# OFA-Sys/ONE-PEACE

Measured on AMD Instinct MI355X. Metric: pretrain samples/s (tri-modal global batch) ONE-PEACE-4B, higher is better.
Workload: dtype bf16

## Files before the change

include/onepeace_hip.h:

```cpp
#ifndef ONEPEACE_HIP_H
#define ONEPEACE_HIP_H

#include <stdint.h>

#ifdef __cplusplus
extern "C" {
#endif

int op_abi_version(void);
const char* op_last_error(void);

int op_prof_enable(int on);
int op_prof_reserve(int events);
int op_prof_collect(double* ms, int64_t* count, double* work, int n_families);

int op_layernorm_fwd(const void* x, const void* w, const void* b, void* y, float* mean, float* rstd, int64_t rows,
                     int64_t cols, float eps, int act_gelu, int dtype, const int* x_rows, void* stream);
int64_t op_layernorm_bwd_workspace_bytes(int64_t rows, int64_t cols);
int op_layernorm_bwd(const void* dy, const void* x, const void* w, const void* b, const float* mean, const float* rstd,
                     const void* add, void* dx, void* dw, void* db, void* workspace, int64_t rows, int64_t cols,
                     int act_gelu, int accumulate, int dtype, const int* x_rows, void* stream);
int op_layernorm_bwd_skip(const void* dy, const void* x, const void* w, const float* mean, const float* rstd, const void* add, void* dx,
                          void* dw, void* db, void* workspace, int64_t rows, int64_t cols, int accumulate, const float* ps,
                          int64_t rows_per_sample, void* stream);

int op_gemm_nt(const void* A, int64_t lda, const void* B0, const void* B1, const void* B2, int64_t ldb, int64_t n_seg,
               const void* bias0, const void* bias1, const void* bias2, void* C, int64_t ldc, void* h0, void* h1,
               const void* resid, int64_t ldr, const void* gamma, const float* rowscale, int64_t rows_per_sample,
               const float* alpha, int64_t M, int64_t N, int64_t K, int epilogue, void* workspace, int64_t workspace_bytes,
               int64_t tune, const int* resid_rows, int64_t resid_rows_total, void* stream);
int op_gemm_tn(const void* A, int64_t lda, const void* B, int64_t ldb, void* C, int64_t ldc, int64_t M, int64_t N, int64_t K,
               int accumulate, void* workspace, int64_t workspace_bytes, int64_t tune, void* stream);
int op_gemm_nt_grouped(int64_t nprob, const void* const* A, const int64_t* M, int64_t lda, const void* const* B, int64_t ldb,
                       const void* const* bias, void* const* C, int64_t ldc, void* const* h0, void* const* h1,
                       const void* const* resid, int64_t ldr, const void* const* gamma, const float* const* rowscale,
                       const int64_t* rows_per_sample, int64_t N, int64_t K, int epilogue, int64_t tune, const int* const* resid_rows,
                       int64_t resid_rows_total, void* stream);
int op_gemm_nt_batched(const void* A, int64_t lda, int64_t stride_a, const void* W, int64_t ldb, int64_t stride_b, const void* bias,
                       int64_t stride_bias, void* C, int64_t ldc, int64_t stride_c, int64_t M, int64_t N, int64_t K, int64_t batch,
                       void* stream);
int op_audio_conv1_ln_gelu_fwd(const void* wav, int64_t stride, const void* w0, const void* b0, const void* lnw, const void* lnb, void* y,
                               float* mean, float* rstd, int64_t rows, int64_t C, float eps, void* stream);
int64_t op_audio_conv1_ln_gelu_bwd_workspace_bytes(int64_t C);
int op_audio_conv1_ln_gelu_bwd(const void* dy, const void* wav, int64_t stride, const void* w0, const void* b0, const void* lnw, const void* lnb,
                               const float* mean, const float* rstd, void* dw0, void* db0, void* dlnw, void* dlnb, void* workspace,
                               int64_t rows, int64_t C, int accumulate, void* stream);
int64_t op_gemm_tn_grouped_counter_bytes(void);
int64_t op_gemm_tn_grouped_plan(int64_t nprob, const int64_t* M, const int64_t* N, const int64_t* K, int64_t workgroups, int64_t tune,
                                int32_t* out, int64_t cap);
int op_gemm_tn_grouped(int64_t nprob, const void* const* A, const int64_t* lda, const void* const* B, const int64_t* ldb, void* const* C,
                       const int64_t* ldc, const int64_t* M, const int64_t* N, const int64_t* K, const int32_t* accumulate,
                       const void* const* W, const int64_t* ldw, float* const* rowdot, const void* const* rscale, void* counters,
                       int64_t tune, void* stream);
int op_gemm_tn_grouped_lists(int64_t nprob, const void* const* A, const int64_t* lda, const void* const* B, const int64_t* ldb, void* const* C,
                             const int64_t* ldc, const int64_t* M, const int64_t* N, const int64_t* K, const int32_t* accumulate,
                             const void* const* W, const int64_t* ldw, float* const* rowdot, const void* const* rscale,
                             const int32_t* const* ktiles, const int32_t* const* n_ktiles, void* counters, int64_t tune, void* stream);
int op_live_ktiles(int64_t nseg, const float* const* ps, const int64_t* row0, const int64_t* S, const int64_t* B, int64_t nprob,
                   const int64_t* prob_row0, const int64_t* prob_rows, int32_t* const* ktiles, int32_t* const* n_ktiles, void* stream);
int op_live_mwindows(int64_t nseg, const float* const* ps, const int64_t* ps_stride, const int64_t* row0, const int64_t* S, const int64_t* B,
                     const int64_t* wps, const int64_t* odd, const int64_t* seg_list, const int64_t* seg_prob, const int64_t* seg_base, int64_t nlist,
                     int32_t* const* windows,
                     int32_t* const* n_windows, const int64_t* max_windows, int64_t nout, void* const* out, const int64_t* out_ld,
                     const int64_t* out_cols, const int64_t* out_rows, void* stream);
int op_gemm_nt_grouped_windows(int64_t nprob, const void* const* A, const int64_t* M, int64_t lda, const void* const* B, int64_t ldb,
                               void* const* C, int64_t ldc, int64_t N, int64_t K, const int32_t* windows, const int32_t* n_windows,
                               int64_t max_windows, int64_t max_row_stride, int64_t tune, void* stream);
int op_live_mwindows_fwd(int64_t nseg, const float* const* ps, const int64_t* ps_stride, const int64_t* row0, const int64_t* S, const int64_t* B,
                         const int64_t* wps, const int64_t* odd, const int64_t* seg_list, const int64_t* seg_prob, const int64_t* seg_base,
                         int64_t nlist, int32_t* const* windows, int32_t* const* n_windows, const int64_t* max_windows, int64_t nout,
                         void* const* out, const int64_t* out_ld, const int64_t* out_cols, const int64_t* out_rows,
                         const void* const* out_src, const int64_t* out_src_ld, void* stream);
int op_gemm_nt_grouped_windows_fwd(int64_t nprob, const void* const* A, const int64_t* M, int64_t lda, const void* const* B, int64_t ldb,
                                   int64_t n_seg, const void* const* bias, void* const* C, int64_t ldc, const void* const* resid, int64_t ldr,
                                   const void* const* gamma, const float* const* rowscale, const int64_t* rows_per_sample, int64_t N,
                                   int64_t K, int epilogue, const int32_t* windows, const int32_t* n_windows, int64_t max_windows,
                                   int64_t max_row_stride, int64_t tune, void* stream);
int op_gemm_plan(int64_t M, int64_t N, int64_t K, int epilogue, int has_bias, int64_t workspace_bytes, int64_t tune, int* plan);

int op_quant_fp8_rows(const void* x, int64_t ldx, void* q, int64_t ldq, float* scale, int64_t rows, int64_t cols, void* stream);
int op_layernorm_fwd_q8(const void* x, const void* w, const void* b, void* y, float* mean, float* rstd, void* q8, float* q8_scale,
                        int64_t rows, int64_t cols, float eps, void* stream);
int op_ln_geglu_fwd_q8(const void* h0, const void* h1, int64_t ldh, const void* w, const void* b, void* y, float* mean, float* rstd, void* q8,
                       float* q8_scale, int64_t rows, int64_t cols, float eps, void* stream);
int op_gemm_nt_fp8(const void* A8, int64_t lda, const float* sa, const void* B0, const void* B1, int64_t ldb, const float* sb0,
                   const float* sb1, const void* bias, void* C, int64_t ldc, void* h0, void* h1, const void* resid, int64_t ldr,
                   const void* gamma, const float* rowscale, int64_t rows_per_sample, int64_t M, int64_t N, int64_t K, int epilogue,
                   int64_t tune, void* stream);

int op_attn_fwd(const void* q, const void* k, const void* v, int64_t ld, const void* bias, int64_t bias_batch_stride,
                const void* bias_frag, const void* key_pad, void* out, int64_t ldo, float* lse, int64_t lse_ld, int64_t B,
                int64_t S, int64_t Spad, int64_t heads, int64_t head_dim, float scale, int64_t tune, void* stream);
int64_t op_attn_bias_frag_elems(int64_t n_img, int64_t S);
int op_attn_bias_pack(const void* src, void* dst, int64_t n_img, int64_t S, int64_t Spad, void* stream);
int op_attn_bwd_delta(const void* dout, const void* out, int64_t ldo, float* delta, int64_t B, int64_t S, int64_t Spad,
                      int64_t heads, void* stream);
int64_t op_attn_bwd_dbias_slabs(int64_t B, int64_t S, int64_t heads, int64_t tune);
int op_attn_bwd(const void* q, const void* k, const void* v, int64_t ld, const void* dout, const void* out, int64_t ldo,
                const void* bias, const void* biasT, const void* bias_frag, int64_t bias_batch_stride, const void* key_pad,
                const float* lse, float* delta, void* dq,
                void* dk, void* dv, int64_t ldg, float* dbias, int64_t B, int64_t S, int64_t Spad, int64_t heads,
                int64_t head_dim, float scale, int64_t tune, void* stream);

int op_relpos_bias_build(const void* table, const int* bucket, int64_t bucket_ld, void* out, int64_t heads, int64_t S,
                         int64_t Spad, int transposed, void* stream);
int op_relpos_bias_bwd(const float* dbias, int64_t S, int64_t Spad, const int* pos, const int* seg, int64_t nseg, const int* bucket_seg,
                       int64_t num_rel, float* partial_ws, float* dtable, int64_t heads, void* stream);
int op_relpos_bias_build_ids(const void* table, const int* bucket, int64_t bucket_ld, const int* ids, void* out, int64_t B,
                             int64_t heads, int64_t K, int64_t Kpad, int transposed, void* stream);
int op_relpos_bias_fold_ids(const float* dbias, const int* ids, float* dense_ws, int64_t Sfull, int64_t B, int64_t heads, int64_t K,
                            int64_t Kpad, void* stream);

int op_transpose(const void* in, void* out, int64_t rows, int64_t cols, int64_t ld_in, int64_t ld_out, void* stream);
int op_transpose_scaled(const void* in, void* out, int64_t rows, int64_t cols, int64_t ld_in, int64_t ld_out, const void* scale,
                        void* stream);
int op_transpose_batched(const void* table, int64_t n, int64_t total_tiles, void* stream);
int64_t op_transpose_desc_bytes(void);
int64_t op_colsum_workspace_bytes(int64_t N);
int op_colsum_segments(const void* x, void* out0, void* out1, void* out2, void* workspace, int64_t M, int64_t n_seg,
                       int64_t seg_cols, int accumulate, void* stream);
int64_t op_resid_bwd_workspace_bytes(int64_t N);
int op_resid_bwd(const void* dout, const void* y, const void* gamma, const float* rowscale, int64_t rows_per_sample,
                 void* dbranch, void* dgamma, void* dbias, float* g0, void* workspace, int64_t M, int64_t N, int accumulate,
                 const int* dout_rows, void* stream);
int op_resid_bwd_skip(const void* dout, const void* y, const void* gamma, const float* rowscale, int64_t rows_per_sample,
                      void* dbranch, void* dgamma, void* dbias, float* g0, void* workspace, int64_t M, int64_t N, int accumulate,
                      const int* dout_rows, void* stream);
int op_gamma_grad_finish(const float* rowdot, int64_t slots, const void* b0, const float* g00, const void* b1, const float* g01,
                         const void* b2, const float* g02, void* dgamma, int64_t N, int accumulate, void* stream);
int op_ln_geglu_bwd(const void* dy, const void* h0, const void* h1, const void* w, const float* mean, const float* rstd,
                    void* dh0, void* dh1, int64_t ldd, int64_t ldh, void* dw, void* db, void* workspace, int64_t rows,
                    int64_t cols, int accumulate, void* stream);
int op_ln_geglu_fwd(const void* h0, const void* h1, int64_t ldh, const void* w, const void* b, void* y, float* mean, float* rstd,
                    int64_t rows, int64_t cols, float eps, void* stream);
int op_ln_geglu_fwd_skip(const void* h0, const void* h1, int64_t ldh, const void* w, const void* b, void* y, float* mean, float* rstd,
                         int64_t rows, int64_t cols, float eps, const float* ps, int64_t rows_per_sample, void* stream);
int op_ln_geglu_bwd_skip(const void* dy, const void* h0, const void* h1, const void* w, const float* mean, const float* rstd,
                         void* dh0, void* dh1, int64_t ldd, int64_t ldh, void* dw, void* db, void* workspace, int64_t rows,
                         int64_t cols, int accumulate, const float* ps, int64_t rows_per_sample, void* stream);
int op_colsum(const void* x, const void* y, const float* rowscale, int64_t rows_per_sample, const void* mul, void* out,
              void* workspace, int64_t M, int64_t N, int accumulate, int out_dtype, void* stream);
int op_geglu_bwd(const void* dg, const void* h0, const void* h1, void* dh0, void* dh1, int64_t numel, void* stream);
int op_scale_rows(const void* dout, const void* gamma, const float* rowscale, int64_t rows_per_sample, void* dbranch,
                  int64_t M, int64_t N, void* stream);

int op_l2norm_fwd(const void* x, void* y, float* inv_norm, int64_t rows, int64_t cols, float eps, int out_dtype, void* stream);
int op_l2norm_bwd(const void* dy, const void* y, const float* inv_norm, void* dx, int64_t rows, int64_t cols, int y_dtype,
                  void* stream);
int op_infonce_rows(float* sim, int64_t rows, int64_t n, int64_t ld, int64_t target0, float label_smoothing, float gscale,
                    float* row_loss, float* row_hit, float* row_dot, int write_grad, void* stream);

int op_adamw_step(void* p, const void* g, float* m, float* v, int64_t numel, float lr, float beta1, float beta2, float eps,
                  float weight_decay, int64_t step, float grad_scale, const float* grad_sqnorm, float clip_norm,
                  void* stream);
int op_adamw_step_groups(void* p, const void* g, float* m, float* v, int64_t numel, const int64_t* group_end8,
                         const float* group_lr_scale, const float* group_weight_decay, int64_t n_groups, float lr, float beta1,
                         float beta2, float eps, int64_t step, float grad_scale, const float* grad_sqnorm, float clip_norm,
                         void* stream);
int op_adamw_step_groups_master(void* p, float* master, const void* g, float* m, float* v, int64_t numel,
                                const int64_t* group_end8, const float* group_lr_scale, const float* group_weight_decay,
                                int64_t n_groups, float lr, float beta1, float beta2, float eps, int64_t step, float grad_scale,
                                const float* grad_sqnorm, float clip_norm, void* stream);
int op_ema_step(float* ema, const void* p, int64_t numel, float keep, float take, void* stream);
int op_adamw_step_groups_ema(void* p, float* master, const void* g, float* m, float* v, float* ema, int64_t numel,
                             const int64_t* group_end8, const float* group_lr_scale, const float* group_weight_decay,
                             int64_t n_groups, float lr, float beta1, float beta2, float eps, int64_t step, float grad_scale,
                             const float* grad_sqnorm, float clip_norm, float ema_keep, float ema_take, void* stream);
int op_adamw_step_shard(void* p, const void* g, int64_t numel, int64_t first8, int64_t count8, float* m, float* v, float* master,
                        float* ema, const int64_t* group_end8, const float* group_lr_scale, const float* group_weight_decay,
                        int64_t n_groups, float lr, float beta1, float beta2, float eps, int64_t step, float grad_scale,
                        const float* grad_sqnorm, float clip_norm, float ema_keep, float ema_take, void* stream);
int op_sqnorm(const void* x, int64_t numel, float* workspace, float* out, void* stream);

int op_rows_gather(const void* src, void* dst, const int* list, int64_t nseg, const int64_t* src_row0, const int64_t* dst_row0,
                   const int64_t* S, const int64_t* n_kept, const int64_t* dst_rows, const int64_t* n_samples, const int64_t* list_off,
                   int64_t dst_total, int64_t cols, void* stream);
int op_rows_merge(const void* base, const void* upd, void* out, const int* list, int64_t nseg, const int64_t* src_row0,
                  const int64_t* dst_row0, const int64_t* S, const int64_t* n_kept, const int64_t* dst_rows, const int64_t* n_samples,
                  const int64_t* list_off, int64_t total, int64_t cols, void* stream);
int op_rows_map(int* map, const int* list, int64_t nseg, const int64_t* src_row0, const int64_t* dst_row0, const int64_t* S,
                const int64_t* n_kept, const int64_t* dst_rows, const int64_t* n_samples, const int64_t* list_off, int64_t dst_total,
                void* stream);

int64_t op_sim_topk_splits(int64_t M, int64_t N, int64_t splits);
int64_t op_sim_topk_workspace_bytes(int64_t M, int64_t N, int64_t k, int64_t splits);
// ... 70 lines not shown
```

one-peace_amd/csrc/attention.hip:

```cpp
#include <type_traits>

#include "common.h"

namespace {

constexpr int HD = 64;
constexpr int BQ = 128;
constexpr int BKV = 64;
constexpr int VSTRIDE = 160;

struct AttnArgs {
  const bf16_t* q; const bf16_t* k; const bf16_t* v; int64_t ld;
  const bf16_t* bias;
  int64_t bias_bs;
  const uint8_t* key_pad;
  bf16_t* out; int64_t ldo;
  float* lse;
  int64_t lse_ld;
  int B, S, Spad, heads;
  float scale;
};

__device__ __forceinline__ bf16x8 pack8(const float* a, const float* b) {
  bf16x8 r;
// ... 366 lines not shown
      if (FULL || kb < nkb) {
#pragma unroll
        for (int r = 0; r < 4; ++r) {
          const float e = __builtin_amdgcn_exp2f(__builtin_fmaf(st[kb][r], c1, -m2_use));
          pv[kb][r] = e;
          psum += e;
        }
      } else {
#pragma unroll
        for (int r = 0; r < 4; ++r) pv[kb][r] = 0.f;
      }
    }
    l_run = l_run * alpha + psum;
#pragma unroll
    for (int db = 0; db < 4; ++db)
#pragma unroll
      for (int r = 0; r < 4; ++r) ot[db][r] *= alpha;
    bf16x8 pf[2];
    pf[0] = pack8(pv[0], pv[1]);
    pf[1] = pack8(pv[2], pv[3]);

#pragma unroll
    for (int m = 0; m < 2; ++m) {
      if (!FULL && 2 * m >= nkb) break;
#pragma unroll
      for (int db = 0; db < 4; ++db) {
        const bf16x8 vf = join_tr(tr_read(vt + trsw[db] + (2 * m) * 2048), tr_read(vt + trsw[db] + (2 * m + 1) * 2048));
        ot[db] = __builtin_amdgcn_mfma_f32_16x16x32_bf16(vf, pf[m], ot[db], 0, 0, 0);
      }
    }
  };

  const int ntiles = (p.S + BKV - 1) / BKV;
  for (int kt = 0; kt < ntiles; ++kt) {
    const int k0 = kt * BKV;
    if (k0 + BKV <= p.S) tile(k0, std::true_type{});
    else tile(k0, std::false_type{});
  }

  float l = l_run;
  l += __shfl_xor(l, 16);
  l += __shfl_xor(l, 32);
  if (q0 + t >= p.S) continue;
  const float inv = 1.f / l;
  bf16_t* op = p.out + (row_base + q0 + t) * p.ldo + h * HD;
#pragma unroll
  for (int db = 0; db < 4; ++db) {
    bf16x4 o;
#pragma unroll
    for (int r = 0; r < 4; ++r) o[r] = (bf16_t)(ot[db][r] * inv);
    *reinterpret_cast<bf16x4*>(op + db * 16 + g * 4) = o;
  }
  if (g == 0 && p.lse) p.lse[((int64_t)b * p.heads + h) * p.lse_ld + q0 + t] = m2_run * (1.0f / LOG2E) + logf(l);
  }
}

constexpr int PERS_NW = 8;
constexpr int PERS_MAX_ROWS = 288;
constexpr int PERS_SCR = 68;
constexpr int PERS_PPT = 2;

__device__ __forceinline__ s16x4 tr_read_a(const char* p) {
  s16x4 r;
  asm volatile("ds_read_b64_tr_b16 %0, %1" : "=v"(r) : "v"((unsigned)(uintptr_t)((__attribute__((address_space(3))) const char*)p)));
  return r;
}
#define ATTN_WAIT_LGKM0()                         \
  do {                                            \
    __builtin_amdgcn_s_waitcnt(0xC07F);           \
    __builtin_amdgcn_sched_barrier(0);            \
  } while (0)

__device__ __forceinline__ void gload16_asm(bf16x8& d, const void* p) { asm volatile("global_load_dwordx4 %0, %1, off" : "=v"(d) : "v"(p)); }
__device__ __forceinline__ void gload4_asm(unsigned& d, const void* p) { asm volatile("global_load_dword %0, %1, off" : "=v"(d) : "v"(p)); }
template <int OFF>
__device__ __forceinline__ void gload16_s(bf16x8& d, const void* sbase, unsigned voff) {
  asm volatile("s_nop 4\n\tglobal_load_dwordx4 %0, %1, %2 offset:%3" : "=v"(d) : "v"(voff), "s"(sbase), "n"(OFF));
}
template <int OFF>
__device__ __forceinline__ void gload4_s(unsigned& d, const void* sbase, unsigned voff) {
  asm volatile("s_nop 4\n\tglobal_load_dword %0, %1, %2 offset:%3" : "=v"(d) : "v"(voff), "s"(sbase), "n"(OFF));
}

template <bool HAS_BIAS, bool HAS_PAD>
__global__ __launch_bounds__(PERS_NW * 64, 2) void attn_fwd_pers_kernel(AttnArgs p, const bf16_t* __restrict__ bias_frag, int rows_pad,
                                                                         int nitems) {
  extern __shared__ __attribute__((aligned(16))) char smem[];
  const int tid = threadIdx.x, lane = tid & 63;
  const int wid = __builtin_amdgcn_readfirstlane(tid >> 6);
  const int g = lane >> 4, t = lane & 15;
  const int KVB = 2 * rows_pad * 128;
  float* scratch = reinterpret_cast<float*>(smem + 2 * KVB);
  const int nqb = (p.S + 15) >> 4, nkp = (p.S + 31) >> 5;
  const bool has_left = nqb > 2 * PERS_NW;
  const int q0 = wid * 32;
  const int nact = min(2, max(0, nqb - 2 * wid));
  const int64_t per_head = (int64_t)nqb * nkp * FRAG_BLOCK;
  const int ntiles = (p.S + BKV - 1) / BKV;
  const float c1 = p.scale * LOG2E;

  bf16x8 sel_lo, sel_hi;
  {
    const bf16_t inv = (bf16_t)(1.0f / p.scale), zero = (bf16_t)0.f;
#pragma unroll
    for (int i = 0; i < 8; ++i) {
      sel_lo[i] = (g * 8 + i == t) ? inv : zero;
      sel_hi[i] = (g * 8 + i == 16 + t) ? inv : zero;
    }
  }
  int trsw[4];
#pragma unroll
  for (int db = 0; db < 4; ++db) trsw[db] = tr_off_swz(0, db, g, t);
  const int kswz[2] = {((0 * 4 + g) ^ (t & 7)) << 4, ((1 * 4 + g) ^ (t & 7)) << 4};

  const int ngrp = rows_pad >> 3;
  const int r_in = lane >> 3, slot = lane & 7;
  const int npiece = (2 * ngrp - wid + PERS_NW - 1) / PERS_NW;
  auto piece = [&](int it, int buf, int j) {
    const int b = it / p.heads, h = it - b * p.heads;
    const int grp = wid + j * PERS_NW;
    const bool isv = grp >= ngrp;
    const int gi = isv ? grp - ngrp : grp;
    const int r = gi * 8 + r_in;
    const int kr = min(r, p.S - 1);
    const bf16_t* src = (isv ? p.v : p.k) + ((int64_t)b * p.S + kr) * p.ld + h * HD + ((slot ^ (r & 7)) << 3);
    char* dst = smem + buf * KVB + (isv ? rows_pad * 128 : 0) + gi * 1024;
    __builtin_amdgcn_global_load_lds((const __attribute__((address_space(1))) void*)src,
                                     (__attribute__((address_space(3))) void*)dst, 16, 0, 0);
  };
  auto load_q = [&](int it, int qrow, bf16x8 (&q)[2]) {
    const int b = it / p.heads, h = it - b * p.heads;
    const bf16_t* qp = p.q + ((int64_t)b * p.S + qrow) * p.ld + h * HD;
#pragma unroll
    for (int kk = 0; kk < 2; ++kk) q[kk] = *reinterpret_cast<const bf16x8*>(qp + kk * 32 + g * 8);
  };
  const int qi_main[2] = {min(q0 + t, p.S - 1), min(q0 + 16 + t, p.S - 1)};

  bf16x8 bn[2][2];
  unsigned padn[4] = {0u, 0u, 0u, 0u};
  auto small_loads = [&](int it, int kt) {
    const int b = it / p.heads, h = it - b * p.heads;
    if constexpr (HAS_BIAS) {
      const bf16_t* fhead = bias_frag + ((p.bias_bs != 0 ? (int64_t)b * p.heads : 0) + h) * per_head + lane * 8;
#pragma unroll
      for (int qb = 0; qb < 2; ++qb) {
        const bf16_t* fb = fhead + (int64_t)min(2 * wid + qb, nqb - 1) * nkp * FRAG_BLOCK;
#pragma unroll
        for (int m = 0; m < 2; ++m) gload16_asm(bn[qb][m], fb + min(2 * kt + m, nkp - 1) * FRAG_BLOCK);
      }
    }
    if constexpr (HAS_PAD) {
      const uint8_t* pr = p.key_pad + (int64_t)b * p.Spad + g * 4 + kt * BKV;
#pragma unroll
      for (int kb = 0; kb < 4; ++kb) gload4_asm(padn[kb], pr + kb * 16);
    }
  };

  constexpr int NSMALL = (HAS_BIAS ? 4 : 0) + (HAS_PAD ? 4 : 0);
  bf16x8 qn[2][2], ql[2], bfl[2];
  unsigned padl[2][2] = {{0u, 0u}, {0u, 0u}};
  auto late_loads = [&](int it_next, int it) {
    {
      const int b = it_next / p.heads, h = it_next - b * p.heads;
#pragma unroll
      for (int qb = 0; qb < 2; ++qb) {
        const bf16_t* qp = p.q + ((int64_t)b * p.S + qi_main[qb]) * p.ld + h * HD;
#pragma unroll
        for (int kk = 0; kk < 2; ++kk) gload16_asm(qn[qb][kk], qp + kk * 32 + g * 8);
      }
    }
    if (has_left) {
      const int b = it / p.heads, h = it - b * p.heads;
      const bf16_t* qp = p.q + ((int64_t)b * p.S + p.S - 1) * p.ld + h * HD;
#pragma unroll
      for (int kk = 0; kk < 2; ++kk) gload16_asm(ql[kk], qp + kk * 32 + g * 8);
      if constexpr (HAS_BIAS) {
        const bf16_t* fleft = bias_frag + ((p.bias_bs != 0 ? (int64_t)b * p.heads : 0) + h) * per_head + lane * 8 + (int64_t)(nqb - 1) * nkp * FRAG_BLOCK;
        gload16_asm(bfl[0], fleft + wid * FRAG_BLOCK);
        gload16_asm(bfl[1], fleft + min(PERS_NW, nkp - 1) * FRAG_BLOCK);
      }
      if constexpr (HAS_PAD) {
        const uint8_t* pr = p.key_pad + (int64_t)b * p.Spad + g * 4;
#pragma unroll
        for (int j = 0; j < 2; ++j) {
          gload4_asm(padl[0][j], pr + (2 * wid + j) * 16);
          gload4_asm(padl[1][j], pr + min((2 * PERS_NW + j) * 16, p.Spad - 16));
        }
      }
    }
  };

  int item = blockIdx.x;
  const int step = gridDim.x;
  if (item < nitems) {
    for (int j = 0; j < npiece; ++j) piece(item, 0, j);
    load_q(item, qi_main[0], qn[0]);
    load_q(item, qi_main[1], qn[1]);
    small_loads(item, 0);
  }
  int buf = 0, prev_item = -1;
  auto wait_all = [&]() {
    asm volatile("s_waitcnt vmcnt(0)" : "+v"(qn[0][0]), "+v"(qn[0][1]), "+v"(qn[1][0]), "+v"(qn[1][1]), "+v"(bn[0][0]), "+v"(bn[0][1]), "+v"(bn[1][0]), "+v"(bn[1][1]),
                 "+v"(padn[0]), "+v"(padn[1]), "+v"(padn[2]), "+v"(padn[3]) : : "memory");
  };
  wait_all();

  auto merge_left = [&](int it, int sb) {
    const float* sc = scratch + sb * (PERS_NW * PERS_SCR);
    float M = -INFINITY;
#pragma unroll
    for (int w = 0; w < PERS_NW; ++w) M = fmaxf(M, sc[w * PERS_SCR + 64]);
    float L = 0.f, o = 0.f;
#pragma unroll
    for (int w = 0; w < PERS_NW; ++w) {
      const float f = __builtin_amdgcn_exp2f(sc[w * PERS_SCR + 64] - M);
      L = __builtin_fmaf(sc[w * PERS_SCR + 65], f, L);
      o = __builtin_fmaf(sc[w * PERS_SCR + lane], f, o);
    }
    const int b = it / p.heads, h = it - b * p.heads;
    const int qrow = p.S - 1;
    p.out[((int64_t)b * p.S + qrow) * p.ldo + h * HD + lane] = (bf16_t)(o / L);
    if (lane == 0 && p.lse) p.lse[((int64_t)b * p.heads + h) * p.lse_ld + qrow] = M * (1.0f / LOG2E) + logf(L);
  };

  for (; item < nitems; item += step, buf ^= 1) {
    const int b = item / p.heads, h = item - b * p.heads;
    const int64_t row_base = (int64_t)b * p.S;
    __syncthreads();
    bf16x8 qf[2][2] = {{qn[0][0], qn[0][1]}, {qn[1][0], qn[1][1]}};
    const bool more = item + step < nitems;
    const int nxt = more ? item + step : item;
    if (has_left && prev_item >= 0 && wid == ((prev_item / step) & (PERS_NW - 1))) merge_left(prev_item, buf ^ 1);
    prev_item = item;

    const char* ldsK = smem + buf * KVB;
    const char* ldsV = ldsK + rows_pad * 128;

    f32x4 ot[2][4];
    float m2_run[2] = {-INFINITY, -INFINITY}, l_run[2] = {0.f, 0.f};
#pragma unroll
    for (int qb = 0; qb < 2; ++qb)
#pragma unroll
      for (int db = 0; db < 4; ++db) ot[qb][db] = (f32x4){0.f, 0.f, 0.f, 0.f};

    auto tile = [&](const int kt, auto full_c) {
      constexpr bool FULL = decltype(full_c)::value;
      const int k0 = kt * BKV;
      const int nkb = FULL ? 4 : ((p.S - k0 + 15) >> 4);
      bf16x8 bf[2][2];
      unsigned padw[4] = {0u, 0u, 0u, 0u};
      if constexpr (HAS_BIAS) {
#pragma unroll
        for (int qb = 0; qb < 2; ++qb)
#pragma unroll
          for (int m = 0; m < 2; ++m) bf[qb][m] = bn[qb][m];
      }
      if constexpr (HAS_PAD) {
#pragma unroll
        for (int kb = 0; kb < 4; ++kb) padw[kb] = padn[kb];
      }
      __builtin_amdgcn_sched_barrier(0);
      if constexpr (FULL) {
        small_loads(item, kt + 1);
      } else {
        late_loads(nxt, item);
        small_loads(nxt, 0);
      }
      __builtin_amdgcn_sched_barrier(0);
#pragma unroll
      for (int jj = 0; jj < PERS_PPT; ++jj) piece(nxt, buf ^ 1, min(kt * PERS_PPT + jj, npiece - 1));
      __builtin_amdgcn_sched_barrier(0);
      if (nact == 0) return;

      const char* kt_ = ldsK + k0 * 128;
      const char* vt = ldsV + k0 * 128;
      f32x4 st[2][4];
#pragma unroll
      for (int qb = 0; qb < 2; ++qb)
#pragma unroll
        for (int kb = 0; kb < 4; ++kb) st[qb][kb] = (f32x4){0.f, 0.f, 0.f, 0.f};
#pragma unroll
      for (int kb = 0; kb < 4; ++kb) {
        if (!FULL && kb >= nkb) break;
#pragma unroll
        for (int kk = 0; kk < 2; ++kk) {
          const bf16x8 kf = *reinterpret_cast<const bf16x8*>(kt_ + (kb * 16 + t) * 128 + kswz[kk]);
#pragma unroll
          for (int qb = 0; qb < 2; ++qb) st[qb][kb] = __builtin_amdgcn_mfma_f32_16x16x32_bf16(kf, qf[qb][kk], st[qb][kb], 0, 0, 0);
        }
        if constexpr (HAS_BIAS) {
#pragma unroll
          for (int qb = 0; qb < 2; ++qb)
            st[qb][kb] = __builtin_amdgcn_mfma_f32_16x16x32_bf16(bf[qb][kb >> 1], (kb & 1) ? sel_hi : sel_lo, st[qb][kb], 0, 0, 0);
        }
      }
      s16x4 va0[4], va1[4];
#pragma unroll
      for (int db = 0; db < 4; ++db) {
        va0[db] = tr_read_a(vt + trsw[db]);
        va1[db] = tr_read_a(vt + trsw[db] + 2048);
      }
      bf16x8 pf[2][2];
#pragma unroll
      for (int qb = 0; qb < 2; ++qb) {
        float mx = -INFINITY;
#pragma unroll
        for (int kb = 0; kb < 4; ++kb) {
          if (!FULL && kb >= nkb) break;
          const int key = k0 + kb * 16 + g * 4;
#pragma unroll
          for (int r = 0; r < 4; ++r) {
            if constexpr (!FULL || HAS_PAD) {
              bool masked = false;
              if constexpr (!FULL) masked = key + r >= p.S;
              if constexpr (HAS_PAD) masked = masked || ((padw[kb] >> (8 * r)) & 0xffu);
              st[qb][kb][r] = masked ? -INFINITY : st[qb][kb][r];
            }
            mx = fmaxf(mx, st[qb][kb][r]);
          }
        }
        mx = fmaxf(mx, __shfl_xor(mx, 16));
        mx = fmaxf(mx, __shfl_xor(mx, 32));
        const float m2_new = fmaxf(m2_run[qb], mx * c1);
        const float m2_use = (m2_new == -INFINITY) ? 0.f : m2_new;
        const float alpha = __builtin_amdgcn_exp2f(m2_run[qb] - m2_use);
        m2_run[qb] = m2_new;
        float psum = 0.f;
        float pv[4][4];
#pragma unroll
        for (int kb = 0; kb < 4; ++kb) {
          if (FULL || kb < nkb) {
#pragma unroll
            for (int r = 0; r < 4; ++r) {
              const float e = __builtin_amdgcn_exp2f(__builtin_fmaf(st[qb][kb][r], c1, -m2_use));
              pv[kb][r] = e;
              psum += e;
            }
          } else {
#pragma unroll
            for (int r = 0; r < 4; ++r) pv[kb][r] = 0.f;
          }
        }
        l_run[qb] = l_run[qb] * alpha + psum;
#pragma unroll
        for (int db = 0; db < 4; ++db)
#pragma unroll
          for (int r = 0; r < 4; ++r) ot[qb][db][r] *= alpha;
        pf[qb][0] = pack8(pv[0], pv[1]);
// ... 776 lines not shown
#pragma unroll
        for (int kb = 0; kb < 4; ++kb) { st[kb] = (f32x4){0.f, 0.f, 0.f, 0.f}; ds[0][kb] = (f32x4){0.f, 0.f, 0.f, 0.f}; }
#pragma unroll
        for (int kb = 0; kb < 4; ++kb) {
          if (k0 + kb * 16 >= p.S) break;
#pragma unroll
          for (int kk = 0; kk < 2; ++kk) {
            st[kb] = __builtin_amdgcn_mfma_f32_16x16x32_bf16(kfrag(kb, kk), qf[0][kk], st[kb], 0, 0, 0);
            ds[0][kb] = __builtin_amdgcn_mfma_f32_16x16x32_bf16(vfrag(kb, kk), of[0][kk], ds[0][kb], 0, 0, 0);
          }
          st[kb] = __builtin_amdgcn_mfma_f32_16x16x32_bf16(bfr[kb >> 1], (kb & 1) ? sel_hi : sel_lo, st[kb], 0, 0, 0);
        }
        const float nl2 = -lse[0] * LOG2E, dl = del[0];
        const bool may_mask = (k0 + BKV > p.S) || (p.key_pad != nullptr);
        if (may_mask) {
#pragma unroll
          for (int kb = 0; kb < 4; ++kb) {
            const int key = k0 + kb * 16 + g * 4;
#pragma unroll
            for (int r = 0; r < 4; ++r) {
              const bool dead = (key + r >= p.S) || ((padw[kb] >> (8 * r)) & 0xffu);
              const float pr = __builtin_amdgcn_exp2f(dead ? -INFINITY : __builtin_fmaf(st[kb][r], c1, nl2));
              ds[0][kb][r] = pr * (ds[0][kb][r] - dl);
            }
          }
        } else {
#pragma unroll
          for (int kb = 0; kb < 4; ++kb)
#pragma unroll
            for (int r = 0; r < 4; ++r)
              ds[0][kb][r] = __builtin_amdgcn_exp2f(__builtin_fmaf(st[kb][r], c1, nl2)) * (ds[0][kb][r] - dl);
        }
      } else {
        ds_tile<1, true, (NT < 6)>(p, b, h, k0, q0w, g, t, qf, of, lse, del, kfrag, vfrag, biasfrag, prefetch, ds);
      }
#pragma unroll
      for (int c = 0; c < NT; ++c) {
        if (kt == c) {
#pragma unroll
          for (int kb = 0; kb < 4; ++kb)
            if (c < NT - 1 || kb < LASTB) acc[c][kb] += ds[0][kb];
        }
      }
#pragma unroll
      for (int m = 0; m < 2; ++m) {
        if (k0 + m * 32 >= p.S) break;
        float a0[4], a1[4];
#pragma unroll
        for (int r = 0; r < 4; ++r) { a0[r] = ds[0][2 * m][r]; a1[r] = ds[0][2 * m + 1][r]; }
        const bf16x8 dsf = pack8(a0, a1);
#pragma unroll
        for (int db = 0; db < 4; ++db) {
          const bf16x8 kT = join_tr(tr_read(ldsK + trsw[db] + (2 * m) * 2048), tr_read(ldsK + trsw[db] + (2 * m + 1) * 2048));
          dqT[db] = __builtin_amdgcn_mfma_f32_16x16x32_bf16(kT, dsf, dqT[db], 0, 0, 0);
        }
      }
    }
    if (wave_active && q0w + t < p.S) {
      bf16_t* qp = p.dq + ((int64_t)b * p.S + q0w + t) * p.ldg + h * HD;
#pragma unroll
      for (int db = 0; db < 4; ++db) {
        bf16x4 a;
#pragma unroll
        for (int r = 0; r < 4; ++r) a[r] = (bf16_t)(dqT[db][r] * p.scale);
        *reinterpret_cast<bf16x4*>(qp + db * 16 + g * 4) = a;
      }
    }
  }
  if (!wave_active || q0w + t >= p.S) return;
  float* drow = p.dbias + (((int64_t)chunk * p.heads + h) * p.S + q0w + t) * p.Spad + g * 4;
#pragma unroll
  for (int kt = 0; kt < NT; ++kt) {
    f32x4 cur[4];
#pragma unroll
    for (int kb = 0; kb < 4; ++kb)
      if ((kt < NT - 1 || kb < LASTB) && kt * BKV + kb * 16 < p.Spad) cur[kb] = *reinterpret_cast<const f32x4*>(drow + kt * BKV + kb * 16);
#pragma unroll
    for (int kb = 0; kb < 4; ++kb)
      if ((kt < NT - 1 || kb < LASTB) && kt * BKV + kb * 16 < p.Spad)
        *reinterpret_cast<f32x4*>(drow + kt * BKV + kb * 16) = cur[kb] + acc[kt][kb];
  }
}

template <bool HAS_BIAS, bool HAS_PAD, int NT, int LASTB, bool LEFT>
__device__ __forceinline__ void attn_bwd_dq_pers_body(const AttnBwdArgs& p, char* smem, int rows_pad, int nqh, int qhalf0) {
  const int tid = threadIdx.x, lane = tid & 63;
  const int wid = __builtin_amdgcn_readfirstlane(tid >> 6);
  const int g = lane >> 4, t = lane & 15;
  const int KVB = 2 * rows_pad * 128;
  float* scratch = reinterpret_cast<float*>(smem + 2 * KVB);
  const int nqb = (p.S + 15) >> 4, nkp = (p.S + 31) >> 5;
  const int qhalf = qhalf0, h = (blockIdx.x / nqh) % p.heads, chunk = blockIdx.x / (nqh * p.heads);
  const int b_begin = chunk * p.bchunk, b_end = min(p.B, b_begin + p.bchunk);
  if (b_begin >= b_end) return;
  const int qblk = qhalf * PERS_NW + wid;
  const bool active = qblk < min(nqb, 2 * PERS_NW);
  constexpr bool has_left = LEFT;
  const int q0w = min(qblk, nqb - 1) * 16;
  const int qi = min(q0w + t, p.S - 1);
  const float c1 = p.scale * LOG2E;
  const int64_t per_head = (int64_t)nqb * nkp * FRAG_BLOCK;

  bf16x8 sel_lo, sel_hi;
  {
    const bf16_t inv = (bf16_t)(1.0f / p.scale), zero = (bf16_t)0.f;
#pragma unroll
    for (int i = 0; i < 8; ++i) {
      sel_lo[i] = (g * 8 + i == t) ? inv : zero;
      sel_hi[i] = (g * 8 + i == 16 + t) ? inv : zero;
    }
  }
  int trsw[4];
#pragma unroll
  for (int db = 0; db < 4; ++db) trsw[db] = tr_off_swz(0, db, g, t);
  const int kswz[2] = {((0 * 4 + g) ^ (t & 7)) << 4, ((1 * 4 + g) ^ (t & 7)) << 4};

  const int ngrp = rows_pad >> 3;
  const int r_in = lane >> 3, slot = lane & 7;
  const int npiece = (2 * ngrp - wid + PERS_NW - 1) / PERS_NW;
  auto piece = [&](int b, int buf, int j) {
    const int grp = wid + j * PERS_NW;
    const bool isv = grp >= ngrp;
    const int gi = isv ? grp - ngrp : grp;
    int rl = r_in;
    asm volatile("" : "+v"(rl));
    const int r = gi * 8 + rl;
    const int kr = min(r, p.S - 1);
    const unsigned voff = (unsigned)((kr * (int)p.ld + ((slot ^ (r & 7)) << 3)) * 2);
    const char* sbase = (const char*)((isv ? p.v : p.k) + (int64_t)b * p.S * p.ld + h * HD);
    char* dst = smem + buf * KVB + (isv ? rows_pad * 128 : 0) + gi * 1024;
    __builtin_amdgcn_global_load_lds((const __attribute__((address_space(1))) void*)(sbase + voff),
                                     (__attribute__((address_space(3))) void*)dst, 16, 0, 0);
  };

  constexpr int NSMALL = (HAS_BIAS ? 2 : 0) + (HAS_PAD ? 4 : 0);
  constexpr int BPPT = 3;
  auto ppt_of = [](int kt) { return kt < 3 ? BPPT : 0; };
  const bf16_t* fwave = HAS_BIAS ? p.bias_frag + (int64_t)h * per_head + (int64_t)(q0w >> 4) * nkp * FRAG_BLOCK : nullptr;
  const bf16_t* fleft = HAS_BIAS ? p.bias_frag + (int64_t)h * per_head + (int64_t)(nqb - 1) * nkp * FRAG_BLOCK : nullptr;
  const unsigned vo_frag = lane * 16, vo_pad = g * 4;
  const unsigned vo_q = (unsigned)(((int64_t)qi * p.ld + h * HD + g * 8) * 2), vo_o = (unsigned)(((int64_t)qi * p.ldo + h * HD + g * 8) * 2);
  const unsigned vo_ql = (unsigned)(((int64_t)(p.S - 1) * p.ld + h * HD + g * 8) * 2), vo_ol = (unsigned)(((int64_t)(p.S - 1) * p.ldo + h * HD + g * 8) * 2);
  const unsigned vo_lse = qi * 4, vo_lsel = (p.S - 1) * 4;
  bf16x8 bn[2];
  unsigned padn[4] = {0u, 0u, 0u, 0u};
  auto small_loads = [&](int b, int kt) {
    if constexpr (HAS_BIAS) {
      gload16_s<0>(bn[0], fwave + min(2 * kt, nkp - 1) * FRAG_BLOCK, vo_frag);
      gload16_s<0>(bn[1], fwave + min(2 * kt + 1, nkp - 1) * FRAG_BLOCK, vo_frag);
    }
    if constexpr (HAS_PAD) {
      const uint8_t* pr = p.key_pad + (int64_t)b * p.Spad + kt * BKV;
      gload4_s<0>(padn[0], pr, vo_pad);
      gload4_s<16>(padn[1], pr, vo_pad);
      gload4_s<32>(padn[2], pr, vo_pad);
      gload4_s<48>(padn[3], pr, vo_pad);
    }
  };
  bf16x8 qn[2], don[2], oon[2], ql[2], dol[2], ool[2], bfl[2];
  float lsen, lsel;
  unsigned padl[2][2] = {{0u, 0u}, {0u, 0u}};
  auto query_loads = [&](int b, unsigned voq, unsigned voo, unsigned vol, bf16x8 (&q)[2], bf16x8 (&d)[2], bf16x8 (&o)[2], float& l) {
    const bf16_t* sq = p.q + (int64_t)b * p.S * p.ld;
    const bf16_t* sd = p.dout + (int64_t)b * p.S * p.ldo;
    const bf16_t* so = p.out + (int64_t)b * p.S * p.ldo;
    gload16_s<0>(q[0], sq, voq);
    gload16_s<64>(q[1], sq, voq);
    gload16_s<0>(d[0], sd, voo);
    gload16_s<64>(d[1], sd, voo);
    gload16_s<0>(o[0], so, voo);
    gload16_s<64>(o[1], so, voo);
    unsigned lw;
    gload4_s<0>(lw, p.lse + ((int64_t)b * p.heads + h) * p.Spad, vol);
    l = __builtin_bit_cast(float, lw);
  };
  auto late_loads = [&](int b_next, int b) {
    (void)b_next;
    if (has_left) {
      query_loads(b, vo_ql, vo_ol, vo_lsel, ql, dol, ool, lsel);
      if constexpr (HAS_BIAS) {
        gload16_s<0>(bfl[0], fleft + wid * FRAG_BLOCK, vo_frag);
        gload16_s<0>(bfl[1], fleft + min(PERS_NW, nkp - 1) * FRAG_BLOCK, vo_frag);
      }
      if constexpr (HAS_PAD) {
        const uint8_t* pr = p.key_pad + (int64_t)b * p.Spad;
        gload4_s<0>(padl[0][0], pr + 2 * wid * 16, vo_pad);
        gload4_s<16>(padl[0][1], pr + 2 * wid * 16, vo_pad);
        gload4_s<0>(padl[1][0], pr + min(2 * PERS_NW * 16, p.Spad - 32), vo_pad);
        gload4_s<16>(padl[1][1], pr + min(2 * PERS_NW * 16, p.Spad - 32), vo_pad);
      }
    }
  };

  f32x4 acc[NT][4], accl[2][2];
#pragma unroll
  for (int kt = 0; kt < NT; ++kt)
#pragma unroll
    for (int kb = 0; kb < 4; ++kb) acc[kt][kb] = (f32x4){0.f, 0.f, 0.f, 0.f};
#pragma unroll
  for (int i = 0; i < 2; ++i)
#pragma unroll
    for (int j = 0; j < 2; ++j) accl[i][j] = (f32x4){0.f, 0.f, 0.f, 0.f};

  for (int j = 0; j < npiece; ++j) piece(b_begin, 0, j);
  query_loads(b_begin, vo_q, vo_o, vo_lse, qn, don, oon, lsen);
  small_loads(b_begin, 0);
  int buf = 0, prev_b = -1;
  auto merge_left = [&](int b, int sb) {
    const float* sc = scratch + sb * (PERS_NW * 64);
    float o = 0.f;
#pragma unroll
    for (int w = 0; w < PERS_NW; ++w) o += sc[w * 64 + lane];
    p.dq[((int64_t)b * p.S + p.S - 1) * p.ldg + h * HD + lane] = (bf16_t)(o * p.scale);
  };

  auto wait_all = [&]() {
    asm volatile("s_waitcnt vmcnt(0)" : "+v"(qn[0]), "+v"(qn[1]), "+v"(don[0]), "+v"(don[1]), "+v"(oon[0]), "+v"(oon[1]), "+v"(lsen), "+v"(bn[0]), "+v"(bn[1]),
                 "+v"(padn[0]), "+v"(padn[1]), "+v"(padn[2]), "+v"(padn[3]) : : "memory");
  };
  wait_all();
  for (int b = b_begin; b < b_end; ++b, buf ^= 1) {
    __syncthreads();
    const bf16x8 qf[2] = {qn[0], qn[1]}, dof[2] = {don[0], don[1]};
    const float dl = delta_from_frags(dof, oon);
    const float nl2 = -lsen * LOG2E;
    if (active && g == 0 && q0w + t < p.S) p.delta_w[((int64_t)b * p.heads + h) * p.Spad + q0w + t] = dl;
    const int nxt = b + 1 < b_end ? b + 1 : b;
    if (has_left && prev_b >= 0 && wid == (prev_b & (PERS_NW - 1))) merge_left(prev_b, buf ^ 1);
    prev_b = b;
    const char* ldsK = smem + buf * KVB;
    const char* ldsV = ldsK + rows_pad * 128;
    f32x4 dqT[4];
#pragma unroll
    for (int db = 0; db < 4; ++db) dqT[db] = (f32x4){0.f, 0.f, 0.f, 0.f};

    auto tile = [&](const int kt, auto last_c) {
      constexpr bool LAST = decltype(last_c)::value;
      const int k0 = kt * BKV;
      if (kt > 0) {
        if (ppt_of(kt - 1) > 0) {
          if constexpr (HAS_BIAS && HAS_PAD)
            asm volatile("s_waitcnt vmcnt(%6)" : "+v"(bn[0]), "+v"(bn[1]), "+v"(padn[0]), "+v"(padn[1]), "+v"(padn[2]), "+v"(padn[3]) : "n"(BPPT));
          else if constexpr (HAS_BIAS)
            asm volatile("s_waitcnt vmcnt(%2)" : "+v"(bn[0]), "+v"(bn[1]) : "n"(BPPT));
          else if constexpr (HAS_PAD)
            asm volatile("s_waitcnt vmcnt(%4)" : "+v"(padn[0]), "+v"(padn[1]), "+v"(padn[2]), "+v"(padn[3]) : "n"(BPPT));
        } else {
          if constexpr (HAS_BIAS && HAS_PAD)
            asm volatile("s_waitcnt vmcnt(0)" : "+v"(bn[0]), "+v"(bn[1]), "+v"(padn[0]), "+v"(padn[1]), "+v"(padn[2]), "+v"(padn[3]));
          else if constexpr (HAS_BIAS)
            asm volatile("s_waitcnt vmcnt(0)" : "+v"(bn[0]), "+v"(bn[1]));
          else if constexpr (HAS_PAD)
            asm volatile("s_waitcnt vmcnt(0)" : "+v"(padn[0]), "+v"(padn[1]), "+v"(padn[2]), "+v"(padn[3]));
        }
      }
      bf16x8 bf[2];
      unsigned padw[4] = {0u, 0u, 0u, 0u};
      if constexpr (HAS_BIAS) { bf[0] = bn[0]; bf[1] = bn[1]; }
      if constexpr (HAS_PAD) {
#pragma unroll
        for (int kb = 0; kb < 4; ++kb) padw[kb] = padn[kb];
      }
      __builtin_amdgcn_sched_barrier(0);
      if constexpr (!LAST) {
        if constexpr (!LEFT) {
          if (kt == NT - 2) query_loads(nxt, vo_q, vo_o, vo_lse, qn, don, oon, lsen);
        }
        small_loads(b, kt + 1);
      } else {
        late_loads(nxt, b);
        small_loads(nxt, 0);
      }
      __builtin_amdgcn_sched_barrier(0);
#pragma unroll
      for (int jj = 0; jj < BPPT; ++jj)
        if (ppt_of(kt) > 0) piece(nxt, buf ^ 1, min(kt * BPPT + jj, npiece - 1));
      __builtin_amdgcn_sched_barrier(0);
      const char* kt_ = ldsK + k0 * 128;
      const char* vt = ldsV + k0 * 128;
      constexpr int NKB = LAST ? LASTB : 4;
      constexpr int NM = (NKB + 1) / 2;
      if (!active) return;
#pragma unroll
      for (int m = 0; m < NM; ++m) {
        f32x4 st[2], ds[2];
#pragma unroll
        for (int j = 0; j < 2; ++j) {
          const int kb = 2 * m + j;
          st[j] = (f32x4){0.f, 0.f, 0.f, 0.f};
          ds[j] = (f32x4){0.f, 0.f, 0.f, 0.f};
          if (kb >= NKB) continue;
#pragma unroll
          for (int kk = 0; kk < 2; ++kk) {
            const bf16x8 kf = *reinterpret_cast<const bf16x8*>(kt_ + (kb * 16 + t) * 128 + kswz[kk]);
            const bf16x8 vf = *reinterpret_cast<const bf16x8*>(vt + (kb * 16 + t) * 128 + kswz[kk]);
            st[j] = __builtin_amdgcn_mfma_f32_16x16x32_bf16(kf, qf[kk], st[j], 0, 0, 0);
            ds[j] = __builtin_amdgcn_mfma_f32_16x16x32_bf16(vf, dof[kk], ds[j], 0, 0, 0);
          }
          if constexpr (HAS_BIAS) st[j] = __builtin_amdgcn_mfma_f32_16x16x32_bf16(bf[m], j ? sel_hi : sel_lo, st[j], 0, 0, 0);
        }
#pragma unroll
        for (int j = 0; j < 2; ++j) {
          const int kb = 2 * m + j;
          if (kb >= NKB) continue;
          const int key = k0 + kb * 16 + g * 4;
#pragma unroll
          for (int r = 0; r < 4; ++r) {
            float x = __builtin_fmaf(st[j][r], c1, nl2);
            if constexpr (LAST || HAS_PAD) {
              bool dead = false;
              if constexpr (LAST) dead = key + r >= p.S;
// ... 58 lines not shown
          s4[j] = (f32x4){0.f, 0.f, 0.f, 0.f};
          d4[j] = (f32x4){0.f, 0.f, 0.f, 0.f};
#pragma unroll
          for (int kk = 0; kk < 2; ++kk) {
            const bf16x8 kf = *reinterpret_cast<const bf16x8*>(ldsK + ((2 * kp + j) * 16 + t) * 128 + kswz[kk]);
            const bf16x8 vf = *reinterpret_cast<const bf16x8*>(ldsV + ((2 * kp + j) * 16 + t) * 128 + kswz[kk]);
            s4[j] = __builtin_amdgcn_mfma_f32_16x16x32_bf16(kf, ql[kk], s4[j], 0, 0, 0);
            d4[j] = __builtin_amdgcn_mfma_f32_16x16x32_bf16(vf, dol[kk], d4[j], 0, 0, 0);
          }
          if constexpr (HAS_BIAS) s4[j] = __builtin_amdgcn_mfma_f32_16x16x32_bf16(bfl[pc], j ? sel_hi : sel_lo, s4[j], 0, 0, 0);
        }
        float a0[4], a1[4];
#pragma unroll
        for (int j = 0; j < 2; ++j)
#pragma unroll
          for (int r = 0; r < 4; ++r) {
            bool dead = (2 * kp + j) * 16 + g * 4 + r >= p.S;
            if constexpr (HAS_PAD) dead = dead || ((padl[pc][j] >> (8 * r)) & 0xffu);
            const float x = dead ? -INFINITY : __builtin_fmaf(s4[j][r], c1, nl2l);
            const float v = __builtin_amdgcn_exp2f(x) * (d4[j][r] - dll);
            d4[j][r] = v;
            (j ? a1 : a0)[r] = v;
          }
        if constexpr (HAS_BIAS) { accl[pc][0] += d4[0]; accl[pc][1] += d4[1]; }
        const bf16x8 dsf = pack8(a0, a1);
        s16x4 k0r[4], k1r[4];
#pragma unroll
        for (int db = 0; db < 4; ++db) {
          k0r[db] = tr_read_a(ldsK + trsw[db] + (2 * kp) * 2048);
          k1r[db] = tr_read_a(ldsK + trsw[db] + (2 * kp + 1) * 2048);
        }
        ATTN_WAIT_LGKM0();
#pragma unroll
        for (int db = 0; db < 4; ++db) dql[db] = __builtin_amdgcn_mfma_f32_16x16x32_bf16(join_tr(k0r[db], k1r[db]), dsf, dql[db], 0, 0, 0);
      }
      float* sc = scratch + (buf * PERS_NW + wid) * 64;
      if (t == 0) {
#pragma unroll
        for (int db = 0; db < 4; ++db) *reinterpret_cast<f32x4*>(sc + db * 16 + g * 4) = dql[db];
      }
    }

    wait_all();
  }
  if (has_left && prev_b >= 0) {
    __syncthreads();
    if (wid == 0) merge_left(prev_b, buf ^ 1);
  }
  if constexpr (HAS_BIAS) {
    if (p.dbias == nullptr) return;
    if (active && q0w + t < p.S) {
      float* drow = p.dbias + (((int64_t)chunk * p.heads + h) * p.S + q0w + t) * p.Spad + g * 4;
#pragma unroll
      for (int kt = 0; kt < NT; ++kt) {
        f32x4 cur[4];
#pragma unroll
        for (int kb = 0; kb < 4; ++kb)
          if ((kt < NT - 1 || kb < LASTB) && kt * BKV + kb * 16 < p.Spad) cur[kb] = *reinterpret_cast<const f32x4*>(drow + kt * BKV + kb * 16);
#pragma unroll
        for (int kb = 0; kb < 4; ++kb)
          if ((kt < NT - 1 || kb < LASTB) && kt * BKV + kb * 16 < p.Spad)
            *reinterpret_cast<f32x4*>(drow + kt * BKV + kb * 16) = cur[kb] + acc[kt][kb];
      }
    }
    if (has_left && t == 0) {
      float* drow = p.dbias + (((int64_t)chunk * p.heads + h) * p.S + p.S - 1) * p.Spad + g * 4;
#pragma unroll
      for (int pc = 0; pc < 2; ++pc) {
        if (pc == 1 && wid != 0) break;
        const int kp = pc == 0 ? wid : PERS_NW;
#pragma unroll
        for (int j = 0; j < 2; ++j) {
          const int key0 = (2 * kp + j) * 16;
          if (key0 < p.Spad) {
            float* d = drow + key0;
            *reinterpret_cast<f32x4*>(d) = *reinterpret_cast<const f32x4*>(d) + accl[pc][j];
          }
        }
      }
    }
  }
}

template <bool HAS_BIAS, bool HAS_PAD, int NT, int LASTB>
__global__ __launch_bounds__(PERS_NW * 64, 2) void attn_bwd_dq_pers_kernel(AttnBwdArgs p, int rows_pad, int nqh) {
  extern __shared__ __attribute__((aligned(16))) char smem[];
  const int qhalf = blockIdx.x % nqh;
  const bool lone = ((p.S + 15) >> 4) > 2 * PERS_NW && qhalf == nqh - 1;
  if constexpr (NT == 5) {
    if (lone) {
      attn_bwd_dq_pers_body<HAS_BIAS, HAS_PAD, NT, LASTB, true>(p, smem, rows_pad, nqh, qhalf);
      return;
    }
  }
  attn_bwd_dq_pers_body<HAS_BIAS, HAS_PAD, NT, LASTB, false>(p, smem, rows_pad, nqh, qhalf);
}

constexpr int PERS_SCRL = 136;

template <int OFF>
__device__ __forceinline__ void gload1_s(unsigned& d, const void* sbase, unsigned voff) {
  asm volatile("s_nop 4\n\tglobal_load_ubyte %0, %1, %2 offset:%3" : "=v"(d) : "v"(voff), "s"(sbase), "n"(OFF));
}

__device__ __forceinline__ u32x4 attn_raw_rsrc(const void* base, int nbytes) {
  const uint64_t a = (uint64_t)base;
  return (u32x4){(unsigned)__builtin_amdgcn_readfirstlane((int)(unsigned)a), (unsigned)__builtin_amdgcn_readfirstlane((int)(unsigned)(a >> 32)) & 0xffffu,
                 (unsigned)__builtin_amdgcn_readfirstlane(nbytes), 0x00020000u};
}
__device__ __forceinline__ void bstore8(const bf16x4& data, const u32x4& rsrc, unsigned voff) {
  asm volatile("s_nop 4\n\tbuffer_store_dwordx2 %0, %1, %2, 0 offen\n\ts_nop 1" ::"v"(data), "v"(voff), "s"(rsrc) : "memory");
}

template <bool HAS_BIAS, bool HAS_PAD, int NT, bool LONE>
__global__ __launch_bounds__(PERS_NW * 64, 2) void attn_bwd_dkdv_pers_kernel(AttnBwdArgs p, int rows_pad, int nitems) {
  extern __shared__ __attribute__((aligned(16))) char smem[];
  const int tid = threadIdx.x, lane = tid & 63;
  const int wid = __builtin_amdgcn_readfirstlane(tid >> 6);
  const int g = lane >> 4, t = lane & 15;
  const int QBY = rows_pad * 128;
  const int BUFB = 2 * QBY + 6144;
  float* scratch = reinterpret_cast<float*>(smem + 2 * BUFB);
  const int kbase = wid * 32;
  const bool wave_active = kbase < min(p.S, 256);
  const float c1 = p.scale * LOG2E;

  bf16x8 sel_lo, sel_hi;
  {
    const bf16_t inv = (bf16_t)(1.0f / p.scale), zero = (bf16_t)0.f;
#pragma unroll
    for (int i = 0; i < 8; ++i) {
      sel_lo[i] = (g * 8 + i == t) ? inv : zero;
      sel_hi[i] = (g * 8 + i == 16 + t) ? inv : zero;
    }
  }
  int trsw[4];
#pragma unroll
  for (int db = 0; db < 4; ++db) trsw[db] = tr_off_swz(0, db, g, t);
  const int kswz[2] = {((0 * 4 + g) ^ (t & 7)) << 4, ((1 * 4 + g) ^ (t & 7)) << 4};

  const int ngrp = rows_pad >> 3;
  const int NG = 2 * ngrp + (LONE ? 6 : 4);
  const int r_in = lane >> 3, slot = lane & 7;
  const int npiece = (NG - wid + PERS_NW - 1) / PERS_NW;
  auto piece = [&](int it, int buf, int j) {
    const int b = it / p.heads, h = it - b * p.heads;
    const int grp = wid + j * PERS_NW;
    int rl = r_in;
    asm volatile("" : "+v"(rl));
    const char* sbase;
    unsigned voff;
    int dst_off;
    if (grp < 2 * ngrp) {
      const bool isd = grp >= ngrp;
      const int gi = isd ? grp - ngrp : grp;
      const int r = gi * 8 + rl;
      const int qr = min(r, p.S - 1);
      const int ldx = isd ? (int)p.ldo : (int)p.ld;
      voff = (unsigned)((qr * ldx + ((slot ^ (r & 7)) << 3)) * 2);
      sbase = isd ? (const char*)(p.dout + (int64_t)b * p.S * p.ldo + h * HD) : (const char*)(p.q + (int64_t)b * p.S * p.ld + h * HD);
      dst_off = (isd ? QBY : 0) + gi * 1024;
    } else {
      const int e = grp - 2 * ngrp;
      if (e < 4) {
        voff = (unsigned)min((e & 1) * 1024 + (rl * 8 + slot) * 16, p.Spad * 4 - 16);
        sbase = (const char*)((e < 2 ? p.lse : p.delta) + ((int64_t)b * p.heads + h) * p.Spad);
      } else {
        voff = (unsigned)(((p.S - 1) * (int)p.ld + slot * 8) * 2);
        sbase = (const char*)((e == 4 ? p.k : p.v) + (int64_t)b * p.S * p.ld + h * HD);
      }
      dst_off = 2 * QBY + e * 1024;
    }
    __builtin_amdgcn_global_load_lds((const __attribute__((address_space(1))) void*)(sbase + voff),
                                     (__attribute__((address_space(3))) void*)(smem + buf * BUFB + dst_off), 16, 0, 0);
  };

  const int key_kb[2] = {min(kbase + t, p.S - 1), min(kbase + 16 + t, p.S - 1)};
  const unsigned vo_k[2] = {(unsigned)((key_kb[0] * (int)p.ld + g * 8) * 2), (unsigned)((key_kb[1] * (int)p.ld + g * 8) * 2)};
  bf16x8 kf[2][2], vf[2][2], kn[LONE ? 1 : 2][2], vn[LONE ? 1 : 2][2];
  unsigned kdn[2] = {0u, 0u}, kdl = 0u;
  auto kv_loads = [&](int it, bf16x8 (&kd)[2][2], bf16x8 (&vd)[2][2]) {
    const int b = it / p.heads, h = it - b * p.heads;
    const bf16_t* sk = p.k + (int64_t)b * p.S * p.ld + h * HD;
    const bf16_t* sv = p.v + (int64_t)b * p.S * p.ld + h * HD;
#pragma unroll
    for (int kb = 0; kb < 2; ++kb) {
      gload16_s<0>(kd[kb][0], sk, vo_k[kb]);
      gload16_s<64>(kd[kb][1], sk, vo_k[kb]);
      gload16_s<0>(vd[kb][0], sv, vo_k[kb]);
      gload16_s<64>(vd[kb][1], sv, vo_k[kb]);
    }
    if constexpr (HAS_PAD) {
      const uint8_t* pr = p.key_pad + (int64_t)b * p.Spad;
      gload1_s<0>(kdn[0], pr, (unsigned)key_kb[0]);
      gload1_s<0>(kdn[1], pr, (unsigned)key_kb[1]);
      if constexpr (LONE) gload1_s<0>(kdl, pr, (unsigned)(p.S - 1));
    }
  };
  constexpr int NKV = 8 + (HAS_PAD ? (LONE ? 3 : 2) : 0);
  const unsigned vo_b[2] = {(unsigned)((key_kb[0] * p.Spad + g * 8) * 2), (unsigned)((key_kb[1] * p.Spad + g * 8) * 2)};
  const unsigned vo_bl = (unsigned)(((p.S - 1) * p.Spad + g * 8) * 2);
  bf16x8 bn[2][2], bfl[2];
  auto bias_loads = [&](int it, auto qt_c, auto m_c) {
    constexpr int QT = decltype(qt_c)::value, M = decltype(m_c)::value;
    if constexpr (HAS_BIAS) {
      const int h = it % p.heads;
      const bf16_t* sb = p.biasT + (int64_t)h * p.S * p.Spad;
      gload16_s<(QT * 64 + M * 32) * 2>(bn[M][0], sb, vo_b[0]);
      gload16_s<(QT * 64 + M * 32) * 2>(bn[M][1], sb, vo_b[1]);
    }
  };
  constexpr int NBH = HAS_BIAS ? 2 : 0;
  auto lone_bias_loads = [&](int it) {
    if constexpr (HAS_BIAS && LONE) {
      const int h = it % p.heads;
      const bf16_t* sb = p.biasT + (int64_t)h * p.S * p.Spad;
      gload16_s<0>(bfl[0], sb + wid * 32, vo_bl);
      gload16_s<512>(bfl[1], sb, vo_bl);
    }
  };
  constexpr int NLB = (HAS_BIAS && LONE) ? 2 : 0;
  constexpr int BPPT = NT == 5 ? 3 : 4;

  int item = blockIdx.x;
  const int step = gridDim.x;
  using I0 = std::integral_constant<int, 0>;
  using I1 = std::integral_constant<int, 1>;
  if (item < nitems) {
    for (int j = 0; j < npiece; ++j) piece(item, 0, j);
    if constexpr (LONE) kv_loads(item, kf, vf);
    else kv_loads(item, kn, vn);
    bias_loads(item, I0{}, I0{});
    bias_loads(item, I0{}, I1{});
  }
#define DKDV_WAIT_LOADS(NST)                                                                                                                  \
  do {                                                                                                                                     \
    if constexpr (LONE)                                                                                                                    \
      asm volatile("s_waitcnt vmcnt(%15)" : "+v"(kf[0][0]), "+v"(kf[0][1]), "+v"(kf[1][0]), "+v"(kf[1][1]), "+v"(vf[0][0]), "+v"(vf[0][1]),   \
                   "+v"(vf[1][0]), "+v"(vf[1][1]), "+v"(bn[0][0]), "+v"(bn[0][1]), "+v"(bn[1][0]), "+v"(bn[1][1]), "+v"(kdn[0]), "+v"(kdn[1]), \
                   "+v"(kdl) : "n"(NST) : "memory");                                                                                      \
    else                                                                                                                                   \
      asm volatile("s_waitcnt vmcnt(%15)" : "+v"(kn[0][0]), "+v"(kn[0][1]), "+v"(kn[1][0]), "+v"(kn[1][1]), "+v"(vn[0][0]), "+v"(vn[0][1]),   \
                   "+v"(vn[1][0]), "+v"(vn[1][1]), "+v"(bn[0][0]), "+v"(bn[0][1]), "+v"(bn[1][0]), "+v"(bn[1][1]), "+v"(kdn[0]), "+v"(kdn[1]), \
                   "+v"(kdl) : "n"(NST) : "memory");                                                                                      \
  } while (0)
  DKDV_WAIT_LOADS(0);
  int buf = 0, prev_item = -1;
  auto merge_lone = [&](int it, int sb) {
    const float* sc = scratch + sb * (PERS_NW * PERS_SCRL);
    float dv = 0.f, dk = 0.f;
#pragma unroll
    for (int w = 0; w < PERS_NW; ++w) { dv += sc[w * PERS_SCRL + lane]; dk += sc[w * PERS_SCRL + 64 + lane]; }
    const bool dead = sc[128] != 0.f;
    const int b = it / p.heads, h = it - b * p.heads;
    const int64_t row = ((int64_t)b * p.S + p.S - 1) * p.ldg + h * HD + lane;
    p.dv[row] = dead ? (bf16_t)0.f : (bf16_t)dv;
    p.dk[row] = dead ? (bf16_t)0.f : (bf16_t)(dk * p.scale);
  };

  for (; item < nitems; item += step, buf ^= 1) {
    const int b = item / p.heads, h = item - b * p.heads;
    asm volatile("s_waitcnt lgkmcnt(0)" ::: "memory");
    __builtin_amdgcn_s_barrier();
    asm volatile("" ::: "memory");
    if constexpr (!LONE) {
#pragma unroll
      for (int kb = 0; kb < 2; ++kb)
#pragma unroll
        for (int kk = 0; kk < 2; ++kk) { kf[kb][kk] = kn[kb][kk]; vf[kb][kk] = vn[kb][kk]; }
    }
    const bool kdead[2] = {HAS_PAD && kdn[0] != 0u, HAS_PAD && kdn[1] != 0u};
    const bool ldead = HAS_PAD && LONE && kdl != 0u;
    const int nxt = item + step < nitems ? item + step : item;
    if (LONE && prev_item >= 0 && wid == ((prev_item / step) & (PERS_NW - 1))) merge_lone(prev_item, buf ^ 1);
    prev_item = item;
    const char* ldsQ = smem + buf * BUFB;
    const char* ldsO = ldsQ + QBY;
    const float* ldsL = reinterpret_cast<const float*>(ldsQ + 2 * QBY);
    const float* ldsD = ldsL + 512;

    f32x4 dvT[2][4], dkT[2][4];
#pragma unroll
    for (int kb = 0; kb < 2; ++kb)
#pragma unroll
      for (int db = 0; db < 4; ++db) { dvT[kb][db] = (f32x4){0.f, 0.f, 0.f, 0.f}; dkT[kb][db] = (f32x4){0.f, 0.f, 0.f, 0.f}; }

    auto half = [&](const int q0h, auto nkb_c, const bf16x8 (&kx)[2][2], const bf16x8 (&vx)[2][2], const bf16x8 (&bx)[2],
                    f32x4 (&dvx)[2][4], f32x4 (&dkx)[2][4]) {
      constexpr int NKB = decltype(nkb_c)::value;
      f32x4 s[2][NKB], dp[2][NKB];
#pragma unroll
      for (int j = 0; j < 2; ++j)
#pragma unroll
        for (int kb = 0; kb < NKB; ++kb) { s[j][kb] = (f32x4){0.f, 0.f, 0.f, 0.f}; dp[j][kb] = (f32x4){0.f, 0.f, 0.f, 0.f}; }
      const bool second = q0h + 16 < p.S;
#pragma unroll
      for (int j = 0; j < 2; ++j) {
        if (j == 1 && !second) continue;
#pragma unroll
        for (int kk = 0; kk < 2; ++kk) {
          const int off = (q0h + j * 16 + t) * 128 + kswz[kk];
          const bf16x8 qfr = *reinterpret_cast<const bf16x8*>(ldsQ + off);
          const bf16x8 ofr = *reinterpret_cast<const bf16x8*>(ldsO + off);
#pragma unroll
          for (int kb = 0; kb < NKB; ++kb) {
            s[j][kb] = __builtin_amdgcn_mfma_f32_16x16x32_bf16(qfr, kx[kb][kk], s[j][kb], 0, 0, 0);
            dp[j][kb] = __builtin_amdgcn_mfma_f32_16x16x32_bf16(ofr, vx[kb][kk], dp[j][kb], 0, 0, 0);
          }
        }
        if constexpr (HAS_BIAS) {
#pragma unroll
          for (int kb = 0; kb < NKB; ++kb) s[j][kb] = __builtin_amdgcn_mfma_f32_16x16x32_bf16(j ? sel_hi : sel_lo, bx[kb], s[j][kb], 0, 0, 0);
        }
      }
      const s16x4 zero4 = {0, 0, 0, 0};
      s16x4 o0[2], o1[2], q0r[2], q1r[2];
      auto tr_request = [&](int dh) {
#pragma unroll
        for (int i = 0; i < 2; ++i) {
          const int db = 2 * dh + i;
          o0[i] = tr_read_a(ldsO + q0h * 128 + trsw[db]);
          q0r[i] = tr_read_a(ldsQ + q0h * 128 + trsw[db]);
          o1[i] = zero4;
          q1r[i] = zero4;
          if (second) {
            o1[i] = tr_read_a(ldsO + q0h * 128 + trsw[db] + 2048);
            q1r[i] = tr_read_a(ldsQ + q0h * 128 + trsw[db] + 2048);
          }
        }
      };
      float l2[2][4], dl[2][4];
#pragma unroll
      for (int j = 0; j < 2; ++j) {
        if (j == 1 && !second) continue;
        const int qrow = q0h + j * 16 + g * 4;
        const f32x4 l4 = *reinterpret_cast<const f32x4*>(ldsL + qrow);
        const f32x4 d4 = *reinterpret_cast<const f32x4*>(ldsD + qrow);
#pragma unroll
        for (int r = 0; r < 4; ++r) {
          const bool live = qrow + r < p.S;
          l2[j][r] = live ? l4[r] * LOG2E : INFINITY;
          dl[j][r] = live ? d4[r] : 0.f;
        }
      }
      __builtin_amdgcn_sched_barrier(0);
      tr_request(0);
      __builtin_amdgcn_sched_barrier(0);
#pragma unroll
      for (int j = 0; j < 2; ++j) {
        if (j == 1 && !second) continue;
#pragma unroll
        for (int kb = 0; kb < NKB; ++kb) {
#pragma unroll
          for (int r = 0; r < 4; ++r) {
            const float pr = __builtin_amdgcn_exp2f(__builtin_fmaf(s[j][kb][r], c1, -l2[j][r]));
            s[j][kb][r] = pr;
            dp[j][kb][r] = pr * (dp[j][kb][r] - dl[j][r]);
          }
        }
      }
      bf16x8 pfr[NKB], dsf[NKB];
#pragma unroll
      for (int kb = 0; kb < NKB; ++kb) {
        float a0[4], a1[4], b0[4], b1[4];
#pragma unroll
        for (int r = 0; r < 4; ++r) {
          a0[r] = s[0][kb][r]; a1[r] = s[1][kb][r];
          b0[r] = dp[0][kb][r]; b1[r] = dp[1][kb][r];
        }
        pfr[kb] = pack8(a0, a1);
        dsf[kb] = pack8(b0, b1);
      }
#pragma unroll
      for (int dh = 0; dh < 2; ++dh) {
        if (dh == 1) tr_request(1);
        ATTN_WAIT_LGKM0();
#pragma unroll
        for (int i = 0; i < 2; ++i) {
          const int db = 2 * dh + i;
          const bf16x8 oT = join_tr(o0[i], o1[i]), qT = join_tr(q0r[i], q1r[i]);
#pragma unroll
          for (int kb = 0; kb < NKB; ++kb) {
            dvx[kb][db] = __builtin_amdgcn_mfma_f32_16x16x32_bf16(oT, pfr[kb], dvx[kb][db], 0, 0, 0);
            dkx[kb][db] = __builtin_amdgcn_mfma_f32_16x16x32_bf16(qT, dsf[kb], dkx[kb][db], 0, 0, 0);
          }
        }
      }
    };

    auto tile = [&](auto qt_c) {
      constexpr int QT = decltype(qt_c)::value;
      constexpr bool LAST = QT == NT - 1;
      using QN = std::integral_constant<int, LAST ? 0 : QT + 1>;
      if constexpr (!LAST) {
#pragma unroll
        for (int jj = 0; jj < BPPT; ++jj) piece(nxt, buf ^ 1, min(QT * BPPT + jj, npiece - 1));
      }
      __builtin_amdgcn_sched_barrier(0);
      if (wave_active) half(QT * 64, std::integral_constant<int, 2>{}, kf, vf, bn[0], dvT, dkT);
      __builtin_amdgcn_sched_barrier(0);
      if constexpr (!LAST) bias_loads(item, QN{}, I0{});
      if constexpr (HAS_BIAS && QT > 0) {
        if constexpr (!LAST) asm volatile("s_waitcnt vmcnt(%2)" : "+v"(bn[1][0]), "+v"(bn[1][1]) : "n"(BPPT + NBH));
        else asm volatile("s_waitcnt vmcnt(0)" : "+v"(bn[1][0]), "+v"(bn[1][1]));
      }
      __builtin_amdgcn_sched_barrier(0);
      if (wave_active && QT * 64 + 32 < p.S) half(QT * 64 + 32, std::integral_constant<int, 2>{}, kf, vf, bn[1], dvT, dkT);
      __builtin_amdgcn_sched_barrier(0);
      if constexpr (!LAST) {
        bias_loads(item, QN{}, I1{});
        if constexpr (HAS_BIAS) asm volatile("s_waitcnt vmcnt(%2)" : "+v"(bn[0][0]), "+v"(bn[0][1]) : "n"(NBH));
      } else {
        lone_bias_loads(item);
        bias_loads(nxt, I0{}, I0{});
        bias_loads(nxt, I0{}, I1{});
        if constexpr (!LONE) kv_loads(nxt, kn, vn);
      }
    };
    tile(std::integral_constant<int, 0>{});
    tile(std::integral_constant<int, 1>{});
    tile(std::integral_constant<int, 2>{});
    tile(std::integral_constant<int, 3>{});
    if constexpr (NT == 5) tile(std::integral_constant<int, 4>{});

    if constexpr (LONE) {
      kv_loads(nxt, kf, vf);
      if constexpr (NLB > 0) asm volatile("s_waitcnt vmcnt(%2)" : "+v"(bfl[0]), "+v"(bfl[1]) : "n"(NKV + 2 * NBH));
      const char* ldsLK = ldsQ + 2 * QBY + 4096;
      bf16x8 kl[2][2], vl[2][2];
#pragma unroll
      for (int kk = 0; kk < 2; ++kk) {
        kl[0][kk] = *reinterpret_cast<const bf16x8*>(ldsLK + (kk * 4 + g) * 16);
        vl[0][kk] = *reinterpret_cast<const bf16x8*>(ldsLK + 1024 + (kk * 4 + g) * 16);
        kl[1][kk] = kl[0][kk];
        vl[1][kk] = vl[0][kk];
      }
      f32x4 dvl[2][4], dkl[2][4];
#pragma unroll
      for (int db = 0; db < 4; ++db) { dvl[0][db] = (f32x4){0.f, 0.f, 0.f, 0.f}; dkl[0][db] = (f32x4){0.f, 0.f, 0.f, 0.f}; }
      const bf16x8 bl0[2] = {bfl[0], bfl[0]}, bl1[2] = {bfl[1], bfl[1]};
      half(wid * 32, std::integral_constant<int, 1>{}, kl, vl, bl0, dvl, dkl);
      if (wid == 0) half(256, std::integral_constant<int, 1>{}, kl, vl, bl1, dvl, dkl);
      float* sc = scratch + (buf * PERS_NW + wid) * PERS_SCRL;
      if (t == 0) {
#pragma unroll
        for (int db = 0; db < 4; ++db) {
          *reinterpret_cast<f32x4*>(sc + db * 16 + g * 4) = dvl[0][db];
          *reinterpret_cast<f32x4*>(sc + 64 + db * 16 + g * 4) = dkl[0][db];
        }
      }
      if (wid == 0 && lane == 0) sc[128] = ldead ? 1.f : 0.f;
    }

    {
      const int nrec = ((min(p.S, 256) - 1) * (int)p.ldg + HD) * 2;
      const u32x4 rk = attn_raw_rsrc(p.dk + (int64_t)b * p.S * p.ldg + h * HD, nrec);
      const u32x4 rv = attn_raw_rsrc(p.dv + (int64_t)b * p.S * p.ldg + h * HD, nrec);
#pragma unroll
      for (int kb = 0; kb < 2; ++kb) {
        const unsigned voff = (unsigned)(((kbase + kb * 16 + t) * (int)p.ldg + g * 4) * 2);
#pragma unroll
        for (int db = 0; db < 4; ++db) {
          bf16x4 a, c;
#pragma unroll
          for (int r = 0; r < 4; ++r) {
            a[r] = kdead[kb] ? (bf16_t)0.f : (bf16_t)(dkT[kb][db][r] * p.scale);
            c[r] = kdead[kb] ? (bf16_t)0.f : (bf16_t)dvT[kb][db][r];
          }
          bstore8(a, rk, voff + db * 32);
          bstore8(c, rv, voff + db * 32);
        }
      }
      DKDV_WAIT_LOADS(16);
    }
  }
  if (LONE && prev_item >= 0) {
    __syncthreads();
    if (wid == 0) merge_lone(prev_item, buf ^ 1);
  }
}

#undef DKDV_WAIT_LOADS

__global__ __launch_bounds__(256, 2) void attn_bwd_dbias_kernel(AttnBwdArgs p) {
  __shared__ __attribute__((aligned(16))) char smem[2 * 64 * 128];
  char* ldsK = smem;
  char* ldsV = smem + 64 * 128;
  const int tid = threadIdx.x, lane = tid & 63, wid = tid >> 6;
  const int g = lane >> 4, t = lane & 15;
  const int h = blockIdx.z % p.heads, chunk = blockIdx.z / p.heads;
  const int q0w = blockIdx.x * BQ + wid * 32;
  const int k0 = blockIdx.y * BKV;
  const bool wave_active = q0w < p.S;
  f32x4 acc[2][4];
  bf16x4 breg[2][4];
#pragma unroll
// ... 16 lines not shown
    for (int i = 0; i < 2; ++i) {
      const int kr = min(k0 + st_row[i], p.S - 1);
      const int64_t off = ((int64_t)b * p.S + kr) * p.ld + h * HD + st_c[i] * 8;
      rk[i] = *reinterpret_cast<const u32x4*>(p.k + off);
      rv[i] = *reinterpret_cast<const u32x4*>(p.v + off);
    }
  };
  auto write_tile = [&]() {
#pragma unroll
    for (int i = 0; i < 2; ++i) {
      const int off = st_row[i] * 128 + ((st_c[i] ^ (st_row[i] & 7)) << 4);
      *reinterpret_cast<u32x4*>(ldsK + off) = rk[i];
      *reinterpret_cast<u32x4*>(ldsV + off) = rv[i];
    }
  };
  const int b_begin = chunk * p.bchunk, b_end = min(p.B, (chunk + 1) * p.bchunk);
  bf16x8 qn[2][2], on[2][2];
  float lsen[2], deln[2];
  auto load_q = [&](int b) {
    const int64_t row_base = (int64_t)b * p.S;
#pragma unroll
    for (int qb = 0; qb < 2; ++qb) {
      const int qi = min(q0w + qb * 16 + t, p.S - 1);
#pragma unroll
      for (int kk = 0; kk < 2; ++kk) {
        qn[qb][kk] = *reinterpret_cast<const bf16x8*>(p.q + (row_base + qi) * p.ld + h * HD + kk * 32 + g * 8);
        on[qb][kk] = *reinterpret_cast<const bf16x8*>(p.dout + (row_base + qi) * p.ldo + h * HD + kk * 32 + g * 8);
      }
      lsen[qb] = p.lse[((int64_t)b * p.heads + h) * p.Spad + qi];
      deln[qb] = p.delta[((int64_t)b * p.heads + h) * p.Spad + qi];
    }
  };
  if (b_begin < b_end) {
    load_tile(b_begin);
    if (wave_active) load_q(b_begin);
  }
  for (int b = b_begin; b < b_end; ++b) {
    __syncthreads();
    write_tile();
    __syncthreads();
    if (b + 1 < b_end) load_tile(b + 1);
    if (!wave_active) continue;
    bf16x8 qf[2][2], of[2][2];
    float lse[2], del[2];
#pragma unroll
    for (int qb = 0; qb < 2; ++qb) {
#pragma unroll
      for (int kk = 0; kk < 2; ++kk) { qf[qb][kk] = qn[qb][kk]; of[qb][kk] = on[qb][kk]; }
      lse[qb] = lsen[qb];
      del[qb] = deln[qb];
    }
    if (b + 1 < b_end) load_q(b + 1);
    auto kfrag = [&](int kb, int kk) {
      return *reinterpret_cast<const bf16x8*>(ldsK + (kb * 16 + t) * 128 + (((kk * 4 + g) ^ (t & 7)) << 4));
    };
    auto vfrag = [&](int kb, int kk) {
      return *reinterpret_cast<const bf16x8*>(ldsV + (kb * 16 + t) * 128 + (((kk * 4 + g) ^ (t & 7)) << 4));
    };
    auto biasfrag = [&](int qb, int kb, int, int) { return breg[qb][kb]; };
    f32x4 ds[2][4];
    ds_tile<2, true, false>(p, b, h, k0, q0w, g, t, qf, of, lse, del, kfrag, vfrag, biasfrag, [] {}, ds);
#pragma unroll
    for (int qb = 0; qb < 2; ++qb)
#pragma unroll
      for (int kb = 0; kb < 4; ++kb)
#pragma unroll
        for (int r = 0; r < 4; ++r) acc[qb][kb][r] += ds[qb][kb][r];
  }
  if (!wave_active) return;
#pragma unroll
  for (int qb = 0; qb < 2; ++qb) {
    const int qi = q0w + qb * 16 + t;
    if (qi >= p.S) continue;
#pragma unroll
    for (int kb = 0; kb < 4; ++kb) {
      float* dst = p.dbias + ((int64_t)chunk * p.heads + h) * ((int64_t)p.S * p.Spad) + (int64_t)qi * p.Spad + k0 + kb * 16 + g * 4;
      if (k0 + kb * 16 >= p.Spad) continue;
#pragma unroll
      for (int r = 0; r < 4; ++r) dst[r] += acc[qb][kb][r];
    }
  }
}

enum : int64_t {
  FWD_STREAMING = 1 << 0, FWD_ABLATE_SHIFT = 1, FWD_ABLATE_MASK = 3, FWD_WAVES_SHIFT = 3, FWD_WAVES_MASK = 15, FWD_NO_PERS = 1 << 7,
  BWD_SEPARATE_DBIAS = 1 << 0, BWD_ROUND2_CHUNKS = 1 << 1, BWD_DKDV_KEYS_SHIFT = 2, BWD_DKDV_KEYS_MASK = 3, BWD_CHUNKS_SHIFT = 4,
  BWD_CHUNKS_MASK = 63, BWD_NO_PERS_DQ = 1 << 10, BWD_NO_LONE_KEYS = 1 << 11, BWD_NO_PERS_DKDV = 1 << 12, BWD_PERS_DKDV_256 = 1 << 13,
};

template <typename F> int with_bias_pad(const void* bias, const void* key_pad, F&& f) {
  return op_with_bool(bias != nullptr, [&](auto hb) { return op_with_bool(key_pad != nullptr, [&](auto hp) { return f(hb, hp); }); });
}

inline int dbias_chunks(int64_t B, int64_t S, int64_t heads, bool merge, bool round2_rule = false, int forced = 0) {
  if (!merge || ceil_div(S, BKV) > 6) return 1;
  if (forced > 0) return ceil_div(B, ceil_div(B, min((int64_t)forced, B)));
  if (round2_rule) {
    const int64_t base2 = (int64_t)ceil_div(S, 64) * heads;
    int chunks = (int)((768 + base2 - 1) / base2);
    if (chunks < 1) chunks = 1;
    if (chunks > B) chunks = (int)B;
    return ceil_div(B, ceil_div(B, chunks));
  }
  const int cus = op_num_cus();
  const int64_t base = (int64_t)ceil_div(S, 64) * heads, slots = 2 * (int64_t)cus;
  int best = 1;
  double best_cost = 1e30;
  for (int c = 1; c <= 32 && c <= B; ++c) {
    const int bchunk = ceil_div(B, c), n = ceil_div(B, bchunk);
    if (n != c) continue;
    const double cost = (double)ceil_div(base * n, slots) * bchunk + 0.05 * n;
    if (cost < best_cost - 1e-9) { best_cost = cost; best = c; }
  }
  return best;
}

inline int sep_bchunk(int64_t B, int64_t S, int64_t heads) {
  const int64_t base = (int64_t)ceil_div(S, BQ) * ceil_div(S, BKV) * heads;
  int chunks = (int)((1024 + base - 1) / base);
  if (chunks < 1) chunks = 1;
  if (chunks > B) chunks = (int)B;
  return ceil_div(B, chunks);
}

inline int pers_bwd_chunks(int64_t B, int64_t S, int64_t heads) {
  const int nqh = ceil_div(min((int64_t)ceil_div(S, 16), (int64_t)2 * PERS_NW), PERS_NW);
  int c = (int)(op_num_cus() / (heads * nqh));
  if (c < 1) c = 1;
  if (c > B) c = (int)B;
  return ceil_div(B, ceil_div(B, c));
}
inline bool pers_bwd_shape(int64_t S) { return S > 192 && S <= 257; }

inline int dkdv_pers_rows(int64_t S) { return (int)((S + 15) / 16) * 16; }
inline size_t dkdv_pers_lds(int64_t S) { return (size_t)2 * (2 * dkdv_pers_rows(S) * 128 + 6144) + 2 * PERS_NW * PERS_SCRL * 4; }

}

extern "C" int op_prof_begin(int family, double work, void* stream);
extern "C" void op_prof_end(int slot, void* stream);

static int attn_launched(int rc, int slot, void* stream) {
  op_prof_end(slot, stream);
  if (rc != OP_OK) return rc;
  OP_LAUNCH_CHECK();
  return OP_OK;
}

extern "C" {

int64_t op_attn_bwd_dbias_slabs(int64_t B, int64_t S, int64_t heads, int64_t tune) {
  if ((tune & BWD_SEPARATE_DBIAS) || ceil_div(S, BKV) > 6) return ceil_div(B, sep_bchunk(B, S, heads));
  const int64_t n = dbias_chunks(B, S, heads, true, (tune & BWD_ROUND2_CHUNKS) != 0, (int)((tune >> BWD_CHUNKS_SHIFT) & BWD_CHUNKS_MASK));
  if (!(tune & BWD_NO_PERS_DQ) && pers_bwd_shape(S)) return max(n, (int64_t)pers_bwd_chunks(B, S, heads));
  return n;
}

int op_attn_fwd(const void* q, const void* k, const void* v, int64_t ld, const void* bias, int64_t bias_batch_stride,
                const void* bias_frag, const void* key_pad, void* out, int64_t ldo, float* lse, int64_t lse_ld, int64_t B,
                int64_t S, int64_t Spad, int64_t heads, int64_t head_dim, float scale, int64_t tune, void* stream) {
  OP_CHECK_ARG(q && k && v && out, "attn_fwd: null pointer");
  OP_CHECK_ARG(head_dim == HD, "attn_fwd: head_dim %lld unsupported (only 64)", (long long)head_dim);
  OP_CHECK_ARG(B > 0 && S > 0 && heads > 0 && ld % 8 == 0 && ldo % 4 == 0, "attn_fwd: bad sizes");
  OP_CHECK_ARG((!bias && !key_pad) || (Spad >= ((S + 63) / 64) * 64 && Spad % 8 == 0),
               "attn_fwd: Spad must be >= S rounded up to 64");
  AttnArgs a;
  a.q = (const bf16_t*)q; a.k = (const bf16_t*)k; a.v = (const bf16_t*)v; a.ld = ld;
  a.bias = (const bf16_t*)bias; a.bias_bs = bias ? bias_batch_stride : 0; a.key_pad = (const uint8_t*)key_pad;
  a.out = (bf16_t*)out; a.ldo = ldo; a.lse = lse; a.lse_ld = lse_ld > 0 ? lse_ld : S;
  a.B = (int)B; a.S = (int)S; a.Spad = (int)Spad; a.heads = (int)heads; a.scale = scale;
  dim3 grid(ceil_div(S, BQ), (unsigned)heads, (unsigned)B);
  const int slot = op_prof_begin(1, 4.0 * (double)B * (double)heads * (double)S * (double)S * HD, stream);
  hipStream_t s = (hipStream_t)stream;
  const bool inv_exact = (float)(bf16_t)(1.0f / scale) * scale == 1.0f;
  const bf16_t* fr = (const bf16_t*)bias_frag;
  if (!(tune & FWD_STREAMING) && !(tune & FWD_NO_PERS) && S > 192 && S <= 257 && (!bias || (bias_frag && inv_exact))) {
    const int rows_pad = ceil_div(S, 32) * 32;
    const size_t sh = (size_t)4 * rows_pad * 128 + 2 * PERS_NW * PERS_SCR * 4;
    const int nitems = (int)(B * heads);
    const int nwg = min(nitems, op_num_cus());
    return attn_launched(with_bias_pad(bias, key_pad, [&](auto hb, auto hp) {
      constexpr auto kern = attn_fwd_pers_kernel<decltype(hb)::value, decltype(hp)::value>;
      OP_ENSURE_LDS(kern, 4 * PERS_MAX_ROWS * 128 + 2 * PERS_NW * PERS_SCR * 4, "attn_fwd");
      hipLaunchKernelGGL(kern, dim3(nwg), dim3(PERS_NW * 64), sh, s, a, fr, rows_pad, nitems);
      return OP_OK;
    }), slot, stream);
  }
  if (!(tune & FWD_STREAMING) && S <= RES_MAX_S && (!bias || (bias_frag && inv_exact))) {
    const int nqb = ceil_div(S, 16);
    const int nwg = ceil_div(nqb, RES_MAX_NW);
    const int qb_per_wg = ceil_div(nqb, nwg);
    int nwaves = qb_per_wg;
    const int forced_waves = (int)((tune >> FWD_WAVES_SHIFT) & FWD_WAVES_MASK);
    if (forced_waves) nwaves = min(qb_per_wg, forced_waves);
    else if (qb_per_wg == 9) nwaves = 8;
    const int rows_pad = ceil_div(S, 32) * 32;
    const size_t sh = (size_t)2 * rows_pad * 128;
    const dim3 rgrid(nwg, (unsigned)heads, (unsigned)B);
    const int abl = (int)((tune >> FWD_ABLATE_SHIFT) & FWD_ABLATE_MASK);
    return attn_launched(with_bias_pad(bias, key_pad, [&](auto hb, auto hp) {
      constexpr auto kern = attn_fwd_res_kernel<decltype(hb)::value, decltype(hp)::value>;
      OP_ENSURE_LDS(kern, 2 * RES_MAX_S * 128, "attn_fwd");
      hipLaunchKernelGGL(kern, rgrid, dim3(nwaves * 64), sh, s, a, fr, rows_pad, qb_per_wg, abl);
      return OP_OK;
    }), slot, stream);
  }
  return attn_launched(with_bias_pad(bias, key_pad, [&](auto hb, auto hp) {
    hipLaunchKernelGGL((attn_fwd_kernel<decltype(hb)::value, decltype(hp)::value>), grid, dim3(256), 0, s, a);
    return OP_OK;
  }), slot, stream);
}


int64_t op_attn_bias_frag_elems(int64_t n_img, int64_t S) {
  return n_img * (int64_t)ceil_div(S, 16) * ceil_div(S, 32) * FRAG_BLOCK;
}

int op_attn_bias_pack(const void* src, void* dst, int64_t n_img, int64_t S, int64_t Spad, void* stream) {
  OP_CHECK_ARG(src && dst && n_img > 0 && S > 0 && Spad >= S, "attn_bias_pack: bad args");
  const int nqb = ceil_div(S, 16), nkp = ceil_div(S, 32);
  const int64_t total = n_img * nqb * nkp * 64;
  hipLaunchKernelGGL(bias_pack_kernel, dim3(ceil_div(total, 256)), dim3(256), 0, (hipStream_t)stream, (const bf16_t*)src,
                     (bf16_t*)dst, (int)S, (int)Spad, nqb, nkp, total);
  OP_LAUNCH_CHECK();
  return OP_OK;
}

int op_attn_bwd_delta(const void* dout, const void* out, int64_t ldo, float* delta, int64_t B, int64_t S, int64_t Spad,
                      int64_t heads, void* stream) {
  OP_CHECK_ARG(dout && out && delta && ldo % 8 == 0, "attn_bwd_delta: bad args");
  const int64_t threads = B * S * heads * 8;
  hipLaunchKernelGGL(attn_delta_kernel, dim3(ceil_div(threads, 256)), dim3(256), 0, (hipStream_t)stream, (const bf16_t*)dout,
                     (const bf16_t*)out, ldo, delta, (int)B, (int)S, (int)Spad, (int)heads);
  OP_LAUNCH_CHECK();
  return OP_OK;
}

int op_attn_bwd(const void* q, const void* k, const void* v, int64_t ld, const void* dout, const void* out, int64_t ldo, const void* bias,
                const void* biasT, const void* bias_frag, int64_t bias_batch_stride, const void* key_pad, const float* lse,
                float* delta, void* dq,
                void* dk, void* dv, int64_t ldg, float* dbias, int64_t B, int64_t S, int64_t Spad, int64_t heads,
                int64_t head_dim, float scale, int64_t tune, void* stream) {
  const bool merge_dbias = !(tune & BWD_SEPARATE_DBIAS);
  OP_CHECK_ARG(q && k && v && dout && lse && delta && dq && dk && dv, "attn_bwd: null pointer");
  OP_CHECK_ARG(head_dim == HD, "attn_bwd: head_dim %lld unsupported (only 64)", (long long)head_dim);
  OP_CHECK_ARG(B > 0 && S > 0 && heads > 0, "attn_bwd: bad sizes");
  OP_CHECK_ARG(Spad >= ((S + 127) / 128) * 128 && Spad % 8 == 0, "attn_bwd: Spad must be >= S rounded up to 128");
  OP_CHECK_ARG((bias == nullptr) == (biasT == nullptr), "attn_bwd: bias and biasT must be given together");
  OP_CHECK_ARG(!dbias || bias, "attn_bwd: dbias without a bias");
  OP_CHECK_ARG(ld % 8 == 0 && ldo % 8 == 0 && ldg % 4 == 0, "attn_bwd: bad leading dims");
  AttnBwdArgs a;
  a.q = (const bf16_t*)q; a.k = (const bf16_t*)k; a.v = (const bf16_t*)v; a.ld = ld;
  a.dout = (const bf16_t*)dout; a.ldo = ldo; a.bias = (const bf16_t*)bias; a.biasT = (const bf16_t*)biasT;
  a.bias_frag = bias ? (const bf16_t*)bias_frag : nullptr;
  a.bias_bs = bias ? bias_batch_stride : 0;
  a.key_pad = (const uint8_t*)key_pad; a.lse = lse; a.delta = delta; a.out = (const bf16_t*)out; a.delta_w = delta;
  a.dq = (bf16_t*)dq; a.dk = (bf16_t*)dk; a.dv = (bf16_t*)dv; a.ldg = ldg; a.dbias = dbias;
  a.B = (int)B; a.S = (int)S; a.Spad = (int)Spad; a.heads = (int)heads; a.scale = scale;
  a.lone_keys = !(tune & BWD_NO_LONE_KEYS);
  a.bchunk = sep_bchunk(B, S, heads);
  hipStream_t s = (hipStream_t)stream;
  const double fl = 4.0 * (double)B * (double)heads * (double)S * (double)S * HD;
  const int bchunk_dkdv = a.bchunk;
  auto launch_dkdv = [&]() {
    AttnBwdArgs d = a;
    d.bchunk = bchunk_dkdv;
    const int sl = op_prof_begin(2, 2.0 * fl, stream);
    const int kb = ((tune >> BWD_DKDV_KEYS_SHIFT) & BWD_DKDV_KEYS_MASK) == 2 ? 1 : 2;
    return attn_launched(op_with_bool(bias != nullptr, [&](auto hb) {
      return op_with_int<1, 2>(kb, [&](auto kbc) {
        constexpr int KB = decltype(kbc)::value;
        hipLaunchKernelGGL((attn_bwd_dkdv_kernel<decltype(hb)::value, KB>), dim3(ceil_div(S, 64 * KB), (unsigned)heads, (unsigned)B), dim3(256),
                           0, s, d);
        return OP_OK;
      });
    }), sl, stream);
  };
  if (!out) {
    const int rc = launch_dkdv();
    if (rc != OP_OK) return rc;
  }
  const int nt = ceil_div(S, BKV);
  if (merge_dbias && !(tune & BWD_NO_PERS_DQ) && out && pers_bwd_shape(S) && a.bias_bs == 0 &&
      (!bias || (a.bias_frag != nullptr && (float)(bf16_t)(1.0f / scale) * scale == 1.0f))) {
    const int nqb = ceil_div(S, 16);
    const int nqh = ceil_div(min(nqb, 2 * PERS_NW), PERS_NW);
    const int chunks = pers_bwd_chunks(B, S, heads);
    a.bchunk = ceil_div(B, chunks);
    const int rows_pad = S > 256 ? PERS_MAX_ROWS : 256;
    const size_t sh = (size_t)4 * rows_pad * 128 + 2 * PERS_NW * 64 * 4;
    const int nwg = chunks * (int)heads * nqh;
    AttnBwdArgs d = a;
    if (!bias) d.dbias = nullptr;
    const int slot = op_prof_begin(2, 1.5 * fl, stream);
    int rc = attn_launched(with_bias_pad(bias, key_pad, [&](auto hb, auto hp) {
      return op_with_bool(S > 256, [&](auto lone) {
        constexpr bool LONE = decltype(lone)::value;
        constexpr auto kern = attn_bwd_dq_pers_kernel<decltype(hb)::value, decltype(hp)::value, LONE ? 5 : 4, LONE ? 1 : 4>;
        OP_ENSURE_LDS(kern, 4 * PERS_MAX_ROWS * 128 + 2 * PERS_NW * 64 * 4, "attn_bwd");
        hipLaunchKernelGGL(kern, dim3(nwg), dim3(PERS_NW * 64), sh, s, d, rows_pad, nqh);
        return OP_OK;
      });
    }), slot, stream);
    if (rc != OP_OK) return rc;
    a.bchunk = bchunk_dkdv;
    if ((tune & BWD_NO_PERS_DKDV) || (bias && !biasT) || (S == 256 && !(tune & BWD_PERS_DKDV_256))) return launch_dkdv();
    const int dk_rows = dkdv_pers_rows(S), nitems = a.B * a.heads, dk_nwg = min(nitems, op_num_cus());
    const int dk_slot = op_prof_begin(2, 2.0 * fl, stream);
    return attn_launched(with_bias_pad(bias, key_pad, [&](auto hb, auto hp) {
      return op_with_bool(S > 256, [&](auto lone) {
        constexpr bool LONE = decltype(lone)::value;
        constexpr auto kern = attn_bwd_dkdv_pers_kernel<decltype(hb)::value, decltype(hp)::value, LONE ? 5 : 4, LONE>;
        OP_ENSURE_LDS(kern, (int)dkdv_pers_lds(LONE ? 257 : 256), "attn_bwd");
        hipLaunchKernelGGL(kern, dim3(dk_nwg), dim3(PERS_NW * 64), dkdv_pers_lds(S), s, a, dk_rows, nitems);
        return OP_OK;
      });
    }), dk_slot, stream);
  }
  if (dbias && nt <= 6 && merge_dbias) {
    const int chunks = a.bias_bs != 0 ? (int)B : dbias_chunks(B, S, heads, true, (tune & BWD_ROUND2_CHUNKS) != 0,
                                                              (int)((tune >> BWD_CHUNKS_SHIFT) & BWD_CHUNKS_MASK));
    a.bchunk = ceil_div(B, chunks);
    const dim3 grid(ceil_div(S, 64), (unsigned)heads, (unsigned)chunks);
    const bool one_block = ceil_div(S - (nt - 1) * BKV, 16) == 1;
    const bool frag = a.bias_frag != nullptr && (float)(bf16_t)(1.0f / scale) * scale == 1.0f && (nt <= 4 || (nt == 5 && one_block));
    const int slot = op_prof_begin(2, 1.5 * fl, stream);
    const int rc = attn_launched(op_with_int<1, 2, 3, 4, 5, 6>(nt, [&](auto n) {
      return op_with_bool(frag, [&](auto fr) {
        return op_with_bool(one_block, [&](auto ob) {
          hipLaunchKernelGGL((attn_bwd_dq_dbias_kernel<decltype(n)::value, decltype(fr)::value, decltype(ob)::value ? 1 : 4>), grid, dim3(256),
                             0, s, a);
          return OP_OK;
        });
      });
    }), slot, stream);
    return rc != OP_OK || !out ? rc : launch_dkdv();
  }
  const int slot = op_prof_begin(2, 1.5 * fl, stream);
  int rc = attn_launched(op_with_bool(bias != nullptr, [&](auto hb) {
    hipLaunchKernelGGL(attn_bwd_dq_kernel<decltype(hb)::value>, dim3(ceil_div(S, BQ), (unsigned)heads, (unsigned)B), dim3(256), 0, s, a);
    return OP_OK;
  }), slot, stream);
  if (rc == OP_OK && out) rc = launch_dkdv();
  if (rc != OP_OK) return rc;
  if (dbias) {
    if (a.bias_bs != 0) a.bchunk = 1;
    const int chunks = ceil_div(B, a.bchunk);
    hipLaunchKernelGGL(attn_bwd_dbias_kernel, dim3(ceil_div(S, BQ), ceil_div(S, BKV), (unsigned)(heads * chunks)), dim3(256), 0,
                       s, a);
    OP_LAUNCH_CHECK();
  }
  return OP_OK;
}

}
```

one-peace_amd/hip.py:

```python
import ctypes
import os
from ctypes import c_double, c_float, c_int, c_int64, c_ubyte, c_void_p

import torch

_HERE = os.path.dirname(os.path.abspath(__file__))
LIB_PATH = os.environ.get("ONEPEACE_HIP_LIB") or os.path.join(_HERE, "lib", "libonepeace_hip.so")
_lib = None

DT_BF16, DT_F32 = 0, 1
EPI_BIAS, EPI_F32, EPI_GEGLU, EPI_RESID = 0, 1, 2, 3
PROF_GEMM, PROF_ATTN = 0, 1
ATTN_RESIDENT_MAX_S = 320

P = c_void_p
I64 = c_int64

SIGNATURES = {
    "op_abi_version": (c_int, []),
    "op_last_error": (ctypes.c_char_p, []),
    "op_prof_enable": (c_int, [c_int]),
    "op_prof_reserve": (c_int, [c_int]),
    "op_prof_collect": (c_int, [P, P, P, c_int]),
    "op_layernorm_fwd": (c_int, [P, P, P, P, P, P, I64, I64, c_float, c_int, c_int, P, P]),
    "op_layernorm_bwd_workspace_bytes": (I64, [I64, I64]),
    "op_attn_bwd_dbias_slabs": (I64, [I64, I64, I64, I64]),
    "op_layernorm_bwd": (c_int, [P, P, P, P, P, P, P, P, P, P, P, I64, I64, c_int, c_int, c_int, P, P]),
    "op_gemm_plan": (c_int, [c_int64, c_int64, c_int64, c_int, c_int, c_int64, I64, P]),
    "op_gemm_nt": (c_int, [P, I64, P, P, P, I64, I64, P, P, P, P, I64, P, P, P, I64, P, P, I64, P, I64, I64, I64,
                           c_int, P, I64, I64, P, I64, P]),
    "op_gemm_nt_grouped": (c_int, [I64, P, P, I64, P, I64, P, P, I64, P, P, P, I64, P, P, P, I64, I64, c_int, I64, P, I64, P]),
    "op_gemm_tn": (c_int, [P, I64, P, I64, P, I64, I64, I64, I64, c_int, P, I64, I64, P]),
    "op_gemm_tn_grouped_counter_bytes": (I64, []),
    "op_gemm_tn_grouped_plan": (I64, [I64, P, P, P, I64, I64, P, I64]),
    "op_gemm_tn_grouped": (c_int, [I64, P, P, P, P, P, P, P, P, P, P, P, P, P, P, P, I64, P]),
    "op_gemm_tn_grouped_lists": (c_int, [I64, P, P, P, P, P, P, P, P, P, P, P, P, P, P, P, P, P, I64, P]),
    "op_live_ktiles": (c_int, [I64, P, P, P, P, I64, P, P, P, P, P]),
    "op_live_mwindows": (c_int, [I64, P, P, P, P, P, P, P, P, P, P, I64, P, P, P, I64, P, P, P, P, P]),
    "op_gemm_nt_grouped_windows": (c_int, [I64, P, P, I64, P, I64, P, I64, I64, I64, P, P, I64, I64, I64, P]),
    "op_live_mwindows_fwd": (c_int, [I64, P, P, P, P, P, P, P, P, P, P, I64, P, P, P, I64, P, P, P, P, P, P, P]),
    "op_gemm_nt_grouped_windows_fwd": (c_int, [I64, P, P, I64, P, I64, I64, P, P, I64, P, I64, P, P, P, I64, I64, c_int, P, P, I64, I64,
                                               I64, P]),
    "op_gemm_nt_batched": (c_int, [P, I64, I64, P, I64, I64, P, I64, P, I64, I64, I64, I64, I64, I64, P]),
    "op_audio_conv1_ln_gelu_fwd": (c_int, [P, I64, P, P, P, P, P, P, P, I64, I64, c_float, P]),
    "op_audio_conv1_ln_gelu_bwd_workspace_bytes": (I64, [I64]),
    "op_audio_conv1_ln_gelu_bwd": (c_int, [P, P, I64, P, P, P, P, P, P, P, P, P, P, P, I64, I64, c_int, P]),
    "op_transpose": (c_int, [P, P, I64, I64, I64, I64, P]),
    "op_transpose_scaled": (c_int, [P, P, I64, I64, I64, I64, P, P]),
    "op_transpose_batched": (c_int, [P, I64, I64, P]),
    "op_transpose_desc_bytes": (I64, []),
    "op_colsum_workspace_bytes": (I64, [I64]),
    "op_colsum_segments": (c_int, [P, P, P, P, P, I64, I64, I64, c_int, P]),
    "op_resid_bwd_workspace_bytes": (I64, [I64]),
    "op_resid_bwd": (c_int, [P, P, P, P, I64, P, P, P, P, P, I64, I64, c_int, P, P]),
    "op_resid_bwd_skip": (c_int, [P, P, P, P, I64, P, P, P, P, P, I64, I64, c_int, P, P]),
    "op_layernorm_bwd_skip": (c_int, [P, P, P, P, P, P, P, P, P, P, I64, I64, c_int, P, I64, P]),
    "op_gamma_grad_finish": (c_int, [P, I64, P, P, P, P, P, P, P, I64, c_int, P]),
    "op_ln_geglu_bwd": (c_int, [P, P, P, P, P, P, P, P, I64, I64, P, P, P, I64, I64, c_int, P]),
    "op_ln_geglu_fwd": (c_int, [P, P, I64, P, P, P, P, P, I64, I64, c_float, P]),
    "op_ln_geglu_bwd_skip": (c_int, [P, P, P, P, P, P, P, P, I64, I64, P, P, P, I64, I64, c_int, P, I64, P]),
    "op_ln_geglu_fwd_skip": (c_int, [P, P, I64, P, P, P, P, P, I64, I64, c_float, P, I64, P]),
    "op_colsum": (c_int, [P, P, P, I64, P, P, P, I64, I64, c_int, c_int, P]),
    "op_geglu_bwd": (c_int, [P, P, P, P, P, I64, P]),
    "op_scale_rows": (c_int, [P, P, P, I64, P, I64, I64, P]),
    "op_l2norm_fwd": (c_int, [P, P, P, I64, I64, c_float, c_int, P]),
    "op_l2norm_bwd": (c_int, [P, P, P, P, I64, I64, c_int, P]),
    "op_infonce_rows": (c_int, [P, I64, I64, I64, I64, c_float, c_float, P, P, P, c_int, P]),
    "op_adamw_step": (c_int, [P, P, P, P, I64, c_float, c_float, c_float, c_float, c_float, I64, c_float, P, c_float, P]),
    "op_adamw_step_groups": (c_int, [P, P, P, P, I64, P, P, P, I64, c_float, c_float, c_float, c_float, I64, c_float, P, c_float, P]),
    "op_adamw_step_groups_master": (c_int, [P, P, P, P, P, I64, P, P, P, I64, c_float, c_float, c_float, c_float, I64, c_float, P,
                                           c_float, P]),
    "op_ema_step": (c_int, [P, P, I64, c_float, c_float, P]),
    "op_adamw_step_groups_ema": (c_int, [P, P, P, P, P, P, I64, P, P, P, I64, c_float, c_float, c_float, c_float, I64, c_float, P,
                                        c_float, c_float, c_float, P]),
    "op_adamw_step_shard": (c_int, [P, P, I64, I64, I64, P, P, P, P, P, P, P, I64, c_float, c_float, c_float, c_float, I64, c_float, P,
                                   c_float, c_float, c_float, P]),
    "op_sqnorm": (c_int, [P, I64, P, P, P]),
    "op_relpos_bias_build": (c_int, [P, P, I64, P, I64, I64, I64, c_int, P]),
    "op_relpos_bias_bwd": (c_int, [P, I64, I64, P, P, I64, P, I64, P, P, I64, P]),
    "op_relpos_bias_build_ids": (c_int, [P, P, I64, P, P, I64, I64, I64, I64, c_int, P]),
    "op_relpos_bias_fold_ids": (c_int, [P, P, P, I64, I64, I64, I64, I64, P]),
    "op_attn_fwd": (c_int, [P, P, P, I64, P, I64, P, P, P, I64, P, I64, I64, I64, I64, I64, I64, c_float, I64, P]),
    "op_attn_bias_frag_elems": (I64, [I64, I64]),
    "op_attn_bias_pack": (c_int, [P, P, I64, I64, I64, P]),
    "op_attn_bwd_delta": (c_int, [P, P, I64, P, I64, I64, I64, I64, P]),
    "op_attn_bwd": (c_int, [P, P, P, I64, P, P, I64, P, P, P, I64, P, P, P, P, P, P, I64, P, I64, I64, I64, I64, I64, c_float, I64, P]),
    "op_quant_fp8_rows": (c_int, [P, I64, P, I64, P, I64, I64, P]),
    "op_layernorm_fwd_q8": (c_int, [P, P, P, P, P, P, P, P, I64, I64, c_float, P]),
    "op_ln_geglu_fwd_q8": (c_int, [P, P, I64, P, P, P, P, P, P, P, I64, I64, c_float, P]),
    "op_gemm_nt_fp8": (c_int, [P, I64, P, P, P, I64, P, P, P, P, I64, P, P, P, I64, P, P, I64, I64, I64, I64, c_int, I64, P]),
    "op_rows_gather": (c_int, [P, P, P, I64, P, P, P, P, P, P, P, I64, I64, P]),
    "op_rows_merge": (c_int, [P, P, P, P, I64, P, P, P, P, P, P, P, I64, I64, P]),
    "op_rows_map": (c_int, [P, P, I64, P, P, P, P, P, P, P, I64, P]),
    "op_sim_topk_splits": (I64, [I64, I64, I64]),
    "op_sim_topk_workspace_bytes": (I64, [I64, I64, I64, I64]),
    "op_sim_topk": (c_int, [P, I64, P, I64, I64, I64, I64, I64, P, P, P, I64, I64, P]),
    "op_image_resize_normalize": (c_int, [P, I64, P, P, I64, P, I64, I64, P, P, P, c_int, P, I64, P]),
    "op_image_resize_normalize_flip": (c_int, [P, I64, P, P, I64, P, I64, I64, P, P, P, c_int, P, I64, P, P]),
    "op_mix_images": (c_int, [P, P, c_int, c_int, I64, I64, I64, I64, P, P, P, P, P]),
    "op_image_color_jitter": (c_int, [P, I64, I64, P, P, P, P, P, P]),
    "op_image_gaussian_blur": (c_int, [P, I64, I64, P, P, P, P, P, P, P]),
    "op_image_normalize_flip": (c_int, [P, I64, I64, P, P, P, c_int, P, P]),
    "op_image_randaug_layer": (c_int, [P, I64, I64, P, P, P, P, P, P, P, P]),
    "op_image_erase": (c_int, [P, c_int, I64, I64, P, P, P, P, P]),
    "op_audio_normalize_pad": (c_int, [P, I64, P, P, I64, I64, I64, P, I64, c_int, P, I64, P]),
    "op_audio_resample": (c_int, [P, I64, P, P, I64, P, I64, P, I64, P]),
    "op_average_precision_workspace_bytes": (I64, [I64, I64]),
    "op_average_precision": (c_int, [P, I64, P, I64, I64, I64, P, P, P, I64, P]),
    "op_row_loss": (c_int, [P, c_int, I64, P, c_int, I64, I64, I64, c_int, c_float, c_float, c_float, P, P, P, P, P]),
    "op_box_loss": (c_int, [P, c_int, P, I64, c_float, P, P, P]),
    "op_attn_pool_fwd": (c_int, [P, P, I64, I64, P, P, I64, P, P, I64, I64, I64, I64, P]),
    "op_attn_pool_bwd": (c_int, [P, P, P, I64, I64, P, P, P, P, I64, I64, P, I64, I64, I64, I64, P]),
    "op_token_mean_ln_fwd": (c_int, [P, I64, I64, P, P, c_float, P, P, P, P, P, I64, I64, I64, P]),
    "op_token_mean_ln_bwd": (c_int, [P, P, P, P, P, P, I64, I64, P, P, I64, I64, I64, P]),
    "op_attn_frames_fwd": (c_int, [P, P, P, I64, P, I64, I64, I64, I64, I64, I64, c_float, P]),
    "op_attn_frames_bwd": (c_int, [P, P, P, I64, P, I64, P, P, P, I64, I64, I64, I64, I64, I64, c_float, P]),
    "op_mask_patches": (c_int, [P, P, I64, I64, I64, I64, P, P, P, P, P]),
    "op_mask_words": (c_int, [P, I64, I64, I64, I64, P, I64, P, P, c_float, c_double, P, P, I64, P, P, I64, P, P]),
    "op_mask_blocks": (c_int, [P, P, P, I64, P, I64, I64, I64, P, P, I64, P]),
}


PROBE_SIGNATURES = {
    "op_last_error": (ctypes.c_char_p, []),
    "op_probe_mfma16": (c_int, [P, P, P, c_int, P]),
    "op_probe_mfma32": (c_int, [P, P, P, c_int, P]),
    "op_probe_tr16": (c_int, [P, P, P, c_int, P]),
    "op_probe_glds": (c_int, [P, P, c_int, P, P]),
    "op_probe_mfma_f8": (c_int, [P, P, P, P, P, c_int, P]),
    "op_probe_mfma_rate": (c_int, [P, P, P, c_int, c_int, P]),
    "op_probe_lds_atomic": (c_int, [P, P, c_int, c_int, c_int, P]),
    "op_probe_occupy": (c_int, [P, ctypes.c_longlong, c_int, ctypes.c_longlong, P, P]),
}


class Tuning:

    def __init__(self):
        self.reset()

    def reset(self):
        self.tile_mode = 0
        self.fullline = 2
        self.tail_rows = 1
        self.gm = 0
        self.force_splits = 0
        self.glds = 1
        self.sched = int(os.environ.get("ONEPEACE_TUNE_SCHED", "0"))
        self.fp8_small = 0
        self.merge_dbias = 1
        self.resident = 1
        self.attn_waves = 0
        self.attn_pers = 1
        self.dbias_chunks_r2 = 0
        self.dkdv_keys = 0
        self.dbias_chunks = 0
        self.attn_pers_dkdv = 1
        self.attn_lone_keys = 1
        self.attn_pers_bwd = 1

    def gemm(self):
        fl = {2: 0, 0: 1, 1: 2, 3: 3}.get(self.fullline, 0)
        tr = 0 if self.tail_rows == 1 else self.tail_rows + 1
        return (self.tile_mode | fl << 2 | tr << 4 | (self.gm & 31) << 7 | (self.force_splits & 15) << 15
                | (0 if self.glds else 1) << 19 | (self.sched & 7) << 20)

    def attn_fwd(self):
        return (0 if self.resident & 1 else 1) | ((self.resident >> 1) & 3) << 1 | (self.attn_waves & 15) << 3 | (0 if self.attn_pers else 128)

# ... 789 lines not shown
def sqnorm(x, out=None):
    if out is None:
        out = torch.empty(1, dtype=torch.float32, device=x.device)
    ws = workspace(4096, x.device, "sqnorm")
    _check(lib().op_sqnorm(ptr(x), x.numel(), ptr(ws), ptr(out), stream()), "op_sqnorm")
    return out


def relpos_bias_build(table, bucket_i32, S, Spad, transposed=False):
    heads = table.shape[1]
    out = torch.empty(heads, S, Spad, dtype=torch.bfloat16, device=table.device)
    _check(lib().op_relpos_bias_build(ptr(table), ptr(bucket_i32), bucket_i32.stride(0), ptr(out), heads, S, Spad,
                                      int(transposed), stream()), "op_relpos_bias_build")
    return out


PAIR_SEG = 32


def relpos_pairs(bucket_i32, S, num_rel):
    key = (S, num_rel, bucket_i32._version)
    cached = getattr(bucket_i32, "_op_pairs", None)
    if cached is not None and cached[0] == key:
        return cached[1]
    dev = bucket_i32.device
    vals, order = torch.sort(bucket_i32[:S, :S].reshape(-1).long(), stable=True)
    pair_off = torch.searchsorted(vals, torch.arange(num_rel + 1, device=dev))
    bucket_seg = torch.zeros(num_rel + 1, dtype=torch.int64, device=dev)
    bucket_seg[1:] = ((pair_off[1:] - pair_off[:-1] + PAIR_SEG - 1) // PAIR_SEG).cumsum(0)
    nseg = S * S // PAIR_SEG + num_rel
    t = torch.arange(nseg, device=dev)
    r = torch.searchsorted(bucket_seg[1:], t, right=True)
    rc = r.clamp(max=num_rel - 1)
    seg = torch.full((nseg + 1,), S * S, dtype=torch.int64, device=dev)
    seg[:nseg] = torch.where(r < num_rel, pair_off[rc] + (t - bucket_seg[rc]) * PAIR_SEG, S * S)
    res = (order.to(torch.int32), seg.to(torch.int32), bucket_seg.to(torch.int32), nseg)
    bucket_i32._op_pairs = (key, res)
    return res


def relpos_bias_bwd(dbias_f32, bucket_i32, num_rel, S, Spad):
    heads = dbias_f32.shape[0]
    pos, seg, bucket_seg, nseg = relpos_pairs(bucket_i32, S, num_rel)
    dtable = torch.empty(num_rel, heads, dtype=torch.float32, device=dbias_f32.device)
    partial = torch.empty(nseg, heads, dtype=torch.float32, device=dbias_f32.device)
    _check(lib().op_relpos_bias_bwd(ptr(dbias_f32), S, Spad, ptr(pos), ptr(seg), nseg, ptr(bucket_seg), num_rel, ptr(partial), ptr(dtable),
                                    heads, stream()), "op_relpos_bias_bwd")
    return dtable


def relpos_bias_build_ids(table, bucket_i32, ids_i32, Kpad, transposed=False):
    B, K = ids_i32.shape
    heads = table.shape[1]
    out = torch.empty(B, heads, K, Kpad, dtype=torch.bfloat16, device=table.device)
    _check(lib().op_relpos_bias_build_ids(ptr(table), ptr(bucket_i32), bucket_i32.stride(0), ptr(ids_i32), ptr(out), B, heads, K, Kpad,
                                          int(transposed), stream()), "op_relpos_bias_build_ids")
    return out


def relpos_bias_bwd_ids(dbias_f32, bucket_i32, ids_i32, num_rel):
    B, heads, K, Kpad = dbias_f32.shape
    Sfull = bucket_i32.shape[0]
    dense = torch.zeros(heads, Sfull, Sfull, dtype=torch.float32, device=dbias_f32.device)
    _check(lib().op_relpos_bias_fold_ids(ptr(dbias_f32), ptr(ids_i32), ptr(dense), Sfull, B, heads, K, Kpad, stream()),
           "op_relpos_bias_fold_ids")
    return relpos_bias_bwd(dense, bucket_i32, num_rel, Sfull, Sfull)


def attn_spad(S):
    return ((S + 127) // 128) * 128


def _bias_bstride(bias):
    return bias.stride(0) if bias is not None and bias.dim() == 4 else 0


def attn_bias_pack(image, S):
    n_img = image.numel() // (image.shape[-2] * image.shape[-1])
    out = torch.empty(lib().op_attn_bias_frag_elems(n_img, S), dtype=torch.bfloat16, device=image.device)
    _check(lib().op_attn_bias_pack(ptr(image), ptr(out), n_img, S, image.shape[-1], stream()), "op_attn_bias_pack")
    return out


def attn_fwd(q, k, v, ld, B, S, heads, scale, bias=None, key_pad=None, Spad=0, out=None, want_lse=True, bias_frag=None):
    dev = q.device
    H = heads * 64
    Spad = Spad or attn_spad(S)
    if out is None:
        out = torch.empty(B * S, H, dtype=torch.bfloat16, device=dev)
    lse = torch.empty(B, heads, Spad, dtype=torch.float32, device=dev) if want_lse else None
    _check(lib().op_attn_fwd(ptr(q), ptr(k), ptr(v), ld, ptr(bias), _bias_bstride(bias), ptr(bias_frag), ptr(key_pad), ptr(out), out.stride(0),
                             ptr(lse), Spad, B, S, Spad, heads, 64, scale, TUNE.attn_fwd(), stream()), "op_attn_fwd")
    return out, lse


def attn_bwd(q, k, v, ld, dout, out, lse, B, S, heads, scale, bias=None, biasT=None, key_pad=None, Spad=0, dqkv=None,
             want_dbias=False, bias_frag=None):
    dev = q.device
    H = heads * 64
    Spad = Spad or attn_spad(S)
    delta = torch.empty(B, heads, Spad, dtype=torch.float32, device=dev)
    assert out.stride(0) == dout.stride(0)
    if dqkv is None:
        dqkv = torch.empty(B * S, 3 * H, dtype=torch.bfloat16, device=dev)
    per_sample = bias is not None and bias.dim() == 4
    dbias = attn_dbias_buffer(B, S, heads, Spad, dev, per_sample) if want_dbias else None
    dq, dk, dv = dqkv[:, :H], dqkv[:, H:2 * H], dqkv[:, 2 * H:]
    attn_bwd_launch(q, k, v, ld, dout, bias, biasT, key_pad, lse, delta, dq, dk, dv, dqkv.stride(0), dbias, B, S, Spad, heads, scale,
                    bias_frag, out=out)
    if dbias is None:
        return dqkv, None
    return dqkv, (dbias if per_sample else dbias.sum(0))


def attn_bwd_launch(q, k, v, ld, dout, bias, biasT, key_pad, lse, delta, dq, dk, dv, ldg, dbias, B, S, Spad, heads, scale,
                    bias_frag=None, out=None):
    _check(lib().op_attn_bwd(ptr(q), ptr(k), ptr(v), ld, ptr(dout), ptr(out), dout.stride(0), ptr(bias), ptr(biasT), ptr(bias_frag),
                             _bias_bstride(bias),
                             ptr(key_pad), ptr(lse), ptr(delta), ptr(dq), ptr(dk), ptr(dv), ldg, ptr(dbias), B, S, Spad, heads,
                             64, scale, TUNE.attn_bwd(), stream()), "op_attn_bwd")


def attn_dbias_buffer(B, S, heads, Spad, device, per_sample=False):
    slabs = B if per_sample else lib().op_attn_bwd_dbias_slabs(B, S, heads, TUNE.attn_bwd())
    return torch.zeros(slabs, heads, S, Spad, dtype=torch.float32, device=device)


class profile_kernels:

    def __enter__(self):
        lib().op_prof_enable(1)
        return self

    def __exit__(self, *exc):
        lib().op_prof_enable(0)

    @staticmethod
    def collect(n=4):
        ms = (c_double * n)()
        cnt = (c_int64 * n)()
        work = (c_double * n)()
        lib().op_prof_collect(ms, cnt, work, n)
        return [dict(ms=ms[i], count=cnt[i], work=work[i]) for i in range(n)]


class KeptRows:

    def __init__(self, segs, lists, base, full_rows, scale, pad=256):
        n = len(segs)
        assert 1 <= n <= 4
        self.lists, self.full_rows, self.scale, self.nseg = lists, int(full_rows), float(scale), n
        self.S = [int(s[1]) for s in segs]
        self.n_samples = [int(s[2]) for s in segs]
        self.n_kept = [len(s[3]) for s in segs]
        self.src_row0 = [int(s[0]) for s in segs]
        self.dst_rows = [-(-(k * S) // pad) * pad for k, S in zip(self.n_kept, self.S)]
        self.dst_row0, self.off_kept, self.off_inv = [], [], []
        r, o = 0, int(base)
        for k, ns, dr in zip(self.n_kept, self.n_samples, self.dst_rows):
            self.dst_row0.append(r)
            self.off_kept.append(o)
            self.off_inv.append(o + k)
            r, o = r + dr, o + k + ns
        self.total, self.list_end = r, o
        arr = lambda v: (c_int64 * n)(*v)
        self._c = tuple(arr(v) for v in (self.src_row0, self.dst_row0, self.S, self.n_kept, self.dst_rows, self.n_samples))
        self._c_kept, self._c_inv = arr(self.off_kept), arr(self.off_inv)

    def kept_list(self, i):
        return self.lists[self.off_kept[i]:self.off_kept[i] + self.n_kept[i]]

    def rowmap(self):
        m = getattr(self, "_rowmap", None)
        if m is None:
            m = torch.empty(self.total, dtype=torch.int32, device=self.lists.device)
            c = self._c
            _check(lib().op_rows_map(ptr(m), ptr(self.lists), self.nseg, c[0], c[1], c[2], c[3], c[4], c[5], self._c_kept, self.total,
                                     stream()), "op_rows_map")
            self._rowmap = m
        return m


def pack_kept_lists(plans):
    out, bases = [], []
    for segs in plans:
        bases.append(len(out))
        for _, _, ns, kept in segs:
            inv = [-1] * ns
            for j, smp in enumerate(kept):
                inv[smp] = j
            out.extend(int(v) for v in kept)
            out.extend(inv)
    return torch.tensor(out if out else [0], dtype=torch.int32), bases


def rows_gather(src, kr):
    assert src.dim() == 2 and src.is_contiguous() and src.shape[0] == kr.full_rows and src.dtype == torch.bfloat16
    dst = torch.empty(kr.total, src.shape[1], dtype=src.dtype, device=src.device)
    c = kr._c
# ... 644 lines not shown
```

one-peace_amd/ops.py:

```python
import math
import os
import weakref

import torch
import torch.nn.functional as F

from . import hip

_wt_cache = {}
_cache_epoch = 0


_refresh_plan = None


def invalidate_weight_cache():
    global _cache_epoch
    _cache_epoch += 1


def refresh_weight_cache():
    global _cache_epoch, _refresh_plan
    _cache_epoch += 1
    if not FP8_FFN and (_fp8_cache or _fp8_derived_cache):
# ... 168 lines not shown
    r, cols = t.shape[0] - rows0, t.shape[1]
    key = (t.device, torch.cuda.current_stream(t.device).cuda_stream, operand, r, cols)
    buf = _tail_pads.get(key)
    if buf is None:
        if len(_tail_pads) > 64:
            _tail_pads.clear()
        buf = _tail_pads[key] = torch.zeros(64, cols, dtype=t.dtype, device=t.device)
    buf[:r].copy_(t[rows0:])
    return buf


def wgrad_tn_rows(K):
    return K - K % 64


def wgrad(dy, x, out=None, accumulate=False):
    K, M = dy.shape
    N = x.shape[1]
    K0 = wgrad_tn_rows(K)
    if K0 >= 64 and hip.gemm_tn_supported(K0, M, N, dy.stride(0), x.stride(0), out.stride(0) if out is not None else 0):
        out = hip.gemm_tn(dy[:K0], x[:K0], out, accumulate)
        if K0 != K:
            hip.gemm_tn(_tail_pad(dy, K0, 0), _tail_pad(x, K0, 1), out, True)
        return out
    if out is not None and accumulate:
        return out.add_(hip.gemm_nt(_t_pad(dy), [_t_pad(x)]))
    return hip.gemm_nt(_t_pad(dy), [_t_pad(x)], out=out)


GROUPED_WGRAD = os.environ.get("ONEPEACE_GROUPED_WGRAD", "1") != "0"
SKIP_ZERO_BACKWARD = os.environ.get("ONEPEACE_SKIP_ZERO_BACKWARD", "1") != "0"


def _live_ktiles(segs, probs, device):
    if not (SKIP_ZERO_BACKWARD and GROUPED_WGRAD) or all(q[0] is None for q in segs):
        return [None] * len(probs)
    if any(rows % 64 != 0 or rows < 64 for _, rows in probs) or len(segs) > 4 or len(probs) > 8:
        return [None] * len(probs)
    if any(ps is not None and (ps.dtype != torch.float32 or not ps.is_contiguous() or ps.numel() < B) for ps, _, _, B in segs):
        return [None] * len(probs)
    return hip.live_ktiles(segs, probs, device)


SKIP_ZERO_DGRAD = os.environ.get("ONEPEACE_SKIP_ZERO_DGRAD", "1") != "0"
_dense_dgrad_plans = {}


def _dense_dgrad_sums_k_in_one_piece(M, N, K, device):
    scratch = hip.splitk_scratch(M, N, K, hip.EPI_BIAS, device)
    ws = scratch.numel() if scratch is not None else 0
    key = (M, N, K, ws, hip.TUNE.gemm())
    if key not in _dense_dgrad_plans:
        _, splits, _, tail = hip.gemm_plan(M, N, K, hip.EPI_BIAS, False, ws)
        _dense_dgrad_plans[key] = splits == 1 and (tail == 0 or hip.gemm_plan(tail, N, K, hip.EPI_BIAS, False, ws)[1] == 1)
    return _dense_dgrad_plans[key]


def _dgrad_windows(segs, lists, outs, dense, unread=()):
    outs = list(outs) + ([] if SKIP_ZERO_ROWS else list(unread))
    every = outs + (list(unread) if SKIP_ZERO_ROWS else [])
    if not SKIP_ZERO_DGRAD or all(q[0] is None for q in segs) or len(segs) > 4 or len(lists) > 4 or len(every) > 4:
        return None
    if any(N % 256 != 0 or K % 64 != 0 or K < 128 or not _dense_dgrad_sums_k_in_one_piece(M, N, K, every[0].device) for M, N, K in dense):
        return None
    if any(ps is not None and (ps.dtype != torch.float32 or not ps.is_contiguous() or ps.numel() <= (B - 1) * st) for ps, _, _, B, st in segs):
        return None
    if any(o.dtype != torch.bfloat16 or o.stride(0) % 8 != 0 or o.shape[1] % 8 != 0 for o in every):
        return None
    return hip.live_mwindows(segs, lists, outs)


def _bwd_fills(pairs):
    pairs = [(o, skips) for o, skips in pairs if o is not None]
    return [o for o, skips in pairs if not skips], [o for o, skips in pairs if skips]


def _dgrad_listed(As, Ws, outs, windows, segs):
    return hip.gemm_nt_windows(As, Ws, outs, windows, max([sg.S for sg in segs if hip.mwindow_rule(sg.S)[1]] or [1]))


SKIP_ZERO_FWD = os.environ.get("ONEPEACE_SKIP_ZERO_FWD", "1") != "0"
_dense_fwd_plans = {}
SKIP_ZERO_ROWS = os.environ.get("ONEPEACE_SKIP_ZERO_ROWS", "1") != "0"


def _dense_fwd_sums_k_in_one_piece(M, N, K, epilogue, has_bias, device):
    scratch = hip.splitk_scratch(M, N, K, epilogue, device)
    ws = scratch.numel() if scratch is not None else 0
    key = (M, N, K, epilogue, has_bias, ws, hip.TUNE.gemm())
    if key not in _dense_fwd_plans:
        _, splits, _, tail = hip.gemm_plan(M, N, K, epilogue, has_bias, ws)
        _dense_fwd_plans[key] = splits == 1 and (tail == 0 or hip.gemm_plan(tail, N, K, epilogue, has_bias, ws)[1] == 1)
    return _dense_fwd_plans[key]


def _fwd_windows_apply(segs, nlists, nouts, dense, device, flags=True):
    if not SKIP_ZERO_FWD or not flags or all(q[0] is None for q in segs) or len(segs) > 4 or nlists > 4 or nouts > 4:
        return False
    if any(ps is not None and (ps.dtype != torch.float32 or not ps.is_contiguous() or ps.numel() <= (B - 1) * st) for ps, _, _, B, st in segs):
        return False
    if any(S * B >= 1 << 27 or row0 + S * B + 256 * 64 >= 1 << 28 for _, row0, S, B, _ in segs):
        return False
    mrs = max([q[2] for q in segs if hip.mwindow_rule(q[2])[1]] or [1])
    for M, N, K, epi, has_bias in dense:
        if N % 256 != 0 or K % 64 != 0 or K < 128 or M * max(N, K) >= 1 << 30 or mrs * max(N, K) >= 1 << 23:
            return False
        if not _dense_fwd_sums_k_in_one_piece(M, N, K, epi, has_bias, device):
            return False
    return True


class _WgradQueue:

    def __init__(self):
        self.items, self.done, self.after, self.armed, self.epoch = [], [], [], False, 0
        self.lists = []

    def reset(self):
        self.items, self.done, self.after, self.armed = [], [], [], False
        self.lists = []
        self.epoch += 1

    @staticmethod
    def _span(out):
        lo = out.data_ptr()
        return lo, lo + ((out.shape[0] - 1) * out.stride(0) + out.shape[1]) * out.element_size()

    def add(self, dy, x, out, params, side=None, after=None, ktiles=None):
        lo, hi = self._span(out)
        for it in self.items:
            l2, h2 = self._span(it[2])
            if lo < h2 and l2 < hi:
                self.flush()
                break
        self.items.append((dy, x, out, True, side))
        self.lists.append(ktiles)
        self.done.extend(params)
        if after is not None:
            self.after.append(after)
        if not self.armed:
            self.armed = True
            epoch = self.epoch
            torch.autograd.Variable._execution_engine.queue_callback(lambda: self._end_of_backward(epoch))
        if len(self.items) >= hip.TN_GROUP_MAX:
            self.flush()

    def _end_of_backward(self, epoch):
        if epoch != self.epoch:
            return
        self.armed = False
        self.flush()

    def flush(self):
        items, done, after, lists = self.items, self.done, self.after, self.lists
        self.items, self.done, self.after, self.lists = [], [], [], []
        if items:
            kw = {"ktiles": lists} if any(k is not None for k in lists) else {}
            if len(items) == 1 or not hip.gemm_tn_grouped(items, **kw):
                for dy, x, out, _, side in items:
                    if side is None:
                        hip.gemm_tn(dy, x, out, True)
                    else:
                        prod = hip.gemm_tn(dy, x, None, False)
                        W, rowdot, gamma = side
                        out.addcmul_(prod, gamma.detach().unsqueeze(1))
                        rowdot.zero_()
# ... 637 lines not shown
        if self._imageT is None:
            img = self.image.detach()
            t = torch.zeros_like(img)
            t[..., : self.S] = img[..., : self.S].transpose(2, 3)
            self._imageT = t
        return self._imageT

    def grad_accumulator(self, B):
        if self.acc is None:
            self.acc = hip.attn_dbias_buffer(B, self.S, self.heads, self.Spad, self.image.device, per_sample=True)
        return self.acc


class _DenseBiasFn(torch.autograd.Function):
    @staticmethod
    def forward(ctx, dense, handle):
        ctx.handle_ref = weakref.ref(handle)
        ctx.S = dense.shape[-1]
        B, heads, S, _ = dense.shape
        img = torch.zeros(B, heads, S, hip.attn_spad(S), dtype=dense.dtype, device=dense.device)
        img[..., :S] = dense
        return img

    @staticmethod
    def backward(ctx, _unused):
        h = ctx.handle_ref()
        if h is None or h.acc is None:
            return torch.zeros(_unused.shape[:-1] + (ctx.S,), dtype=_unused.dtype, device=_unused.device), None
        g = h.acc[..., : ctx.S].to(_unused.dtype)
        h.acc = None
        return g, None


class _RelPosImageFn(torch.autograd.Function):
    @staticmethod
    def forward(ctx, table, handle):
        ctx.handle_ref = weakref.ref(handle)
        ctx.shape = tuple(table.shape)
        if handle.ids is not None:
            return hip.relpos_bias_build_ids(table, handle.bucket, handle.ids, handle.Spad)
        return hip.relpos_bias_build(table, handle.bucket, handle.S, handle.Spad)

    @staticmethod
    def backward(ctx, _unused):
        h = ctx.handle_ref()
        if h is None or h.acc is None:
            return torch.zeros(ctx.shape, dtype=torch.bfloat16, device=_unused.device), None
        if h.ids is not None:
            dtable = hip.relpos_bias_bwd_ids(h.acc, h.bucket, h.ids, h.num_rel)
        else:
            dtable = hip.relpos_bias_bwd(h.acc.sum(0), h.bucket, h.num_rel, h.S, h.Spad)
        h.acc = None
        return dtable.to(torch.bfloat16), None


_DIRECT_WEIGHTS = ("wq", "wk", "wv", "wo", "w0", "w1", "w2")
ATTN_PARAMS = ("ln1_w", "ln1_b", "wq", "bq", "wk", "wv", "bv", "aln_w", "aln_b", "wo", "bo", "g1")
FFN_PARAMS = ("ln2_w", "ln2_b", "w0", "w1", "fln_w", "fln_b", "w2", "b2", "g2")
LAYER_PARAMS = ATTN_PARAMS + FFN_PARAMS


class StreamSeg:
    __slots__ = ("name", "B", "S", "row0", "bias", "key_pad", "pad")

    def __init__(self, name, B, S, row0, bias=None, key_pad=None, pad=0):
        self.name, self.B, self.S, self.row0, self.bias, self.key_pad, self.pad = name, B, S, row0, bias, key_pad, pad

    @property
    def tokens(self):
        return self.B * self.S

    @property
    def rows(self):
        return self.B * self.S + self.pad

    @property
    def end(self):
        return self.row0 + self.B * self.S + self.pad

    def frag(self, limit):
        return self.bias.frag if self.bias is not None and self.S <= limit else None


def _attn_forward(x2, P, segs, heads, scale, rowscale, rps, keep, want_y=True, xmap=None, out=None, listed=False):
    H = x2.shape[1]
    xln1, mean1, rstd1 = hip.layernorm_fwd(x2, P["ln1_w"], P["ln1_b"], want_stats=keep, x_rows=xmap)
    Nr = xln1.shape[0]
    full = _qkv_rows_that_fill_whole_rounds(Nr, 3 * H) if QKV_ROUND_SPLIT and H % 128 == 0 else Nr
    win, mrs, qkv, x_mid = None, 1, None, None
    if (listed and rowscale is not None and xmap is None and out is None and not (keep and want_y) and H % 256 == 0 and Nr % rps == 0
            and sum(sg.rows for sg in segs) == Nr and all(sg.S % rps == 0 and sg.row0 % rps == 0 for sg in segs)):
        wsegs = [(rowscale[sg.row0 // rps:], sg.row0, sg.S, sg.B, sg.S // rps) for sg in segs]
        dense = [(m, 3 * H, H, hip.EPI_BIAS, True) for m in ((full, Nr - full) if full < Nr else (Nr,))] + [(Nr, H, H, hip.EPI_RESID, True)]
        if _fwd_windows_apply(wsegs, 1, 2, dense, x2.device, flags=not any(sg.pad for sg in segs)):
            qkv = torch.empty(Nr, 3 * H, dtype=x2.dtype, device=x2.device)
            x_mid = torch.empty_like(x2)
            win = hip.live_mwindows_fwd(wsegs, [[(i, 0, 0) for i in range(len(segs))]], [qkv, x_mid], [None, x2])[0]
            mrs = max([sg.S for sg in segs if hip.mwindow_rule(sg.S)[1]] or [1])
    if win is not None and hip.gemm_nt_windows_fwd([xln1], [[P["wq"], P["wk"], P["wv"]]], [[P["bq"], None, P["bv"]]], [qkv], win, H,
                                                   max_row_stride=mrs):
        pass
    elif H % 128 == 0:
        if full < Nr:
            qkv = torch.empty(Nr, 3 * H, dtype=x2.dtype, device=x2.device)
            for lo, hi in ((0, full), (full, Nr)):
                hip.gemm_nt(xln1[lo:hi], [P["wq"], P["wk"], P["wv"]], [P["bq"], None, P["bv"]], n_seg=H, N=3 * H, out=qkv[lo:hi])
        else:
            qkv = hip.gemm_nt(xln1, [P["wq"], P["wk"], P["wv"]], [P["bq"], None, P["bv"]], n_seg=H, N=3 * H)
    else:
        qkv = torch.empty(xln1.shape[0], 3 * H, dtype=x2.dtype, device=x2.device)
        for i, (w, b) in enumerate(((P["wq"], P["bq"]), (P["wk"], None), (P["wv"], P["bv"]))):
            hip.gemm_nt(xln1, [w], [b] if b is not None else None, out=qkv[:, i * H:(i + 1) * H], ldc=3 * H)
    attn = torch.empty_like(xln1)
    lses = []
    for sg in segs:
        r = slice(sg.row0, sg.end)
        _, lse = hip.attn_fwd(qkv[r, :H], qkv[r, H:2 * H], qkv[r, 2 * H:], 3 * H, sg.B, sg.S, heads, scale,
                              sg.bias.image.detach() if sg.bias is not None else None, sg.key_pad, hip.attn_spad(sg.S), out=attn[r],
                              want_lse=keep, bias_frag=sg.frag(hip.ATTN_RESIDENT_MAX_S))
        lses.append(lse)
        if sg.pad:
            attn[sg.end - sg.pad:sg.end].zero_()
    if P["aln_w"] is not None:
        aln, mean_a, rstd_a = hip.layernorm_fwd(attn, P["aln_w"], P["aln_b"], want_stats=keep)
    else:
        aln, mean_a, rstd_a = attn, None, None
    y1 = torch.empty_like(xln1) if keep and want_y else None
    if win is None or not hip.gemm_nt_windows_fwd([aln], [[P["wo"]]], [[P["bo"]]], [x_mid], win, H, epilogue=hip.EPI_RESID, resids=[x2],
                                                  gammas=[P["g1"]], rowscales=[rowscale], rows_per_sample=[rps], max_row_stride=mrs):
        x_mid = hip.gemm_nt(aln, [P["wo"]], [P["bo"]], epilogue=hip.EPI_RESID, resid=x2, gamma=P["g1"], rowscale=rowscale,
                            rows_per_sample=rps, h0=y1, out=out, resid_rows=xmap)
    if not keep:
        return x_mid, None
    acts = dict(xln1=xln1, mean1=mean1, rstd1=rstd1, qkv=qkv, attn=attn, aln=aln, mean_a=mean_a, rstd_a=rstd_a, y1=y1)
    for i, lse in enumerate(lses):
        acts["lse%d" % i] = lse
    return x_mid, acts


QKV_ROUND_SPLIT = os.environ.get("ONEPEACE_QKV_ROUND_SPLIT", "1") != "0"
SKIP_ROW_TABLES = os.environ.get("ONEPEACE_SKIP_ROW_TABLES", "1") != "0"


def _row_tables(kept):
    return kept is not None and SKIP_ROW_TABLES and not FP8_FFN


def _qkv_rows_that_fill_whole_rounds(rows, n_out, cus=256, max_tail=512):
    tn, tm = (n_out + 255) // 256, (rows + 255) // 256
    rounds = -(-tm * tn // cus)
    tm_main = (rounds - 1) * cus // tn
    full = tm_main * 256
    return full if 0 < rows - full <= max_tail and tm_main > 0 else rows


GEGLU_SPLIT = os.environ.get("ONEPEACE_GEGLU_SPLIT", "1") != "0"
SEPARATE_DELTA = os.environ.get("ONEPEACE_SEPARATE_DELTA", "0") == "1"


def _geglu_split(Fd, fln_w):
    return GEGLU_SPLIT and fln_w is not None and Fd % 256 == 0


def _register_direct(ctx, names, params, needs):
    ctx.direct = tuple((n, q) for n, q, ng in zip(names, params, needs) if ng and q is not None and _direct_grad(q))
    for _, q in ctx.direct:
        q._op_pending = getattr(q, "_op_pending", 0) + 1


def _targets(direct, *names):
    if all(n in direct for n in names):
        return [direct[n].grad for n in names], True
    return [None] * len(names), False


def _finish(direct, G, names, values, accumulated):
    for n, v in zip(names, values):
        if accumulated:
            _direct_grad_done(direct[n])
        else:
            G[n] = v


def _return_grads(names, params, G, direct):
    out = []
    for n, q in zip(names, params):
        g = G.get(n) if q is not None else None
        if g is not None and n in direct:
            direct[n].grad.add_(g.view_as(direct[n].grad))
            _direct_grad_done(direct[n])
            g = None
        out.append(g)
    return out


def _resid_backward(dout, y, gamma, ps, S, gname, bname, direct, G, needs, g0=None, rows=None, fold=None, skip_zero_rows=False):
    names = tuple(n for n, present in ((gname, gamma is not None and g0 is None), (bname, True)) if present and needs.get(n))
    tgt, acc = _targets(direct, *names) if names else ([], False)
    t = dict(zip(names, tgt))
    dgamma = (t[gname] if acc else True) if gname in t else None
    dbias = (t[bname] if acc else True) if bname in t else None
    dy, dg, db = hip.resid_bwd(dout, y if dgamma is not None else None, gamma, ps, S, dgamma=dgamma, dbias=dbias, accumulate=acc, g0=g0,
                               dout_rows=rows, skip_zero_rows=skip_zero_rows)
    if fold is not None and gname in t:
        if not acc:
            fold[gname] = fold[gname] + dg.float() if gname in fold else dg.float()
        names = tuple(n for n in names if n != gname)
    _finish(direct, G, names, tuple({gname: dg, bname: db}[n] for n in names), acc)
    return dy


def _adjacent_grads(direct, names):
    if not all(n in direct for n in names):
        return None
    order = sorted(names, key=lambda n: direct[n].grad.data_ptr())
    for a, b in zip(order, order[1:]):
        ga, gb = direct[a].grad, direct[b].grad
        if not ga.is_contiguous() or ga.data_ptr() + ga.numel() * ga.element_size() != gb.data_ptr() or ga.shape[1:] != gb.shape[1:]:
            return None
    return order


def _span(direct, order):
    g0 = direct[order[0]].grad
    return torch.as_strided(g0, (sum(direct[n].grad.shape[0] for n in order), g0.shape[1]), (g0.shape[1], 1))


def _weight_grad_fn(ctx, G):
    direct = dict(ctx.direct)

    def weight_grad(name, dyv, xv, side=None, after=None, ktiles=None):
        target = direct.get(name)
        if target is not None:
            wgrad_into(dyv, xv, target.grad, (target,), side, after, ktiles)
        else:
            assert side is None and after is None
            G[name] = wgrad(dyv, xv)
    return weight_grad, direct


def _gamma_finish_hook(rowdot, gamma_param, pairs, done):
    def run():
        hip.gamma_grad_finish(rowdot, pairs, gamma_param.grad, True)
        if done:
            _direct_grad_done(gamma_param)
    return run


def _save(ctx, keep, acts, *tensors):
    if keep:
        ctx.act_names = [k for k, v in acts.items() if v is not None]
        ctx.save_for_backward(*tensors, *[acts[k] for k in ctx.act_names])
    else:
        ctx.act_names = None
        ctx.save_for_backward(*tensors)


def _restore(ctx, saved_acts, optional):
    A = dict(zip(ctx.act_names, saved_acts))
    for k in optional:
        A.setdefault(k, None)
    return A


class AttnBranchFn(torch.autograd.Function):

    @staticmethod
    def forward(ctx, x2, segs, rowscale, rps, heads, save_acts, kept, *rest):
        nseg = len(segs)
        params = rest[nseg:]
        P = dict(zip(ATTN_PARAMS, params))
        need_grad = any(ctx.needs_input_grad) and bool(int(save_acts) & 2)
        keep = bool(int(save_acts) & 1) and need_grad
        first_param = 7 + nseg
        needs = dict(zip(ATTN_PARAMS, ctx.needs_input_grad[first_param:]))
        x_full = x2
        mapped = _row_tables(kept)
        if kept is not None and not mapped:
            x2 = hip.rows_gather(x_full, kept)
        H = x2.shape[1]
        N = kept.total if mapped else x2.shape[0]
        scale = (H // heads) ** -0.5
        ctx.dg_fused = need_grad and dgamma_from_wgrad_ok([N], P["g1"], [P["wo"]], [P["bo"]], needs["g1"], [needs["wo"]])
        if mapped:
            x_mid = torch.empty_like(x_full)
            _, acts = _attn_forward(x_full, P, segs, heads, scale, rowscale, rps, keep, want_y=needs["g1"] and not ctx.dg_fused,
                                    xmap=kept.rowmap(), out=x_mid)
            hip.rows_merge(x_full, None, kept, out=x_mid)
        else:
            x_mid, acts = _attn_forward(x2, P, segs, heads, scale, rowscale, rps, keep, want_y=needs["g1"] and not ctx.dg_fused,
                                        listed=kept is None and ctx.dg_fused)
            if kept is not None:
                x_mid = hip.rows_merge(x_full, x_mid, kept)
        ctx.kept, ctx.mapped = kept, mapped
        ctx.segs, ctx.dims, ctx.n_params, ctx.first_param = segs, (N, H, heads, scale, rps), len(params), first_param
        ctx.direct = ()
        if need_grad:
            _register_direct(ctx, ATTN_PARAMS, params, ctx.needs_input_grad[first_param:])
        if keep:
            if not needs["wo"]:
                acts["aln"] = None if P["aln_w"] is not None else acts["aln"]
            if not (needs["wq"] or needs["wk"] or needs["wv"]):
                acts["xln1"] = None
        ctx.cheap = keep and bool(int(save_acts) & 4)
        if ctx.cheap:
            acts["xln1"] = None
            if P["aln_w"] is not None:
                acts["aln"] = None
        _save(ctx, keep, acts, x2, rowscale, *params)
        return x_mid

    @staticmethod
    def backward(ctx, dx_mid):
        x2, rowscale, *rest = ctx.saved_tensors
        params, saved_acts = rest[:ctx.n_params], rest[ctx.n_params:]
        N, H, heads, scale, rps = ctx.dims
        segs = ctx.segs
        nseg = len(segs)
        P = dict(zip(ATTN_PARAMS, params))
        needs = {n: bool(ng) and q is not None for n, q, ng in zip(ATTN_PARAMS, params, ctx.needs_input_grad[ctx.first_param:])}
        need_x = bool(ctx.needs_input_grad[0])
        want_dbias = [sg.bias is not None and sg.bias.image.requires_grad for sg in segs]
        kept, mapped = ctx.kept, ctx.mapped
        xmap = kept.rowmap() if mapped else None
        if ctx.act_names is not None:
            A = _restore(ctx, saved_acts, ("mean_a", "rstd_a", "y1", "xln1", "aln"))
            if ctx.cheap:
                if needs["wq"] or needs["wk"] or needs["wv"]:
                    A["xln1"] = hip.layernorm_fwd(x2, P["ln1_w"], P["ln1_b"], x_rows=xmap)[0]
                if needs["wo"] and P["aln_w"] is not None:
                    A["aln"] = hip.layernorm_fwd(A["attn"], P["aln_w"], P["aln_b"])[0]
        else:
            _, A = _attn_forward(x2, P, segs, heads, scale, rowscale, rps, True, want_y=not ctx.dg_fused, xmap=xmap,
                                 out=torch.empty_like(x2) if mapped else None, listed=kept is None and ctx.dg_fused)
        if not dx_mid.is_contiguous():
            dx_mid = dx_mid.contiguous()
        dx_full = dx_mid
        if kept is not None and not mapped:
            dx_mid = hip.rows_gather(dx_full, kept)
        G = {}
        weight_grad, direct = _weight_grad_fn(ctx, G)
        kt1 = None
        whole = rowscale is not None and kept is None and N % rps == 0 and not any(sg.pad for sg in segs) and sum(sg.rows for sg in segs) == N
        if whole:
            kt1 = _live_ktiles([(rowscale, 0, rps, N // rps)], [(0, N)], dx_mid.device)[0]
        upstream = ("ln1_w", "ln1_b", "wq", "bq", "wk", "wv", "bv", "aln_w", "aln_b")
        need_up = need_x or any(want_dbias) or any(needs[n] for n in upstream)
        need_dxln1 = need_x or needs["ln1_w"] or needs["ln1_b"]
        win1, daln, dxln1 = None, None, None
        if need_up and whole and all(sg.S % rps == 0 and sg.row0 % rps == 0 for sg in segs):
            daln = torch.empty(N, H, dtype=dx_mid.dtype, device=dx_mid.device)
            dxln1 = torch.empty_like(daln) if need_dxln1 else None
            filled, unread = _bwd_fills([(daln, P["aln_w"] is not None), (dxln1, True)])
            win1 = _dgrad_windows([(rowscale[sg.row0 // rps:], sg.row0, sg.S, sg.B, sg.S // rps) for sg in segs],
                                  [[(i, 0, 0) for i in range(nseg)]], filled,
                                  [(N, H, H)] + ([(N, H, 3 * H)] if need_dxln1 else []), unread=unread)
        zr_b = SKIP_ZERO_ROWS and win1 is not None
        if ctx.dg_fused:
            g0 = torch.empty(H, dtype=torch.float32, device=dx_mid.device)
            dy1 = _resid_backward(dx_mid, None, P["g1"], rowscale, rps, "g1", "bo", direct, G, needs, g0=g0, rows=xmap, skip_zero_rows=zr_b)
            rowdot, (rd_wo,) = _rowdot_slots(dx_mid.device, [P["wo"]])
            weight_grad("wo", dy1, A["aln"], side=(P["wo"], rd_wo, P["g1"]),
                        after=_gamma_finish_hook(rowdot, direct["g1"], [(P["bo"], g0)] if P["bo"] is not None else [], True), ktiles=kt1)
            wo_t = _transposed(P["wo"], scale=P["g1"])
        else:
            dy1 = _resid_backward(dx_mid, A["y1"], P["g1"], rowscale, rps, "g1", "bo", direct, G, needs, rows=xmap, skip_zero_rows=zr_b)
            if needs["wo"]:
                weight_grad("wo", dy1, A["aln"], ktiles=kt1)
            wo_t = None
        dx = None
        if need_up:
            wo_in = wo_t if wo_t is not None else _transposed(P["wo"])
            if win1 is None or not _dgrad_listed([dy1], [wo_in], [daln], win1[0], segs):
                daln = hip.gemm_nt(dy1, [wo_in])
            if P["aln_w"] is not None:
                want = needs["aln_w"] or needs["aln_b"]
                (tw, tb), acc = _targets(direct, "aln_w", "aln_b") if want else ((None, None), False)
                dattn, dw_, db_ = hip.layernorm_bwd(daln, A["attn"], P["aln_w"], P["aln_b"], A["mean_a"], A["rstd_a"], dw=tw, db=tb,
                                                    accumulate=acc, need_wgrad=want, ps=rowscale if zr_b else None, rows_per_sample=rps)
                if want:
                    _finish(direct, G, ("aln_w", "aln_b"), (dw_, db_), acc)
            else:
                dattn = daln
            qkv_names = ("wq", "wk", "wv")
            order = _adjacent_grads(direct, qkv_names) if all(needs[n] for n in qkv_names) and H % 8 == 0 else None
            cols = tuple(order) if order else qkv_names
            slot = {n: i for i, n in enumerate(cols)}
            qkv = A["qkv"]
            dqkv = torch.empty_like(qkv)
            for i, sg in enumerate(segs):
                r = slice(sg.row0, sg.end)
                if sg.pad:
                    dqkv[sg.end - sg.pad:sg.end].zero_()
                dparts = {n: dqkv[r, slot[n] * H:(slot[n] + 1) * H] for n in qkv_names}
                _attn_backward(qkv[r], dattn[r], A["attn"][r], A["lse%d" % i], sg.B, sg.S, heads, scale,
                               sg.bias.image.detach() if sg.bias is not None else None, sg.bias.imageT if sg.bias is not None else None,
                               sg.key_pad, sg.bias.grad_accumulator(sg.B) if want_dbias[i] else None, sg.frag(384),
                               dparts["wq"], dparts["wk"], dparts["wv"])
            bias_of = {"wq": "bq", "wv": "bv"}
            bnames = tuple(bias_of[n] for n in cols if n in bias_of and needs[bias_of[n]])
            if bnames:
                tgt, acc = _targets(direct, *bnames)
                if H % 8 == 0:
                    outs = [None, None, None]
                    for n, t_ in zip(bnames, tgt):
                        outs[slot["wq" if n == "bq" else "wv"]] = t_ if acc else torch.empty(H, dtype=dqkv.dtype, device=dqkv.device)
                    hip.colsum_segments(dqkv, H, outs, accumulate=acc)
                    _finish(direct, G, bnames, tuple(outs[slot["wq" if n == "bq" else "wv"]] for n in bnames), acc)
                else:
                    sums = hip.colsum(dqkv)
                    for n in bnames:
                        i = slot["wq" if n == "bq" else "wv"]
                        G[n] = sums[i * H:(i + 1) * H]
            if order:
                wgrad_into(dqkv, A["xln1"], _span(direct, order), [direct[n] for n in order], ktiles=kt1)
            elif any(n in direct for n in qkv_names) or not all(needs[n] for n in qkv_names):
                for n in qkv_names:
                    if needs[n]:
                        weight_grad(n, dqkv[:, slot[n] * H:(slot[n] + 1) * H], A["xln1"], ktiles=kt1)
            else:
                dW = wgrad(dqkv, A["xln1"])
                G["wq"], G["wk"], G["wv"] = dW[:H], dW[H:2 * H], dW[2 * H:]
            if need_dxln1:
                wqkv_t = _transposed(tuple(P[n] for n in cols))
                if win1 is None or not _dgrad_listed([dqkv], [wqkv_t], [dxln1], win1[0], segs):
                    dxln1 = hip.gemm_nt(dqkv, [wqkv_t])
                want = needs["ln1_w"] or needs["ln1_b"]
                (tw, tb), acc = _targets(direct, "ln1_w", "ln1_b") if want else ((None, None), False)
                dx, dw_, db_ = hip.layernorm_bwd(dxln1, x2, P["ln1_w"], P["ln1_b"], A["mean1"], A["rstd1"], add=dx_mid, dw=tw, db=tb,
                                                 accumulate=acc, need_wgrad=want, dx=torch.empty_like(dx_full) if mapped else None,
                                                 x_rows=xmap, ps=rowscale if zr_b else None, rows_per_sample=rps)
                if want:
                    _finish(direct, G, ("ln1_w", "ln1_b"), (dw_, db_), acc)
        if dx is None and need_x:
            dx = dx_full
        elif dx is not None and mapped:
            hip.rows_merge(dx_full, None, kept, out=dx)
        elif dx is not None and kept is not None:
            dx = hip.rows_merge(dx_full, dx, kept)
        flush_wgrads()
        grads = _return_grads(ATTN_PARAMS, params, G, direct)
        dimgs = []
        for sg, w in zip(segs, want_dbias):
            if w and not getattr(sg.bias, "_grad_routed", False):
                sg.bias._grad_routed = True
                img = sg.bias.image
                dimgs.append(torch.zeros((), dtype=img.dtype, device=img.device).expand(img.shape))
            else:
                dimgs.append(None)
        return (dx, None, None, None, None, None, None, *dimgs, *grads)


FFN_SHARED = ("ln2_w", "ln2_b", "g2")
FFN_OWN = ("w0", "w1", "fln_w", "fln_b", "w2", "b2")


class FfnBranchMultiFn(torch.autograd.Function):

    @staticmethod
    def _compute(x2, segs, pss, params, keep, want_y, grad=None, xmap=None, listed=False, info=None):
        nseg = len(segs)
        shared = dict(zip(FFN_SHARED, params[:3]))
        own = [dict(zip(FFN_OWN, params[3 + 6 * i:9 + 6 * i])) for i in range(nseg)]
        H = x2.shape[1]
        N = xmap.numel() if xmap is not None else x2.shape[0]
        Fd = own[0]["w0"].shape[0]
        dev, dt = x2.device, x2.dtype
        has_fln = own[0]["fln_w"] is not None
        split = (keep if grad is None else grad) and _geglu_split(Fd, own[0]["fln_w"])
        fp8 = FP8_FFN and H % 128 == 0 and Fd % 128 == 0
        gq = None
        if fp8 and split:
            xln2, mean2, rstd2, (xq, xs) = hip.layernorm_fwd(x2, shared["ln2_w"], shared["ln2_b"], want_stats=keep, q8=True)
            gq, gs = torch.empty(N, Fd, dtype=torch.uint8, device=dev), torch.empty(N, dtype=torch.float32, device=dev)
        else:
            xln2, mean2, rstd2 = hip.layernorm_fwd(x2, shared["ln2_w"], shared["ln2_b"], want_stats=keep, x_rows=xmap)
            if fp8:
                xq, xs = hip.quant_fp8_rows(xln2)
        if split:
            hh = torch.empty(N, 2 * Fd, dtype=dt, device=dev)
            g, h0, h1 = None, hh[:, :Fd], hh[:, Fd:]
# ... 208 lines not shown
            pair = (k("w0"), k("w1"))
            order = _adjacent_grads(direct, pair) if needs[pair[0]] and needs[pair[1]] and Fd % 8 == 0 else None
            cols = tuple(order) if order else pair
            colsets.append(cols)
            dpart = {n: dh[r, j * Fd:(j + 1) * Fd] for j, n in enumerate(cols)}
            if has_fln:
                want = needs[k("fln_w")] or needs[k("fln_b")]
                (tw, tb2), acc = _targets(direct, k("fln_w"), k("fln_b")) if want else ((None, None), False)
                _, _, dw_, db2_ = hip.ln_geglu_bwd(dgln[r], A["h0"][r], A["h1"][r], P[k("fln_w")], A["mean_f"][r], A["rstd_f"][r], dw=tw,
                                                   db=tb2, accumulate=acc, need_wgrad=want, dh0=dpart[pair[0]], dh1=dpart[pair[1]],
                                                   ps=pss[i] if zr_b or ctx.zero_rows else None, rows_per_sample=sg.S)
                if want:
                    _finish(direct, G, (k("fln_w"), k("fln_b")), (dw_, db2_), acc)
            else:
                d0, d1 = hip.geglu_bwd(dgln[r], A["h0"][r], A["h1"][r])
                dpart[pair[0]].copy_(d0)
                dpart[pair[1]].copy_(d1)
            if order:
                wgrad_into(dh[r], A["xln2"][r], _span(direct, order), [direct[n] for n in order], ktiles=kts[i])
            else:
                for n in pair:
                    if needs[n]:
                        weight_grad(n, dpart[n], A["xln2"][r], ktiles=kts[i])
        if fold is not None and needs["g2"] and not fused:
            if "g2" in fold:
                G["g2"] = fold["g2"].to(dt)
            else:
                _direct_grad_done(direct["g2"])
        dx = None
        if need_dxln2:
            if dxln2 is None:
                dxln2 = torch.empty(N, H, dtype=dt, device=dev)
            rs = [slice(sg.row0, sg.end) for sg in segs]
            wts = [_transposed(tuple(P[n] for n in cols)) for cols in colsets]
            if fp8b:
                for r, wt in zip(rs, wts):
                    hip.gemm_nt_fp8(*hip.quant_fp8_rows(dh[r]), *[[x] for x in _fp8_derived(wt)], out=dxln2[r])
            elif wins is not None and _dgrad_listed([dh[r] for r in rs], wts, [dxln2[r] for r in rs], wins[nseg], segs):
                pass
            elif nseg == 1 or hip.gemm_nt_grouped([dh[r] for r in rs], wts, outs=[dxln2[r] for r in rs]) is None:
                for r, wt in zip(rs, wts):
                    hip.gemm_nt(dh[r], [wt], out=dxln2[r])
            want = needs["ln2_w"] or needs["ln2_b"]
            (tw, tb), acc = _targets(direct, "ln2_w", "ln2_b") if want else ((None, None), False)
            dx, dw_, db_ = hip.layernorm_bwd(dxln2, x2, P["ln2_w"], P["ln2_b"], A["mean2"], A["rstd2"], add=dout, dw=tw, db=tb,
                                             accumulate=acc, need_wgrad=want, dx=torch.empty_like(dout_full) if mapped else None, x_rows=xmap,
                                             ps=pss[0] if zr_b and ln2_one else None, rows_per_sample=segs[0].S)
            if want:
                _finish(direct, G, ("ln2_w", "ln2_b"), (dw_, db_), acc)
        if dx is None and need_x:
            dx = dout_full
        elif dx is not None and mapped:
            hip.rows_merge(dout_full, None, kept, out=dx)
        elif dx is not None and kept is not None:
            dx = hip.rows_merge(dout_full, dx, kept)
        grads = _return_grads(names, params, G, direct)
        return (dx, None, None, None, None, *grads)


def ffn_branch_multi(x2, segs, pss, shared, own, save_acts=True, kept=None):
    flat = list(shared)
    for o in own:
        flat += list(o)
    return FfnBranchMultiFn.apply(x2, segs, tuple(pss), _save_flags(save_acts), kept, *flat)


_SCALE_ROWS = {}


def kept_segments(kept, segs, device):
    out = []
    for i, sg in enumerate(segs):
        key_pad = sg.key_pad.index_select(0, kept.kept_list(i)) if sg.key_pad is not None else None
        out.append(StreamSeg(sg.name, kept.n_kept[i], sg.S, kept.dst_row0[i], sg.bias, key_pad, pad=kept.dst_rows[i] - kept.n_kept[i] * sg.S))
    key = (device, kept.scale)
    vec = _SCALE_ROWS.get(key)
    if vec is None or vec.numel() < kept.total + 8:
        if len(_SCALE_ROWS) > 256:
            _SCALE_ROWS.clear()
        vec = _SCALE_ROWS[key] = torch.full((max(kept.full_rows, kept.total) + 8,), kept.scale, dtype=torch.float32, device=device)
    return out, vec


def _attn_backward(qkv, dattn, attn, lse, B, S, heads, scale, bias_img, biasT, key_pad, dbias_acc, bias_frag, dq, dk, dv):
    H = heads * 64
    dev = qkv.device
    Spad = hip.attn_spad(S)
    delta = torch.empty(B, heads, Spad, dtype=torch.float32, device=dev)
    if attn.stride(0) != dattn.stride(0) or SEPARATE_DELTA:
        hip._check(hip.lib().op_attn_bwd_delta(hip.ptr(dattn), hip.ptr(attn), dattn.stride(0), hip.ptr(delta), B, S, Spad, heads,
                                               hip.stream()), "op_attn_bwd_delta")
        attn = None
    hip.attn_bwd_launch(qkv[:, :H], qkv[:, H:2 * H], qkv[:, 2 * H:], 3 * H, dattn, bias_img, biasT, key_pad, lse, delta, dq, dk,
                        dv, dq.stride(0), dbias_acc, B, S, Spad, heads, scale, bias_frag, out=attn)


def attn_branch(x, bias, key_pad, ps, heads, params, save_acts=False):
    B, S, H = x.shape
    seg = StreamSeg("x", B, S, 0, bias, key_pad)
    out = AttnBranchFn.apply(x.reshape(B * S, H), [seg], ps, S, heads, _save_flags(save_acts), None, bias.image if bias is not None else None, *params)
    return out.view(B, S, H)


def attn_branch_multi(x2, segs, ps_rows, heads, params, save_acts=False, kept=None):
    return AttnBranchFn.apply(x2, segs, ps_rows, 1, heads, _save_flags(save_acts), kept,
                              *[sg.bias.image if sg.bias is not None else None for sg in segs], *params)


def _save_flags(save_acts):
    return int(bool(save_acts)) | (2 if torch.is_grad_enabled() else 0) | (4 if RECOMPUTE_CHEAP and save_acts else 0)


def ffn_branch(x, ps, params, save_acts=False):
    B, S, H = x.shape
    P = dict(zip(FFN_PARAMS, params))
    out = ffn_branch_multi(x.reshape(B * S, H), [StreamSeg("x", B, S, 0)], [ps], [P[n] for n in FFN_SHARED], [[P[n] for n in FFN_OWN]],
                           save_acts)
    return out.view(B, S, H)


class L2NormalizeFn(torch.autograd.Function):

    @staticmethod
    def forward(ctx, x):
        y, inv = hip.l2norm_fwd(x.contiguous())
        ctx.save_for_backward(y, inv)
        return y

    @staticmethod
    def backward(ctx, dy):
        y, inv = ctx.saved_tensors
        return hip.l2norm_bwd(dy.contiguous(), y, inv)


def l2_normalize(x):
    return L2NormalizeFn.apply(x)


class InfoNCEFn(torch.autograd.Function):

    @staticmethod
    def forward(ctx, a_local, b_local, a_all, b_all, scale, rank, label_smoothing):
        b = a_local.shape[0]
        t0 = rank * b
        scale_f = scale.detach().float().reshape(1)
        sims, rows = [], []
        for loc, allv in ((a_local, b_all), (b_local, a_all)):
            sim = gemm_any(loc.detach(), allv.detach(), out_f32=True, alpha=scale_f)
            loss_r, hit_r, dot_r = hip.infonce_rows(sim, t0, label_smoothing, gscale=0.5 / b, write_grad=True)
            sims.append(sim)
            rows.append((loss_r, hit_r, dot_r))
        loss = 0.5 * (rows[0][0].mean() + rows[1][0].mean())
        ctx.save_for_backward(a_local, b_local, a_all, b_all, scale_f, sims[0], sims[1], rows[0][2], rows[1][2])
        ctx.scale_dtype = scale.dtype
        hits_a, hits_b = rows[0][1].sum(), rows[1][1].sum()
        ctx.mark_non_differentiable(hits_a, hits_b)
        return loss, hits_a, hits_b

    @staticmethod
    def backward(ctx, gl, _ga, _gb):
        a_local, b_local, a_all, b_all, scale_f, ds_ab, ds_ba, dot_ab, dot_ba = ctx.saved_tensors
        g = gl.float()
        coef = (g * scale_f).reshape(1)
        da = gemm_any(ds_ab.to(torch.bfloat16), hip.transpose(b_all.contiguous()), out_f32=True, alpha=coef)
        db = gemm_any(ds_ba.to(torch.bfloat16), hip.transpose(a_all.contiguous()), out_f32=True, alpha=coef)
        dscale = (g * (dot_ab.sum() + dot_ba.sum()) / scale_f).reshape(()).to(ctx.scale_dtype)
        return da.to(a_local.dtype), db.to(b_local.dtype), None, None, dscale, None, None


def info_nce(a_local, b_local, a_all, b_all, scale, rank=0, label_smoothing=0.0):
    return InfoNCEFn.apply(a_local, b_local, a_all, b_all, scale, rank, label_smoothing)


class DclFn(torch.autograd.Function):

    @staticmethod
    def forward(ctx, student, teacher, scale, label_smoothing, block):
# ... 516 lines not shown
```

Baseline: 210.0.

## Skip attention work for dropped samples via on-device live-sample lists

```diff
diff --git a/include/onepeace_hip.h b/include/onepeace_hip.h
--- a/include/onepeace_hip.h
+++ b/include/onepeace_hip.h
@@ -101,6 +101,16 @@
                 const float* lse, float* delta, void* dq,
                 void* dk, void* dv, int64_t ldg, float* dbias, int64_t B, int64_t S, int64_t Spad, int64_t heads,
                 int64_t head_dim, float scale, int64_t tune, void* stream);
+int op_live_samples(const float* ps, int64_t ps_stride, int64_t B, int64_t S, int64_t heads, int32_t* list, void* fill, int64_t fill_ld,
+                    int64_t fill_cols, void* stream);
+int op_attn_fwd_kept(const void* q, const void* k, const void* v, int64_t ld, const void* bias, int64_t bias_batch_stride,
+                     const void* bias_frag, const void* key_pad, void* out, int64_t ldo, float* lse, int64_t lse_ld, int64_t B,
+                     int64_t S, int64_t Spad, int64_t heads, int64_t head_dim, float scale, const int32_t* kept, int64_t tune, void* stream);
+int op_attn_bwd_kept(const void* q, const void* k, const void* v, int64_t ld, const void* dout, const void* out, int64_t ldo,
+                     const void* bias, const void* biasT, const void* bias_frag, int64_t bias_batch_stride, const void* key_pad,
+                     const float* lse, float* delta, void* dq,
+                     void* dk, void* dv, int64_t ldg, float* dbias, int64_t B, int64_t S, int64_t Spad, int64_t heads,
+                     int64_t head_dim, float scale, const int32_t* kept, int64_t tune, void* stream);
 
 int op_relpos_bias_build(const void* table, const int* bucket, int64_t bucket_ld, void* out, int64_t heads, int64_t S,
                          int64_t Spad, int transposed, void* stream);
diff --git a/one-peace_amd/csrc/attention.hip b/one-peace_amd/csrc/attention.hip
--- a/one-peace_amd/csrc/attention.hip
+++ b/one-peace_amd/csrc/attention.hip
@@ -472,10 +472,27 @@
   asm volatile("s_nop 4\n\tglobal_load_dword %0, %1, %2 offset:%3" : "=v"(d) : "v"(voff), "s"(sbase), "n"(OFF));
 }
 
-template <bool HAS_BIAS, bool HAS_PAD>
+__device__ __forceinline__ int attn_sload(const int* addr) {
+  int v;
+  asm volatile("s_nop 4\n\ts_load_dword %0, %1, 0x0\n\ts_waitcnt lgkmcnt(0)" : "=&s"(v) : "s"(addr) : "memory");
+  return v;
+}
+template <bool LIST>
+__device__ __forceinline__ int attn_list_item(const int* list, int pos, int heads) {
+  if constexpr (LIST) {
+    const int i = pos / heads;
+    return attn_sload(list + 1 + i) * heads + (pos - i * heads);
+  } else {
+    return pos;
+  }
+}
+
+template <bool HAS_BIAS, bool HAS_PAD, bool LIST>
 __global__ __launch_bounds__(PERS_NW * 64, 2) void attn_fwd_pers_kernel(AttnArgs p, const bf16_t* __restrict__ bias_frag, int rows_pad,
-                                                                         int nitems) {
+                                                                         int nitems_arg, const int* __restrict__ list) {
   extern __shared__ __attribute__((aligned(16))) char smem[];
+  int nitems = nitems_arg;
+  if constexpr (LIST) nitems = attn_sload(list);
   const int tid = threadIdx.x, lane = tid & 63;
   const int wid = __builtin_amdgcn_readfirstlane(tid >> 6);
   const int g = lane >> 4, t = lane & 15;
@@ -583,10 +600,11 @@
   int item = blockIdx.x;
   const int step = gridDim.x;
   if (item < nitems) {
-    for (int j = 0; j < npiece; ++j) piece(item, 0, j);
-    load_q(item, qi_main[0], qn[0]);
-    load_q(item, qi_main[1], qn[1]);
-    small_loads(item, 0);
+    const int it0 = attn_list_item<LIST>(list, item, p.heads);
+    for (int j = 0; j < npiece; ++j) piece(it0, 0, j);
+    load_q(it0, qi_main[0], qn[0]);
+    load_q(it0, qi_main[1], qn[1]);
+    small_loads(it0, 0);
   }
   int buf = 0, prev_item = -1;
   auto wait_all = [&]() {
@@ -614,14 +632,19 @@
   };
 
   for (; item < nitems; item += step, buf ^= 1) {
-    const int b = item / p.heads, h = item - b * p.heads;
+    const int cur = attn_list_item<LIST>(list, item, p.heads);
+    const int b = cur / p.heads, h = cur - b * p.heads;
     const int64_t row_base = (int64_t)b * p.S;
     __syncthreads();
     bf16x8 qf[2][2] = {{qn[0][0], qn[0][1]}, {qn[1][0], qn[1][1]}};
     const bool more = item + step < nitems;
-    const int nxt = more ? item + step : item;
-    if (has_left && prev_item >= 0 && wid == ((prev_item / step) & (PERS_NW - 1))) merge_left(prev_item, buf ^ 1);
-    prev_item = item;
+    const int nxt = attn_list_item<LIST>(list, more ? item + step : item, p.heads);
+    if constexpr (LIST) {
+      if (has_left && prev_item >= 0 && wid == ((item / step - 1) & (PERS_NW - 1))) merge_left(prev_item, buf ^ 1);
+    } else {
+      if (has_left && prev_item >= 0 && wid == ((prev_item / step) & (PERS_NW - 1))) merge_left(prev_item, buf ^ 1);
+    }
+    prev_item = cur;
 
     const char* ldsK = smem + buf * KVB;
     const char* ldsV = ldsK + rows_pad * 128;
@@ -651,9 +674,9 @@
       }
       __builtin_amdgcn_sched_barrier(0);
       if constexpr (FULL) {
-        small_loads(item, kt + 1);
+        small_loads(cur, kt + 1);
       } else {
-        late_loads(nxt, item);
+        late_loads(nxt, cur);
         small_loads(nxt, 0);
       }
       __builtin_amdgcn_sched_barrier(0);
@@ -1596,8 +1619,8 @@
   }
 }
 
-template <bool HAS_BIAS, bool HAS_PAD, int NT, int LASTB, bool LEFT>
-__device__ __forceinline__ void attn_bwd_dq_pers_body(const AttnBwdArgs& p, char* smem, int rows_pad, int nqh, int qhalf0) {
+template <bool HAS_BIAS, bool HAS_PAD, int NT, int LASTB, bool LEFT, bool LIST>
+__device__ __forceinline__ void attn_bwd_dq_pers_body(const AttnBwdArgs& p, char* smem, int rows_pad, int nqh, int qhalf0, const int* list) {
   const int tid = threadIdx.x, lane = tid & 63;
   const int wid = __builtin_amdgcn_readfirstlane(tid >> 6);
   const int g = lane >> 4, t = lane & 15;
@@ -1605,8 +1628,17 @@
   float* scratch = reinterpret_cast<float*>(smem + 2 * KVB);
   const int nqb = (p.S + 15) >> 4, nkp = (p.S + 31) >> 5;
   const int qhalf = qhalf0, h = (blockIdx.x / nqh) % p.heads, chunk = blockIdx.x / (nqh * p.heads);
-  const int b_begin = chunk * p.bchunk, b_end = min(p.B, b_begin + p.bchunk);
+  int b_begin = chunk * p.bchunk, b_end = min(p.B, b_begin + p.bchunk);
   if (b_begin >= b_end) return;
+  if constexpr (LIST) {
+    b_begin = attn_sload(list + 1 + p.B + b_begin);
+    b_end = attn_sload(list + 1 + p.B + b_end);
+    if (b_begin >= b_end) return;
+  }
+  auto sample_at = [&](int pos) {
+    if constexpr (LIST) return attn_sload(list + 1 + pos);
+    else return pos;
+  };
   const int qblk = qhalf * PERS_NW + wid;
   const bool active = qblk < min(nqb, 2 * PERS_NW);
   constexpr bool has_left = LEFT;
@@ -1716,9 +1748,12 @@
 #pragma unroll
     for (int j = 0; j < 2; ++j) accl[i][j] = (f32x4){0.f, 0.f, 0.f, 0.f};
 
-  for (int j = 0; j < npiece; ++j) piece(b_begin, 0, j);
-  query_loads(b_begin, vo_q, vo_o, vo_lse, qn, don, oon, lsen);
-  small_loads(b_begin, 0);
+  {
+    const int b0 = sample_at(b_begin);
+    for (int j = 0; j < npiece; ++j) piece(b0, 0, j);
+    query_loads(b0, vo_q, vo_o, vo_lse, qn, don, oon, lsen);
+    small_loads(b0, 0);
+  }
   int buf = 0, prev_b = -1;
   auto merge_left = [&](int b, int sb) {
     const float* sc = scratch + sb * (PERS_NW * 64);
@@ -1733,14 +1768,19 @@
                  "+v"(padn[0]), "+v"(padn[1]), "+v"(padn[2]), "+v"(padn[3]) : : "memory");
   };
   wait_all();
-  for (int b = b_begin; b < b_end; ++b, buf ^= 1) {
+  for (int pos = b_begin; pos < b_end; ++pos, buf ^= 1) {
+    const int b = sample_at(pos);
     __syncthreads();
     const bf16x8 qf[2] = {qn[0], qn[1]}, dof[2] = {don[0], don[1]};
     const float dl = delta_from_frags(dof, oon);
     const float nl2 = -lsen * LOG2E;
     if (active && g == 0 && q0w + t < p.S) p.delta_w[((int64_t)b * p.heads + h) * p.Spad + q0w + t] = dl;
-    const int nxt = b + 1 < b_end ? b + 1 : b;
-    if (has_left && prev_b >= 0 && wid == (prev_b & (PERS_NW - 1))) merge_left(prev_b, buf ^ 1);
+    const int nxt = sample_at(pos + 1 < b_end ? pos + 1 : pos);
+    if constexpr (LIST) {
+      if (has_left && prev_b >= 0 && wid == ((pos - 1) & (PERS_NW - 1))) merge_left(prev_b, buf ^ 1);
+    } else {
+      if (has_left && prev_b >= 0 && wid == (prev_b & (PERS_NW - 1))) merge_left(prev_b, buf ^ 1);
+    }
     prev_b = b;
     const char* ldsK = smem + buf * KVB;
     const char* ldsV = ldsK + rows_pad * 128;
@@ -1965,18 +2005,18 @@
   }
 }
 
-template <bool HAS_BIAS, bool HAS_PAD, int NT, int LASTB>
-__global__ __launch_bounds__(PERS_NW * 64, 2) void attn_bwd_dq_pers_kernel(AttnBwdArgs p, int rows_pad, int nqh) {
+template <bool HAS_BIAS, bool HAS_PAD, int NT, int LASTB, bool LIST>
+__global__ __launch_bounds__(PERS_NW * 64, 2) void attn_bwd_dq_pers_kernel(AttnBwdArgs p, int rows_pad, int nqh, const int* __restrict__ list) {
   extern __shared__ __attribute__((aligned(16))) char smem[];
   const int qhalf = blockIdx.x % nqh;
   const bool lone = ((p.S + 15) >> 4) > 2 * PERS_NW && qhalf == nqh - 1;
   if constexpr (NT == 5) {
     if (lone) {
-      attn_bwd_dq_pers_body<HAS_BIAS, HAS_PAD, NT, LASTB, true>(p, smem, rows_pad, nqh, qhalf);
+      attn_bwd_dq_pers_body<HAS_BIAS, HAS_PAD, NT, LASTB, true, LIST>(p, smem, rows_pad, nqh, qhalf, list);
       return;
     }
   }
-  attn_bwd_dq_pers_body<HAS_BIAS, HAS_PAD, NT, LASTB, false>(p, smem, rows_pad, nqh, qhalf);
+  attn_bwd_dq_pers_body<HAS_BIAS, HAS_PAD, NT, LASTB, false, LIST>(p, smem, rows_pad, nqh, qhalf, list);
 }
 
 constexpr int PERS_SCRL = 136;
@@ -1995,9 +2035,12 @@
   asm volatile("s_nop 4\n\tbuffer_store_dwordx2 %0, %1, %2, 0 offen\n\ts_nop 1" ::"v"(data), "v"(voff), "s"(rsrc) : "memory");
 }
 
-template <bool HAS_BIAS, bool HAS_PAD, int NT, bool LONE>
-__global__ __launch_bounds__(PERS_NW * 64, 2) void attn_bwd_dkdv_pers_kernel(AttnBwdArgs p, int rows_pad, int nitems) {
+template <bool HAS_BIAS, bool HAS_PAD, int NT, bool LONE, bool LIST>
+__global__ __launch_bounds__(PERS_NW * 64, 2) void attn_bwd_dkdv_pers_kernel(AttnBwdArgs p, int rows_pad, int nitems_arg,
+                                                                              const int* __restrict__ list) {
   extern __shared__ __attribute__((aligned(16))) char smem[];
+  int nitems = nitems_arg;
+  if constexpr (LIST) nitems = attn_sload(list);
   const int tid = threadIdx.x, lane = tid & 63;
   const int wid = __builtin_amdgcn_readfirstlane(tid >> 6);
   const int g = lane >> 4, t = lane & 15;
@@ -2110,11 +2153,12 @@
   using I0 = std::integral_constant<int, 0>;
   using I1 = std::integral_constant<int, 1>;
   if (item < nitems) {
-    for (int j = 0; j < npiece; ++j) piece(item, 0, j);
-    if constexpr (LONE) kv_loads(item, kf, vf);
-    else kv_loads(item, kn, vn);
-    bias_loads(item, I0{}, I0{});
-    bias_loads(item, I0{}, I1{});
+    const int it0 = attn_list_item<LIST>(list, item, p.heads);
+    for (int j = 0; j < npiece; ++j) piece(it0, 0, j);
+    if constexpr (LONE) kv_loads(it0, kf, vf);
+    else kv_loads(it0, kn, vn);
+    bias_loads(it0, I0{}, I0{});
+    bias_loads(it0, I0{}, I1{});
   }
 #define DKDV_WAIT_LOADS(NST)                                                                                                                  \
   do {                                                                                                                                     \
@@ -2142,7 +2186,8 @@
   };
 
   for (; item < nitems; item += step, buf ^= 1) {
-    const int b = item / p.heads, h = item - b * p.heads;
+    const int cur = attn_list_item<LIST>(list, item, p.heads);
+    const int b = cur / p.heads, h = cur - b * p.heads;
     asm volatile("s_waitcnt lgkmcnt(0)" ::: "memory");
     __builtin_amdgcn_s_barrier();
     asm volatile("" ::: "memory");
@@ -2154,9 +2199,13 @@
     }
     const bool kdead[2] = {HAS_PAD && kdn[0] != 0u, HAS_PAD && kdn[1] != 0u};
     const bool ldead = HAS_PAD && LONE && kdl != 0u;
-    const int nxt = item + step < nitems ? item + step : item;
-    if (LONE && prev_item >= 0 && wid == ((prev_item / step) & (PERS_NW - 1))) merge_lone(prev_item, buf ^ 1);
-    prev_item = item;
+    const int nxt = attn_list_item<LIST>(list, item + step < nitems ? item + step : item, p.heads);
+    if constexpr (LIST) {
+      if (LONE && prev_item >= 0 && wid == ((item / step - 1) & (PERS_NW - 1))) merge_lone(prev_item, buf ^ 1);
+    } else {
+      if (LONE && prev_item >= 0 && wid == ((prev_item / step) & (PERS_NW - 1))) merge_lone(prev_item, buf ^ 1);
+    }
+    prev_item = cur;
     const char* ldsQ = smem + buf * BUFB;
     const char* ldsO = ldsQ + QBY;
     const float* ldsL = reinterpret_cast<const float*>(ldsQ + 2 * QBY);
@@ -2282,7 +2331,7 @@
       __builtin_amdgcn_sched_barrier(0);
       if (wave_active) half(QT * 64, std::integral_constant<int, 2>{}, kf, vf, bn[0], dvT, dkT);
       __builtin_amdgcn_sched_barrier(0);
-      if constexpr (!LAST) bias_loads(item, QN{}, I0{});
+      if constexpr (!LAST) bias_loads(cur, QN{}, I0{});
       if constexpr (HAS_BIAS && QT > 0) {
         if constexpr (!LAST) asm volatile("s_waitcnt vmcnt(%2)" : "+v"(bn[1][0]), "+v"(bn[1][1]) : "n"(BPPT + NBH));
         else asm volatile("s_waitcnt vmcnt(0)" : "+v"(bn[1][0]), "+v"(bn[1][1]));
@@ -2291,10 +2340,10 @@
       if (wave_active && QT * 64 + 32 < p.S) half(QT * 64 + 32, std::integral_constant<int, 2>{}, kf, vf, bn[1], dvT, dkT);
       __builtin_amdgcn_sched_barrier(0);
       if constexpr (!LAST) {
-        bias_loads(item, QN{}, I1{});
+        bias_loads(cur, QN{}, I1{});
         if constexpr (HAS_BIAS) asm volatile("s_waitcnt vmcnt(%2)" : "+v"(bn[0][0]), "+v"(bn[0][1]) : "n"(NBH));
       } else {
-        lone_bias_loads(item);
+        lone_bias_loads(cur);
         bias_loads(nxt, I0{}, I0{});
         bias_loads(nxt, I0{}, I1{});
         if constexpr (!LONE) kv_loads(nxt, kn, vn);
@@ -2477,6 +2526,47 @@
   }
 }
 
+constexpr int LS_SPLIT = 64;
+__global__ __launch_bounds__(256) void live_samples_kernel(const float* __restrict__ ps, int64_t ps_stride, int B, int heads,
+                                                           int* __restrict__ list, bf16_t* __restrict__ fill, int64_t fill_ld, int fill_cols,
+                                                           int S) {
+  const int tid = threadIdx.x, lane = tid & 63, wid = tid >> 6;
+  if (blockIdx.x == 0 && blockIdx.y == 0) {
+    __shared__ int wsum[4];
+    int base = 0;
+    for (int b0 = 0; b0 < B; b0 += 256) {
+      const int b = b0 + tid;
+      const bool keep = b < B && ps[(int64_t)b * ps_stride] != 0.f;
+      const unsigned long long m = __ballot(keep);
+      if (lane == 0) wsum[wid] = __popcll(m);
+      __syncthreads();
+      int below = base + __popcll(m & ((1ull << lane) - 1ull)), total = 0;
+#pragma unroll
+      for (int w = 0; w < 4; ++w) {
+        below += w < wid ? wsum[w] : 0;
+        total += wsum[w];
+      }
+      if (b < B) list[1 + B + b] = below;
+      if (keep) list[1 + below] = b;
+      base += total;
+      __syncthreads();
+    }
+    if (tid == 0) {
+      list[0] = base * heads;
+      list[1 + B + B] = base;
+    }
+  }
+  const int b = blockIdx.x;
+  if (fill == nullptr || ps[(int64_t)b * ps_stride] != 0.f) return;
+  const int cpr = fill_cols >> 3;
+  const int total = S * cpr;
+  bf16_t* rows = fill + (int64_t)b * S * fill_ld;
+  for (int i = blockIdx.y * 256 + tid; i < total; i += LS_SPLIT * 256) {
+    const int r = i / cpr, c = i - r * cpr;
+    *reinterpret_cast<uint4*>(rows + (int64_t)r * fill_ld + c * 8) = make_uint4(0u, 0u, 0u, 0u);
+  }
+}
+
 enum : int64_t {
   FWD_STREAMING = 1 << 0, FWD_ABLATE_SHIFT = 1, FWD_ABLATE_MASK = 3, FWD_WAVES_SHIFT = 3, FWD_WAVES_MASK = 15, FWD_NO_PERS = 1 << 7,
   BWD_SEPARATE_DBIAS = 1 << 0, BWD_ROUND2_CHUNKS = 1 << 1, BWD_DKDV_KEYS_SHIFT = 2, BWD_DKDV_KEYS_MASK = 3, BWD_CHUNKS_SHIFT = 4,
@@ -2551,9 +2641,9 @@
   return n;
 }
 
-int op_attn_fwd(const void* q, const void* k, const void* v, int64_t ld, const void* bias, int64_t bias_batch_stride,
-                const void* bias_frag, const void* key_pad, void* out, int64_t ldo, float* lse, int64_t lse_ld, int64_t B,
-                int64_t S, int64_t Spad, int64_t heads, int64_t head_dim, float scale, int64_t tune, void* stream) {
+static int attn_fwd_impl(const void* q, const void* k, const void* v, int64_t ld, const void* bias, int64_t bias_batch_stride,
+                         const void* bias_frag, const void* key_pad, void* out, int64_t ldo, float* lse, int64_t lse_ld, int64_t B,
+                         int64_t S, int64_t Spad, int64_t heads, int64_t head_dim, float scale, const int* kept, int64_t tune, void* stream) {
   OP_CHECK_ARG(q && k && v && out, "attn_fwd: null pointer");
   OP_CHECK_ARG(head_dim == HD, "attn_fwd: head_dim %lld unsupported (only 64)", (long long)head_dim);
   OP_CHECK_ARG(B > 0 && S > 0 && heads > 0 && ld % 8 == 0 && ldo % 4 == 0, "attn_fwd: bad sizes");
@@ -2569,16 +2659,23 @@
   hipStream_t s = (hipStream_t)stream;
   const bool inv_exact = (float)(bf16_t)(1.0f / scale) * scale == 1.0f;
   const bf16_t* fr = (const bf16_t*)bias_frag;
-  if (!(tune & FWD_STREAMING) && !(tune & FWD_NO_PERS) && S > 192 && S <= 257 && (!bias || (bias_frag && inv_exact))) {
+  const bool pers = !(tune & FWD_STREAMING) && !(tune & FWD_NO_PERS) && S > 192 && S <= 257 && (!bias || (bias_frag && inv_exact));
+  if (kept && !(pers && a.bias_bs == 0)) {
+    op_prof_end(slot, stream);
+    OP_CHECK_ARG(false, "attn_fwd_kept: only the persistent kernel takes a list (193 ... 257 tokens, a shared fragment-major bias image or none)");
+  }
+  if (pers) {
     const int rows_pad = ceil_div(S, 32) * 32;
     const size_t sh = (size_t)4 * rows_pad * 128 + 2 * PERS_NW * PERS_SCR * 4;
     const int nitems = (int)(B * heads);
     const int nwg = min(nitems, op_num_cus());
     return attn_launched(with_bias_pad(bias, key_pad, [&](auto hb, auto hp) {
-      constexpr auto kern = attn_fwd_pers_kernel<decltype(hb)::value, decltype(hp)::value>;
-      OP_ENSURE_LDS(kern, 4 * PERS_MAX_ROWS * 128 + 2 * PERS_NW * PERS_SCR * 4, "attn_fwd");
-      hipLaunchKernelGGL(kern, dim3(nwg), dim3(PERS_NW * 64), sh, s, a, fr, rows_pad, nitems);
-      return OP_OK;
+      return op_with_bool(kept != nullptr, [&](auto ls) {
+        constexpr auto kern = attn_fwd_pers_kernel<decltype(hb)::value, decltype(hp)::value, decltype(ls)::value>;
+        OP_ENSURE_LDS(kern, 4 * PERS_MAX_ROWS * 128 + 2 * PERS_NW * PERS_SCR * 4, "attn_fwd");
+        hipLaunchKernelGGL(kern, dim3(nwg), dim3(PERS_NW * 64), sh, s, a, fr, rows_pad, nitems, kept);
+        return OP_OK;
+      });
     }), slot, stream);
   }
   if (!(tune & FWD_STREAMING) && S <= RES_MAX_S && (!bias || (bias_frag && inv_exact))) {
@@ -2606,6 +2703,34 @@
   }), slot, stream);
 }
 
+int op_attn_fwd(const void* q, const void* k, const void* v, int64_t ld, const void* bias, int64_t bias_batch_stride,
+                const void* bias_frag, const void* key_pad, void* out, int64_t ldo, float* lse, int64_t lse_ld, int64_t B,
+                int64_t S, int64_t Spad, int64_t heads, int64_t head_dim, float scale, int64_t tune, void* stream) {
+  return attn_fwd_impl(q, k, v, ld, bias, bias_batch_stride, bias_frag, key_pad, out, ldo, lse, lse_ld, B, S, Spad, heads, head_dim, scale,
+                       nullptr, tune, stream);
+}
+
+int op_live_samples(const float* ps, int64_t ps_stride, int64_t B, int64_t S, int64_t heads, int* list, void* fill, int64_t fill_ld,
+                    int64_t fill_cols, void* stream) {
+  OP_CHECK_ARG(ps && list && ps_stride >= 0, "live_samples: null pointer or negative stride");
+  OP_CHECK_ARG(B > 0 && S > 0 && heads > 0 && B <= 65535 && B * heads < ((int64_t)1 << 30) && S < ((int64_t)1 << 20), "live_samples: bad sizes");
+  OP_CHECK_ARG(!fill || (((uintptr_t)fill & 15) == 0 && fill_ld % 8 == 0 && fill_cols % 8 == 0 && fill_cols > 0 && fill_cols <= fill_ld &&
+                         S * (fill_cols / 8) < ((int64_t)1 << 31)),
+               "live_samples: rows to fill must be 16-byte aligned with ld and cols multiples of 8, cols <= ld");
+  hipLaunchKernelGGL(live_samples_kernel, dim3((unsigned)B, LS_SPLIT), dim3(256), 0, (hipStream_t)stream, ps, ps_stride, (int)B, (int)heads,
+                     list, (bf16_t*)fill, fill_ld, (int)fill_cols, (int)S);
+  OP_LAUNCH_CHECK();
+  return OP_OK;
+}
+
+int op_attn_fwd_kept(const void* q, const void* k, const void* v, int64_t ld, const void* bias, int64_t bias_batch_stride,
+                     const void* bias_frag, const void* key_pad, void* out, int64_t ldo, float* lse, int64_t lse_ld, int64_t B,
+                     int64_t S, int64_t Spad, int64_t heads, int64_t head_dim, float scale, const int* kept, int64_t tune, void* stream) {
+  OP_CHECK_ARG(kept, "attn_fwd_kept: null list");
+  return attn_fwd_impl(q, k, v, ld, bias, bias_batch_stride, bias_frag, key_pad, out, ldo, lse, lse_ld, B, S, Spad, heads, head_dim, scale,
+                       kept, tune, stream);
+}
+
 
 int64_t op_attn_bias_frag_elems(int64_t n_img, int64_t S) {
   return n_img * (int64_t)ceil_div(S, 16) * ceil_div(S, 32) * FRAG_BLOCK;
@@ -2631,11 +2756,11 @@
   return OP_OK;
 }
 
-int op_attn_bwd(const void* q, const void* k, const void* v, int64_t ld, const void* dout, const void* out, int64_t ldo, const void* bias,
-                const void* biasT, const void* bias_frag, int64_t bias_batch_stride, const void* key_pad, const float* lse,
-                float* delta, void* dq,
-                void* dk, void* dv, int64_t ldg, float* dbias, int64_t B, int64_t S, int64_t Spad, int64_t heads,
-                int64_t head_dim, float scale, int64_t tune, void* stream) {
+static int attn_bwd_impl(const void* q, const void* k, const void* v, int64_t ld, const void* dout, const void* out, int64_t ldo, const void* bias,
+                         const void* biasT, const void* bias_frag, int64_t bias_batch_stride, const void* key_pad, const float* lse,
+                         float* delta, void* dq,
+                         void* dk, void* dv, int64_t ldg, float* dbias, int64_t B, int64_t S, int64_t Spad, int64_t heads,
+                         int64_t head_dim, float scale, const int* kept, int64_t tune, void* stream) {
   const bool merge_dbias = !(tune & BWD_SEPARATE_DBIAS);
   OP_CHECK_ARG(q && k && v && dout && lse && delta && dq && dk && dv, "attn_bwd: null pointer");
   OP_CHECK_ARG(head_dim == HD, "attn_bwd: head_dim %lld unsupported (only 64)", (long long)head_dim);
@@ -2671,13 +2796,16 @@
       });
     }), sl, stream);
   };
+  const bool pers_dq = merge_dbias && !(tune & BWD_NO_PERS_DQ) && out && pers_bwd_shape(S) && a.bias_bs == 0 &&
+                       (!bias || (a.bias_frag != nullptr && (float)(bf16_t)(1.0f / scale) * scale == 1.0f));
+  OP_CHECK_ARG(!kept || (pers_dq && !(tune & BWD_NO_PERS_DKDV) && (!bias || biasT)),
+               "attn_bwd_kept: only the persistent kernels take a list (193 ... 257 tokens, `out` given, a shared fragment-major bias image or none)");
   if (!out) {
     const int rc = launch_dkdv();
     if (rc != OP_OK) return rc;
   }
   const int nt = ceil_div(S, BKV);
-  if (merge_dbias && !(tune & BWD_NO_PERS_DQ) && out && pers_bwd_shape(S) && a.bias_bs == 0 &&
-      (!bias || (a.bias_frag != nullptr && (float)(bf16_t)(1.0f / scale) * scale == 1.0f))) {
+  if (pers_dq) {
     const int nqb = ceil_div(S, 16);
     const int nqh = ceil_div(min(nqb, 2 * PERS_NW), PERS_NW);
     const int chunks = pers_bwd_chunks(B, S, heads);
@@ -2691,24 +2819,28 @@
     int rc = attn_launched(with_bias_pad(bias, key_pad, [&](auto hb, auto hp) {
       return op_with_bool(S > 256, [&](auto lone) {
         constexpr bool LONE = decltype(lone)::value;
-        constexpr auto kern = attn_bwd_dq_pers_kernel<decltype(hb)::value, decltype(hp)::value, LONE ? 5 : 4, LONE ? 1 : 4>;
-        OP_ENSURE_LDS(kern, 4 * PERS_MAX_ROWS * 128 + 2 * PERS_NW * 64 * 4, "attn_bwd");
-        hipLaunchKernelGGL(kern, dim3(nwg), dim3(PERS_NW * 64), sh, s, d, rows_pad, nqh);
-        return OP_OK;
+        return op_with_bool(kept != nullptr, [&](auto ls) {
+          constexpr auto kern = attn_bwd_dq_pers_kernel<decltype(hb)::value, decltype(hp)::value, LONE ? 5 : 4, LONE ? 1 : 4, decltype(ls)::value>;
+          OP_ENSURE_LDS(kern, 4 * PERS_MAX_ROWS * 128 + 2 * PERS_NW * 64 * 4, "attn_bwd");
+          hipLaunchKernelGGL(kern, dim3(nwg), dim3(PERS_NW * 64), sh, s, d, rows_pad, nqh, kept);
+          return OP_OK;
+        });
       });
     }), slot, stream);
     if (rc != OP_OK) return rc;
     a.bchunk = bchunk_dkdv;
-    if ((tune & BWD_NO_PERS_DKDV) || (bias && !biasT) || (S == 256 && !(tune & BWD_PERS_DKDV_256))) return launch_dkdv();
+    if ((tune & BWD_NO_PERS_DKDV) || (bias && !biasT) || (S == 256 && !(tune & BWD_PERS_DKDV_256) && !kept)) return launch_dkdv();
     const int dk_rows = dkdv_pers_rows(S), nitems = a.B * a.heads, dk_nwg = min(nitems, op_num_cus());
     const int dk_slot = op_prof_begin(2, 2.0 * fl, stream);
     return attn_launched(with_bias_pad(bias, key_pad, [&](auto hb, auto hp) {
       return op_with_bool(S > 256, [&](auto lone) {
         constexpr bool LONE = decltype(lone)::value;
-        constexpr auto kern = attn_bwd_dkdv_pers_kernel<decltype(hb)::value, decltype(hp)::value, LONE ? 5 : 4, LONE>;
-        OP_ENSURE_LDS(kern, (int)dkdv_pers_lds(LONE ? 257 : 256), "attn_bwd");
-        hipLaunchKernelGGL(kern, dim3(dk_nwg), dim3(PERS_NW * 64), dkdv_pers_lds(S), s, a, dk_rows, nitems);
-        return OP_OK;
+        return op_with_bool(kept != nullptr, [&](auto ls) {
+          constexpr auto kern = attn_bwd_dkdv_pers_kernel<decltype(hb)::value, decltype(hp)::value, LONE ? 5 : 4, LONE, decltype(ls)::value>;
+          OP_ENSURE_LDS(kern, (int)dkdv_pers_lds(LONE ? 257 : 256), "attn_bwd");
+          hipLaunchKernelGGL(kern, dim3(dk_nwg), dim3(PERS_NW * 64), dkdv_pers_lds(S), s, a, dk_rows, nitems, kept);
+          return OP_OK;
+        });
       });
     }), dk_slot, stream);
   }
@@ -2748,4 +2880,23 @@
   return OP_OK;
 }
 
-}
+int op_attn_bwd(const void* q, const void* k, const void* v, int64_t ld, const void* dout, const void* out, int64_t ldo, const void* bias,
+                const void* biasT, const void* bias_frag, int64_t bias_batch_stride, const void* key_pad, const float* lse,
+                float* delta, void* dq,
+                void* dk, void* dv, int64_t ldg, float* dbias, int64_t B, int64_t S, int64_t Spad, int64_t heads,
+                int64_t head_dim, float scale, int64_t tune, void* stream) {
+  return attn_bwd_impl(q, k, v, ld, dout, out, ldo, bias, biasT, bias_frag, bias_batch_stride, key_pad, lse, delta, dq, dk, dv, ldg, dbias, B, S,
+                       Spad, heads, head_dim, scale, nullptr, tune, stream);
+}
+
+int op_attn_bwd_kept(const void* q, const void* k, const void* v, int64_t ld, const void* dout, const void* out, int64_t ldo, const void* bias,
+                     const void* biasT, const void* bias_frag, int64_t bias_batch_stride, const void* key_pad, const float* lse,
+                     float* delta, void* dq,
+                     void* dk, void* dv, int64_t ldg, float* dbias, int64_t B, int64_t S, int64_t Spad, int64_t heads,
+                     int64_t head_dim, float scale, const int* kept, int64_t tune, void* stream) {
+  OP_CHECK_ARG(kept, "attn_bwd_kept: null list");
+  return attn_bwd_impl(q, k, v, ld, dout, out, ldo, bias, biasT, bias_frag, bias_batch_stride, key_pad, lse, delta, dq, dk, dv, ldg, dbias, B, S,
+                       Spad, heads, head_dim, scale, kept, tune, stream);
+}
+
+}
diff --git a/one-peace_amd/hip.py b/one-peace_amd/hip.py
--- a/one-peace_amd/hip.py
+++ b/one-peace_amd/hip.py
@@ -85,6 +85,9 @@
     "op_attn_bias_pack": (c_int, [P, P, I64, I64, I64, P]),
     "op_attn_bwd_delta": (c_int, [P, P, I64, P, I64, I64, I64, I64, P]),
     "op_attn_bwd": (c_int, [P, P, P, I64, P, P, I64, P, P, P, I64, P, P, P, P, P, P, I64, P, I64, I64, I64, I64, I64, c_float, I64, P]),
+    "op_live_samples": (c_int, [P, I64, I64, I64, I64, P, P, I64, I64, P]),
+    "op_attn_fwd_kept": (c_int, [P, P, P, I64, P, I64, P, P, P, I64, P, I64, I64, I64, I64, I64, I64, c_float, P, I64, P]),
+    "op_attn_bwd_kept": (c_int, [P, P, P, I64, P, P, I64, P, P, P, I64, P, P, P, P, P, P, I64, P, I64, I64, I64, I64, I64, c_float, P, I64, P]),
     "op_quant_fp8_rows": (c_int, [P, I64, P, I64, P, I64, I64, P]),
     "op_layernorm_fwd_q8": (c_int, [P, P, P, P, P, P, P, P, I64, I64, c_float, P]),
     "op_ln_geglu_fwd_q8": (c_int, [P, P, I64, P, P, P, P, P, P, P, I64, I64, c_float, P]),
@@ -1040,13 +1043,47 @@
     return out
 
 
-def attn_fwd(q, k, v, ld, B, S, heads, scale, bias=None, key_pad=None, Spad=0, out=None, want_lse=True, bias_frag=None):
+_INV_EXACT = {}
+
+
+def _inv_scale_exact(scale):
+    if scale not in _INV_EXACT:
+        s32 = torch.tensor(scale, dtype=torch.float32)
+        _INV_EXACT[scale] = bool(((1.0 / s32).to(torch.bfloat16).to(torch.float32) * s32) == 1.0)
+    return _INV_EXACT[scale]
+
+
+def attn_kept_shape(S, heads, scale, bias, bias_frag):
+    if not (192 < S <= 257) or TUNE.attn_fwd() != 0 or TUNE.attn_bwd() != 0:
+        return False
+    if bias is None:
+        return True
+    return bias.dim() == 3 and bias_frag is not None and _inv_scale_exact(float(scale))
+
+
+def live_samples(ps, ps_stride, B, S, heads, fill=None, cols=None):
+    assert ps.dtype == torch.float32 and ps.is_contiguous() and ps.numel() > (B - 1) * ps_stride
+    lst = torch.empty(2 * B + 2, dtype=torch.int32, device=ps.device)
+    if fill is not None:
+        assert fill.dtype == torch.bfloat16 and fill.stride(1) == 1 and fill.shape[0] >= B * S
+        cols = fill.shape[1] if cols is None else cols
+    _check(lib().op_live_samples(ptr(ps), ps_stride, B, S, heads, ptr(lst), ptr(fill), fill.stride(0) if fill is not None else 0,
+                                 cols or 0, stream()), "op_live_samples")
+    return lst
+
+
+def attn_fwd(q, k, v, ld, B, S, heads, scale, bias=None, key_pad=None, Spad=0, out=None, want_lse=True, bias_frag=None, kept=None):
     dev = q.device
     H = heads * 64
     Spad = Spad or attn_spad(S)
     if out is None:
         out = torch.empty(B * S, H, dtype=torch.bfloat16, device=dev)
     lse = torch.empty(B, heads, Spad, dtype=torch.float32, device=dev) if want_lse else None
+    if kept is not None:
+        _check(lib().op_attn_fwd_kept(ptr(q), ptr(k), ptr(v), ld, ptr(bias), _bias_bstride(bias), ptr(bias_frag), ptr(key_pad), ptr(out),
+                                      out.stride(0), ptr(lse), Spad, B, S, Spad, heads, 64, scale, ptr(kept), TUNE.attn_fwd(), stream()),
+               "op_attn_fwd_kept")
+        return out, lse
     _check(lib().op_attn_fwd(ptr(q), ptr(k), ptr(v), ld, ptr(bias), _bias_bstride(bias), ptr(bias_frag), ptr(key_pad), ptr(out), out.stride(0),
                              ptr(lse), Spad, B, S, Spad, heads, 64, scale, TUNE.attn_fwd(), stream()), "op_attn_fwd")
     return out, lse
@@ -1072,7 +1109,13 @@
 
 
 def attn_bwd_launch(q, k, v, ld, dout, bias, biasT, key_pad, lse, delta, dq, dk, dv, ldg, dbias, B, S, Spad, heads, scale,
-                    bias_frag=None, out=None):
+                    bias_frag=None, out=None, kept=None):
+    if kept is not None:
+        _check(lib().op_attn_bwd_kept(ptr(q), ptr(k), ptr(v), ld, ptr(dout), ptr(out), dout.stride(0), ptr(bias), ptr(biasT), ptr(bias_frag),
+                                      _bias_bstride(bias),
+                                      ptr(key_pad), ptr(lse), ptr(delta), ptr(dq), ptr(dk), ptr(dv), ldg, ptr(dbias), B, S, Spad, heads,
+                                      64, scale, ptr(kept), TUNE.attn_bwd(), stream()), "op_attn_bwd_kept")
+        return
     _check(lib().op_attn_bwd(ptr(q), ptr(k), ptr(v), ld, ptr(dout), ptr(out), dout.stride(0), ptr(bias), ptr(biasT), ptr(bias_frag),
                              _bias_bstride(bias),
                              ptr(key_pad), ptr(lse), ptr(delta), ptr(dq), ptr(dk), ptr(dv), ldg, ptr(dbias), B, S, Spad, heads,
diff --git a/one-peace_amd/ops.py b/one-peace_amd/ops.py
--- a/one-peace_amd/ops.py
+++ b/one-peace_amd/ops.py
@@ -274,6 +274,7 @@
 SKIP_ZERO_FWD = os.environ.get("ONEPEACE_SKIP_ZERO_FWD", "1") != "0"
 _dense_fwd_plans = {}
 SKIP_ZERO_ROWS = os.environ.get("ONEPEACE_SKIP_ZERO_ROWS", "1") != "0"
+SKIP_ZERO_ATTN = os.environ.get("ONEPEACE_SKIP_ZERO_ATTN", "1") != "0"
 
 
 def _dense_fwd_sums_k_in_one_piece(M, N, K, epilogue, has_bias, device):
@@ -1077,12 +1078,20 @@
         return self.bias.frag if self.bias is not None and self.S <= limit else None
 
 
-def _attn_forward(x2, P, segs, heads, scale, rowscale, rps, keep, want_y=True, xmap=None, out=None, listed=False):
+def _attn_list_applies(sg, heads, scale, H):
+    if sg.S == 256:
+        return False
+    return bool(SKIP_ZERO_ATTN and not SEPARATE_DELTA and not sg.pad and H == heads * 64 and sg.B > 0 and
+                hip.attn_kept_shape(sg.S, heads, scale, sg.bias.image if sg.bias is not None else None,
+                                    sg.frag(hip.ATTN_RESIDENT_MAX_S)))
+
+
+def _attn_forward(x2, P, segs, heads, scale, rowscale, rps, keep, want_y=True, xmap=None, out=None, listed=False, info=None):
     H = x2.shape[1]
     xln1, mean1, rstd1 = hip.layernorm_fwd(x2, P["ln1_w"], P["ln1_b"], want_stats=keep, x_rows=xmap)
     Nr = xln1.shape[0]
     full = _qkv_rows_that_fill_whole_rounds(Nr, 3 * H) if QKV_ROUND_SPLIT and H % 128 == 0 else Nr
-    win, mrs, qkv, x_mid = None, 1, None, None
+    win, mrs, qkv, x_mid, attn, attn_list, wsegs = None, 1, None, None, None, [False] * len(segs), None
     if (listed and rowscale is not None and xmap is None and out is None and not (keep and want_y) and H % 256 == 0 and Nr % rps == 0
             and sum(sg.rows for sg in segs) == Nr and all(sg.S % rps == 0 and sg.row0 % rps == 0 for sg in segs)):
         wsegs = [(rowscale[sg.row0 // rps:], sg.row0, sg.S, sg.B, sg.S // rps) for sg in segs]
@@ -1090,7 +1099,15 @@
         if _fwd_windows_apply(wsegs, 1, 2, dense, x2.device, flags=not any(sg.pad for sg in segs)):
             qkv = torch.empty(Nr, 3 * H, dtype=x2.dtype, device=x2.device)
             x_mid = torch.empty_like(x2)
-            win = hip.live_mwindows_fwd(wsegs, [[(i, 0, 0) for i in range(len(segs))]], [qkv, x_mid], [None, x2])[0]
+            attn_list = [_attn_list_applies(sg, heads, scale, H) for sg in segs]
+            if any(attn_list):
+                attn = torch.empty_like(xln1)
+                win = hip.live_mwindows_fwd(wsegs, [[(i, 0, 0) for i in range(len(segs))]], [attn, x_mid], [None, x2])[0]
+                for sg, ls, ws in zip(segs, attn_list, wsegs):
+                    if not ls:
+                        hip.live_samples(ws[0], ws[4], sg.B, sg.S, heads, fill=qkv[sg.row0:sg.end])
+            else:
+                win = hip.live_mwindows_fwd(wsegs, [[(i, 0, 0) for i in range(len(segs))]], [qkv, x_mid], [None, x2])[0]
             mrs = max([sg.S for sg in segs if hip.mwindow_rule(sg.S)[1]] or [1])
     if win is not None and hip.gemm_nt_windows_fwd([xln1], [[P["wq"], P["wk"], P["wv"]]], [[P["bq"], None, P["bv"]]], [qkv], win, H,
                                                    max_row_stride=mrs):
@@ -1106,13 +1123,21 @@
         qkv = torch.empty(xln1.shape[0], 3 * H, dtype=x2.dtype, device=x2.device)
         for i, (w, b) in enumerate(((P["wq"], P["bq"]), (P["wk"], None), (P["wv"], P["bv"]))):
             hip.gemm_nt(xln1, [w], [b] if b is not None else None, out=qkv[:, i * H:(i + 1) * H], ldc=3 * H)
-    attn = torch.empty_like(xln1)
+    if win is None:
+        attn_list = [False] * len(segs)
+    if info is not None:
+        info["attn_list"] = tuple(attn_list)
+    if attn is None:
+        attn = torch.empty_like(xln1)
     lses = []
-    for sg in segs:
+    for i, sg in enumerate(segs):
         r = slice(sg.row0, sg.end)
+        lst = None
+        if attn_list[i]:
+            lst = hip.live_samples(wsegs[i][0], wsegs[i][4], sg.B, sg.S, heads, fill=None if hip.mwindow_rule(sg.S)[0] > 0 else attn[r])
         _, lse = hip.attn_fwd(qkv[r, :H], qkv[r, H:2 * H], qkv[r, 2 * H:], 3 * H, sg.B, sg.S, heads, scale,
                               sg.bias.image.detach() if sg.bias is not None else None, sg.key_pad, hip.attn_spad(sg.S), out=attn[r],
-                              want_lse=keep, bias_frag=sg.frag(hip.ATTN_RESIDENT_MAX_S))
+                              want_lse=keep, bias_frag=sg.frag(hip.ATTN_RESIDENT_MAX_S), kept=lst)
         lses.append(lse)
         if sg.pad:
             attn[sg.end - sg.pad:sg.end].zero_()
@@ -1277,16 +1302,18 @@
         N = kept.total if mapped else x2.shape[0]
         scale = (H // heads) ** -0.5
         ctx.dg_fused = need_grad and dgamma_from_wgrad_ok([N], P["g1"], [P["wo"]], [P["bo"]], needs["g1"], [needs["wo"]])
+        info = {}
         if mapped:
             x_mid = torch.empty_like(x_full)
             _, acts = _attn_forward(x_full, P, segs, heads, scale, rowscale, rps, keep, want_y=needs["g1"] and not ctx.dg_fused,
-                                    xmap=kept.rowmap(), out=x_mid)
+                                    xmap=kept.rowmap(), out=x_mid, info=info)
             hip.rows_merge(x_full, None, kept, out=x_mid)
         else:
             x_mid, acts = _attn_forward(x2, P, segs, heads, scale, rowscale, rps, keep, want_y=needs["g1"] and not ctx.dg_fused,
-                                        listed=kept is None and ctx.dg_fused)
+                                        listed=kept is None and ctx.dg_fused, info=info)
             if kept is not None:
                 x_mid = hip.rows_merge(x_full, x_mid, kept)
+        ctx.attn_list = info["attn_list"]
         ctx.kept, ctx.mapped = kept, mapped
         ctx.segs, ctx.dims, ctx.n_params, ctx.first_param = segs, (N, H, heads, scale, rps), len(params), first_param
         ctx.direct = ()
@@ -1326,8 +1353,10 @@
                 if needs["wo"] and P["aln_w"] is not None:
                     A["aln"] = hip.layernorm_fwd(A["attn"], P["aln_w"], P["aln_b"])[0]
         else:
+            info = {}
             _, A = _attn_forward(x2, P, segs, heads, scale, rowscale, rps, True, want_y=not ctx.dg_fused, xmap=xmap,
-                                 out=torch.empty_like(x2) if mapped else None, listed=kept is None and ctx.dg_fused)
+                                 out=torch.empty_like(x2) if mapped else None, listed=kept is None and ctx.dg_fused, info=info)
+            assert info["attn_list"] == ctx.attn_list
         if not dx_mid.is_contiguous():
             dx_mid = dx_mid.contiguous()
         dx_full = dx_mid
@@ -1388,10 +1417,13 @@
                 if sg.pad:
                     dqkv[sg.end - sg.pad:sg.end].zero_()
                 dparts = {n: dqkv[r, slot[n] * H:(slot[n] + 1) * H] for n in qkv_names}
+                lst = None
+                if ctx.attn_list[i]:
+                    lst = hip.live_samples(rowscale[sg.row0 // rps:], sg.S // rps, sg.B, sg.S, heads, fill=dqkv[r])
                 _attn_backward(qkv[r], dattn[r], A["attn"][r], A["lse%d" % i], sg.B, sg.S, heads, scale,
                                sg.bias.image.detach() if sg.bias is not None else None, sg.bias.imageT if sg.bias is not None else None,
                                sg.key_pad, sg.bias.grad_accumulator(sg.B) if want_dbias[i] else None, sg.frag(384),
-                               dparts["wq"], dparts["wk"], dparts["wv"])
+                               dparts["wq"], dparts["wk"], dparts["wv"], kept=lst)
             bias_of = {"wq": "bq", "wv": "bv"}
             bnames = tuple(bias_of[n] for n in cols if n in bias_of and needs[bias_of[n]])
             if bnames:
@@ -1766,17 +1798,18 @@
     return out, vec
 
 
-def _attn_backward(qkv, dattn, attn, lse, B, S, heads, scale, bias_img, biasT, key_pad, dbias_acc, bias_frag, dq, dk, dv):
+def _attn_backward(qkv, dattn, attn, lse, B, S, heads, scale, bias_img, biasT, key_pad, dbias_acc, bias_frag, dq, dk, dv, kept=None):
     H = heads * 64
     dev = qkv.device
     Spad = hip.attn_spad(S)
     delta = torch.empty(B, heads, Spad, dtype=torch.float32, device=dev)
+    assert kept is None or (attn.stride(0) == dattn.stride(0) and not SEPARATE_DELTA)
     if attn.stride(0) != dattn.stride(0) or SEPARATE_DELTA:
         hip._check(hip.lib().op_attn_bwd_delta(hip.ptr(dattn), hip.ptr(attn), dattn.stride(0), hip.ptr(delta), B, S, Spad, heads,
                                                hip.stream()), "op_attn_bwd_delta")
         attn = None
     hip.attn_bwd_launch(qkv[:, :H], qkv[:, H:2 * H], qkv[:, 2 * H:], 3 * H, dattn, bias_img, biasT, key_pad, lse, delta, dq, dk,
-                        dv, dq.stride(0), dbias_acc, B, S, Spad, heads, scale, bias_frag, out=attn)
+                        dv, dq.stride(0), dbias_acc, B, S, Spad, heads, scale, bias_frag, out=attn, kept=kept)
 
 
 def attn_branch(x, bias, key_pad, ps, heads, params, save_acts=False):
```

New measurement: 210.4 (median of 2 runs). About the same (+0.2%).
